# antonilo/unsupervised_detection

Measured on AMD Instinct MI355X. Metric: frame-pairs/sec per adversarial step, DAVIS 480p batch4, 1/2/4/8 GPU, higher is better.
Workload: dtype f32

## Files before the change

### include/udet.h

```cpp
#ifndef UDET_H
#define UDET_H
#include <stddef.h>
#ifdef __cplusplus
extern "C" {
#endif

#define UDET_OK 0
#define UDET_ERR_SHAPE (-1)
#define UDET_ERR_ALIGN (-2)
#define UDET_ERR_HIP (-3)
#define UDET_ERR_UNSUPPORTED (-4)
#define UDET_ERR_ARG (-5)
#define UDET_ERR_OVERFLOW (-6)

#define UDET_ACT_NONE 0
#define UDET_ACT_LEAKY 1
#define UDET_ACT_ELU 2

int udet_version(void);
const char* udet_last_error(void);


int udet_warp(const float* image, const float* flow, float flow_scale, float* out, int n, int h, int w, int c,
              void* stream);
// ... 31 lines not shown
size_t udet_conv2d_workspace_bytes(int n, int h, int w, int cin, int cout, int kh, int kw, int upsample2x);
int udet_conv2d(const float* x, const float* w_hwio, const float* bias, float* y, int n, int h, int w, int cin, int cout,
                int kh, int kw, int stride, int dilation, int upsample2x, int act, float alpha, void* workspace,
                size_t workspace_bytes, void* stream);
int udet_conv2d_backward_data(const float* dy, const float* y_saved, const float* w_hwio, float* dx, int n, int h, int w,
                              int cin, int cout, int kh, int kw, int stride, int dilation, int act, float alpha,
                              void* workspace, size_t workspace_bytes, void* stream);
int udet_conv2d_backward_filter(const float* x, const float* dy, const float* y_saved, float* dw_hwio, float* dbias, int n,
                                int h, int w, int cin, int cout, int kh, int kw, int stride, int dilation, int upsample2x,
                                int act, float alpha, void* workspace, size_t workspace_bytes, void* stream);
int udet_conv2d_transpose4x4s2(const float* x, const float* w_hwoi, const float* bias, float* y, int n, int h, int w,
                               int cin, int cout, void* workspace, size_t workspace_bytes, void* stream);


size_t udet_stage_workspace_bytes(int n);
int udet_flow_normalize(const float* flow, float* out, int n, int h, int w, void* workspace, size_t workspace_bytes, void* stream);
int udet_charbonnier_loss(const float* gt_flows, const float* pred_flows, const float* masks, int mask_channels, int n, int h, int w,
                          float cbn, float* out, void* workspace, size_t workspace_bytes, void* stream);
int udet_losses_forward(const float* flow, const float* mask, const float* pred3, int b, int h, int w, float cbn, float epsilon,
                        float* losses8, float* coef, void* workspace, size_t workspace_bytes, void* stream);
int udet_losses_backward(const float* flow, const float* mask, const float* pred3, const float* coef, int which, int b, int h, int w,
                         float cbn, float* dpred, float* dmask, void* stream);
int udet_clip_or_noise(float* g, size_t n, float clip, const float* flag2, unsigned long long seed, long step, void* stream);
int udet_adam_step(float* w, const float* g, float* m, float* v, size_t n, float lr, float beta1, float beta2, float eps, long t,
                   void* stream);

typedef struct udet_plan udet_plan;
typedef struct {
  int batch;
  int in_h, in_w;
  int img_h, img_w;
  float flow_normalizer;
  float cbn;
  float epsilon;
  float lr, beta1, beta2, adam_eps;
  float clip;
  unsigned long long noise_seed;
  int conv_fp16;
} udet_config;

int udet_plan_create(const udet_config* cfg, udet_plan** out);
void udet_plan_destroy(udet_plan* plan);
size_t udet_workspace_bytes(const udet_plan* plan);
int udet_plan_init(udet_plan* plan, void* workspace, void* stream);

int udet_param_count(int net);
size_t udet_param_total(int net);
int udet_param_info(int net, int index, const char** name, int* rank, int* shape4, size_t* offset_floats);
int udet_buffer_count(const udet_plan* plan);
int udet_buffer_info(const udet_plan* plan, int index, const char** name, size_t* offset_bytes, int* dims_nhw_ld);

int udet_pack_pwc(udet_plan* plan, const float* w_pwc, void* workspace, void* stream);
int udet_pack_trainable(udet_plan* plan, const float* w_gen, const float* w_rec, void* workspace, void* stream);

int udet_pwc_forward(udet_plan* plan, const float* img1, const float* img2, void* workspace, void* stream);
int udet_forward(udet_plan* plan, const float* img1, const float* img2, int ncalls, void* workspace, void* stream);
int udet_prefetch_flow(udet_plan* plan, const float* img1, const float* img2, void* workspace, void* stream);
int udet_forward_prefetched(udet_plan* plan, int ncalls, void* workspace, void* stream);
int udet_prefetch_consume(udet_plan* plan, void* workspace, void* stream);
int udet_forward_from_flow(udet_plan* plan, int ncalls, void* workspace, void* stream);
int udet_generator_forward(udet_plan* plan, void* workspace, void* stream);
int udet_generator_layers(udet_plan* plan, void* workspace, void* stream);
int udet_recover_forward(udet_plan* plan, int n, void* workspace, void* stream);
int udet_backward(udet_plan* plan, int which, const float* w_gen, const float* w_rec, float* g_gen, float* g_rec,
                  void* workspace, void* stream);
int udet_stream_wait_grads(udet_plan* plan, int net, void* stream);
int udet_generator_backward(udet_plan* plan, const float* w_gen, float* g_gen, void* workspace, void* stream);
int udet_recover_backward(udet_plan* plan, const float* w_rec, float* g_rec, void* workspace, void* stream);
int udet_grad_absmean(udet_plan* plan, int net, const float* g, float* out2, void* workspace, void* stream);
int udet_apply(udet_plan* plan, int net, float* w, float* g, float* m, float* v, void* workspace, void* stream);
long udet_fp16_overflow_count(udet_plan* plan);
long udet_get_adam_step(const udet_plan* plan);
void udet_set_adam_step(udet_plan* plan, long t);
int udet_train_step(udet_plan* plan, int which, const float* img1, const float* img2, float* w_gen, float* w_rec,
                    float* g_gen, float* g_rec, float* m_gen, float* v_gen, float* m_rec, float* v_rec, void* workspace,
                    void* stream);

int udet_autotune(udet_plan* plan, const float* w_gen, const float* w_rec, float* g_gen, float* g_rec, void* workspace,
                  void* stream);
int udet_tuned_shapes(void);
int udet_tune_save(const char* path);
int udet_tune_load(const char* path);
int udet_tune_rejected(void);
int udet_profile_begin(udet_plan* plan);
int udet_profile_end(udet_plan* plan, double* out, int ncat, void* stream);

int udet_plan_set_concurrent(udet_plan* plan, int on);

int udet_plan_lane_queues(udet_plan* plan, void* stream, int* queue);
int udet_plan_pin_lanes(udet_plan* plan, void* stream, void* const* side_streams, int n);

#ifdef __cplusplus
}
#endif
#endif
```

### include/udet_debug.h

```cpp
#ifndef UDET_DEBUG_H
#define UDET_DEBUG_H
#ifdef __cplusplus
extern "C" {
#endif
void udet_debug_force_conv(int bm, int bn, int ks);
void udet_debug_conv_fp16(int on);
void udet_debug_force_wgrad(int nsplit, int dma);
int udet_debug_last_wgrad(void);
void udet_debug_upb_min_pixels(long v);
void udet_debug_set_tuning(int on);
void udet_debug_force_pair(int on);
int udet_debug_last_pair(void);
#include <stddef.h>
int udet_debug_conv2d_pair(const float* xa, const float* xb, const float* wa, const float* wb, const float* ba, const float* bb, float* ya, float* yb,
                           int na, int nb, int h, int w, int cin, int cout, int k, int stride, int dilation, int act, float alpha, void* workspace,
                           size_t workspace_bytes, void* stream);
int udet_debug_last_conv(void);
#ifdef __cplusplus
}
#endif
#endif
```

### unsupervised_detection_amd/_devel.py

```python
from __future__ import annotations

import ctypes
import os

from ._ffi import lib as _lib

_PATH = os.path.join(os.path.dirname(os.path.abspath(__file__)), "libudet_debug.so")
if not os.path.exists(_PATH):
    raise RuntimeError(f"{_PATH} is missing: build it with `make -C unsupervised_detection_amd/csrc`")
dbg = ctypes.CDLL(_PATH, mode=ctypes.RTLD_GLOBAL)
dbg.udet_debug_force_conv.restype = None
dbg.udet_debug_force_conv.argtypes = [ctypes.c_int, ctypes.c_int, ctypes.c_int]
dbg.udet_debug_last_conv.restype = ctypes.c_int
dbg.udet_debug_last_conv.argtypes = []
dbg.udet_debug_conv_fp16.restype = None
dbg.udet_debug_conv_fp16.argtypes = [ctypes.c_int]
dbg.udet_debug_force_wgrad.restype = None
dbg.udet_debug_force_wgrad.argtypes = [ctypes.c_int, ctypes.c_int]
dbg.udet_debug_upb_min_pixels.restype = None
dbg.udet_debug_upb_min_pixels.argtypes = [ctypes.c_long]
dbg.udet_debug_set_tuning.restype = None
dbg.udet_debug_set_tuning.argtypes = [ctypes.c_int]
dbg.udet_debug_last_wgrad.restype = ctypes.c_int
dbg.udet_debug_last_wgrad.argtypes = []
dbg.udet_debug_force_pair.restype = None
dbg.udet_debug_force_pair.argtypes = [ctypes.c_int]
dbg.udet_debug_last_pair.restype = ctypes.c_int
dbg.udet_debug_last_pair.argtypes = []
dbg.udet_debug_conv2d_pair.restype = ctypes.c_int
dbg.udet_debug_conv2d_pair.argtypes = [ctypes.c_void_p] * 8 + [ctypes.c_int] * 10 + [ctypes.c_float, ctypes.c_void_p, ctypes.c_size_t, ctypes.c_void_p]
```

### unsupervised_detection_amd/csrc/api_plan.hip

```cpp
#include <stdlib.h>
#include <string.h>

#include "conv_host.h"
#include "elementwise.h"
#include "plan.h"

using namespace udet;

struct udet_plan {
  Plan* p;
};

extern "C" {

int udet_plan_create(const udet_config* c, udet_plan** out) {
  if (!c || !out) { set_error("plan_create: null argument"); return UDET_ERR_ARG; }
  Config k;
  k.batch = c->batch; k.in_h = c->in_h; k.in_w = c->in_w; k.img_h = c->img_h; k.img_w = c->img_w;
  k.flow_normalizer = c->flow_normalizer; k.cbn = c->cbn; k.epsilon = c->epsilon;
  k.lr = c->lr; k.beta1 = c->beta1; k.beta2 = c->beta2; k.adam_eps = c->adam_eps; k.clip = c->clip;
  k.noise_seed = c->noise_seed;
  k.conv_fp16 = c->conv_fp16 ? 1 : 0;
  Plan* P = plan_build(k);
  if (!P) return UDET_ERR_SHAPE;
// ... 8 lines not shown

int udet_param_count(int net) { return (net < 0 || net > 2) ? 0 : (int)net_params(net).p.size(); }
size_t udet_param_total(int net) { return (net < 0 || net > 2) ? 0 : net_params(net).total; }
int udet_param_info(int net, int i, const char** name, int* rank, int* shape, size_t* offset) {
  if (net < 0 || net > 2 || i < 0 || i >= (int)net_params(net).p.size()) { set_error("param_info: out of range"); return UDET_ERR_ARG; }
  const ParamDesc& d = net_params(net).p[i];
  *name = d.name.c_str(); *rank = d.rank; *offset = d.offset;
  for (int k = 0; k < 4; ++k) shape[k] = d.shape[k];
  return UDET_OK;
}
int udet_buffer_count(const udet_plan* h) { return (int)h->p->bufs.size(); }
int udet_buffer_info(const udet_plan* h, int i, const char** name, size_t* offset_bytes, int* dims) {
  if (i < 0 || i >= (int)h->p->bufs.size()) { set_error("buffer_info: out of range"); return UDET_ERR_ARG; }
  const Buf& b = h->p->bufs[i];
  *name = b.name.c_str(); *offset_bytes = b.off * sizeof(float);
  dims[0] = b.n; dims[1] = b.h; dims[2] = b.w; dims[3] = b.ld;
  return UDET_OK;
}
int udet_plan_set_concurrent(udet_plan* h, int on) {
  if (!h) { set_error("plan_set_concurrent: null plan"); return UDET_ERR_ARG; }
  if (on)
    if (h->p->cand.empty()) { set_error("plan_set_concurrent: the plan has no side streams"); return UDET_ERR_UNSUPPORTED; }
  h->p->concurrent = on != 0;
  return UDET_OK;
}
int udet_plan_lane_queues(udet_plan* h, void* stream, int* queue) {
  if (!h || !queue) { set_error("plan_lane_queues: null argument"); return UDET_ERR_ARG; }
  return plan_lane_queues(h->p, (hipStream_t)stream, queue);
}
int udet_plan_pin_lanes(udet_plan* h, void* stream, void* const* side_streams, int n) {
  if (!h || (n > 0 && !side_streams)) { set_error("plan_pin_lanes: null argument"); return UDET_ERR_ARG; }
  return plan_pin_lanes(h->p, (hipStream_t)stream, reinterpret_cast<hipStream_t const*>(side_streams), n);
}
long udet_fp16_overflow_count(udet_plan* h) {
  if (!h) return 0;
  (void)plan_check_overflow(h->p, true);
  return h->p->ovf_skipped;
}
long udet_get_adam_step(const udet_plan* h) {
  plan_settle_adam_step(h->p);
  return h->p->adam_t;
}
void udet_set_adam_step(udet_plan* h, long t) {
  plan_settle_adam_step(h->p);
  h->p->adam_t = t;
}

int udet_pack_pwc(udet_plan* h, const float* w_pwc, void* ws, void* stream) {
  return plan_pack_pwc(h->p, w_pwc, (float*)ws, (hipStream_t)stream);
}
int udet_pack_trainable(udet_plan* h, const float* w_gen, const float* w_rec, void* ws, void* stream) {
  return plan_pack_trainable(h->p, w_gen, w_rec, (float*)ws, (hipStream_t)stream);
}
int udet_pwc_forward(udet_plan* h, const float* img1, const float* img2, void* ws, void* stream) {
  return plan_pwc_forward(h->p, img1, img2, (float*)ws, (hipStream_t)stream);
}
int udet_forward_from_flow(udet_plan* h, int ncalls, void* ws, void* stream) {
  UDET_TRY(plan_check_overflow(h->p, false));
  if (ncalls < 0 || ncalls > 3) { set_error("forward: ncalls must be 0..3"); return UDET_ERR_ARG; }
  return plan_forward(h->p, nullptr, nullptr, ncalls, (float*)ws, (hipStream_t)stream);
}
int udet_generator_forward(udet_plan* h, void* ws, void* stream) {
  UDET_TRY(plan_generator_forward(h->p, (float*)ws, (hipStream_t)stream));
  return plan_recover_forward(h->p, 0, (float*)ws, (hipStream_t)stream);
}
int udet_generator_layers(udet_plan* h, void* ws, void* stream) {
  h->p->ev_next = 0;
  UDET_TRY(plan_generator_layers(h->p, (float*)ws, (hipStream_t)stream));
  return plan_recover_forward(h->p, 0, (float*)ws, (hipStream_t)stream);
}
int udet_recover_forward(udet_plan* h, int n, void* ws, void* stream) {
  if (n < 1 || n > 3) { set_error("recover_forward: n must be 1..3 (multiples of the plan batch)"); return UDET_ERR_ARG; }
  return plan_recover_forward(h->p, n, (float*)ws, (hipStream_t)stream, true);
}
int udet_forward(udet_plan* h, const float* img1, const float* img2, int ncalls, void* ws, void* stream) {
  UDET_TRY(plan_check_overflow(h->p, false));
  if (ncalls < 0 || ncalls > 3) { set_error("forward: ncalls must be 0..3"); return UDET_ERR_ARG; }
  if (!img1 || !img2) { set_error("forward: null image pointer"); return UDET_ERR_ARG; }
  return plan_forward(h->p, img1, img2, ncalls, (float*)ws, (hipStream_t)stream);
}
int udet_prefetch_flow(udet_plan* h, const float* img1, const float* img2, void* ws, void* stream) {
  if (!img1 || !img2) { set_error("prefetch_flow: null image pointer"); return UDET_ERR_ARG; }
  return plan_prefetch(h->p, img1, img2, (float*)ws, (hipStream_t)stream);
}
int udet_prefetch_consume(udet_plan* h, void* ws, void* stream) {
  return plan_prefetch_consume(h->p, (float*)ws, (hipStream_t)stream);
}
int udet_forward_prefetched(udet_plan* h, int ncalls, void* ws, void* stream) {
  UDET_TRY(plan_check_overflow(h->p, false));
  if (ncalls < 0 || ncalls > 3) { set_error("forward: ncalls must be 0..3"); return UDET_ERR_ARG; }
  return plan_forward(h->p, nullptr, nullptr, ncalls, (float*)ws, (hipStream_t)stream, true);
}
int udet_backward(udet_plan* h, int which, const float* w_gen, const float* w_rec, float* g_gen, float* g_rec, void* ws,
                  void* stream) {
  UDET_TRY(plan_check_overflow(h->p, false));
  if (which < 1 || which > 3) { set_error("backward: which must be 1 (generator), 2 (recover) or 3 (both)"); return UDET_ERR_ARG; }
  return plan_backward(h->p, which, w_gen, w_rec, g_gen, g_rec, (float*)ws, (hipStream_t)stream);
}
int udet_apply(udet_plan* h, int net, float* w, float* g, float* m, float* v, void* ws, void* stream) {
  return plan_apply(h->p, net, w, g, m, v, (float*)ws, (hipStream_t)stream);
}
int udet_train_step(udet_plan* h, int which, const float* img1, const float* img2, float* w_gen, float* w_rec, float* g_gen,
                    float* g_rec, float* m_gen, float* v_gen, float* m_rec, float* v_rec, void* ws, void* stream) {
  UDET_TRY(udet_pack_trainable(h, w_gen, w_rec, ws, stream));
  UDET_TRY(udet_forward(h, img1, img2, 3, ws, stream));
  UDET_TRY(udet_backward(h, which, w_gen, w_rec, g_gen, g_rec, ws, stream));
  if (which & 1) UDET_TRY(udet_apply(h, NET_GEN, w_gen, g_gen, m_gen, v_gen, ws, stream));
  if (which & 2) UDET_TRY(udet_apply(h, NET_REC, w_rec, g_rec, m_rec, v_rec, ws, stream));
  return UDET_OK;
}

int udet_autotune(udet_plan* h, const float* w_gen, const float* w_rec, float* g_gen, float* g_rec, void* ws_, void* stream) {
  Plan* P = h->p;
  float* ws = (float*)ws_;
  hipStream_t s = (hipStream_t)stream;
  if (!P->pwc_packed) { set_error("autotune: pack the PWC-Net and trainable weights first"); return UDET_ERR_ARG; }
  const size_t lo = P->packed_floats, hi = P->small_off;
  UDET_TRY(launch_fill_uniform(ws + lo, (long)(hi - lo), 0x5eedull, -0.5f, 0.5f, s));
  const size_t img_floats = (size_t)P->cfg.batch * P->cfg.in_h * P->cfg.in_w * 3;
  if (P->wgrad_floats < 2 * img_floats) { set_error("autotune: workspace too small for the probe images"); return UDET_ERR_ARG; }
  const float* img1 = ws + P->wgrad_off[0];
  const float* img2 = img1 + img_floats;
  const bool was_concurrent = P->concurrent;
  P->concurrent = false;
  conv_set_tuning(1);
  wgrad_set_tuning(1);
  int rc = udet_forward(h, img1, img2, 3, ws_, stream);
  if (rc == UDET_OK) rc = udet_backward(h, 3, w_gen, w_rec, g_gen, g_rec, ws_, stream);
  conv_set_tuning(0);
  wgrad_set_tuning(0);
  P->concurrent = was_concurrent;
  UDET_HIP(hipMemsetAsync(ws + lo, 0, (hi - lo) * sizeof(float), s));
  UDET_HIP(hipStreamSynchronize(s));
  return rc;
}
int udet_tuned_shapes(void) { return conv_tuned_shapes() + wgrad_tuned_shapes() + conv_pair_tuned_shapes(); }
int udet_tune_save(const char* path) {
  FILE* f = path ? fopen(path, "w") : nullptr;
  if (!f) { set_error("tune_save: cannot open %s", path ? path : "(null)"); return UDET_ERR_ARG; }
  fprintf(f, "udet-tune 2 abi %d\n", UDET_TUNE_ABI);
  conv_tune_dump(f);
  wgrad_tune_dump(f);
  conv_pair_tune_dump(f);
  fclose(f);
  return UDET_OK;
}
int udet_tune_load(const char* path) {
  FILE* f = path ? fopen(path, "r") : nullptr;
  if (!f) { set_error("tune_load: cannot open %s", path ? path : "(null)"); return UDET_ERR_ARG; }
  char line[256];
  int n = 0, ver = 0, abi = -1;
  if (!fgets(line, sizeof(line), f) || sscanf(line, "udet-tune %d abi %d", &ver, &abi) != 2 || ver != 2 || abi != UDET_TUNE_ABI) {
    fclose(f);
    set_error("tune_load: %s is not a udet-tune 2 file of this build (abi %d)", path, UDET_TUNE_ABI);
    return UDET_ERR_ARG;
  }
  while (fgets(line, sizeof(line), f)) {
    unsigned long long key;
    int a, b, c, d, e;
// ... 83 lines not shown
```

### unsupervised_detection_amd/csrc/common.h

```cpp
#pragma once
#include <hip/hip_runtime.h>
#include <hip/hip_ext.h>
#include <stdint.h>
#include <stdio.h>
#include <string>

#include "../../include/udet.h"

namespace udet {

void set_error(const char* fmt, ...);
int hip_fail(hipError_t e, const char* what);
#define UDET_HIP(x)                                   \
  do {                                                \
    hipError_t _e = (x);                              \
    if (_e != hipSuccess) return udet::hip_fail(_e, #x); \
  } while (0)
#define UDET_TRY(x)            \
  do {                         \
    int _s = (x);              \
    if (_s != 0) return _s;    \
  } while (0)

struct LaunchSink {
// ... 76 lines not shown
  int OHq, OWq;
  int osy, osx, ooy, oox;
  int isy, isx;
  int ntaps;
  ConvTap taps[UDET_MAX_TAPS];
  int ncls;
  int cls_tap[5];
  int nseg;
  ConvSeg seg[UDET_MAX_SEGS];
  int seg_tap[UDET_MAX_SEGS + 1];
  const ConvTap* tap_tab;
  int Mall;
  FastDiv fd_ohw, fd_ow;
  int kfast;
  const float* zero16;
  int act;
  float alpha;
  const float* res;
  int ldres, res_coff;
  float* y2;
  int ldy2, y2_coff;
  int accumulate;
  float* uo;
  int ldu, u_coff;
  const float* ua;
  int ldua, ua_coff, uact;
  float ualpha;
  int u_c0, u_c1;
  int ksplit;
  float* partial;
  size_t partial_cap;
  int ldp;
  int fold;
  int* tickets;
  int tail_full, tail_ks, tail_prow0;
  int f16;
  float f16_xscale;
  const float* wino_u;
  int wino_np;
  int kreal;
};
#define UDET_MAX_TICKETS 4096

int launch_conv(ConvParams& p, hipStream_t stream);
int launch_conv_pair(ConvParams& a, ConvParams& b, hipStream_t stream);
int launch_tap_gather(const ConvParams& g, const float* z, int ldz, hipStream_t stream);

struct PackJob {
  long src_off, dst_off, gamma_off, beta_off;
  long total;
  int T, R, C, Kc, ldw, k_split, k_gap, mode;
};

struct WgradParams {
  const float* x;
  int ldx, x_coff;
  int N, H, W, up_shift;
  int Cin;
  const float* dy;
  const float* ya;
  int ldy, y_coff, Cout;
  int yact;
  float yalpha;
  int OH, OW, isy, isx;
  int ycls, OHf, OWf;
  int ntaps;
  ConvTap taps[UDET_MAX_TAPS];
  float* dw;
  float* db;
  float* partial;
  size_t partial_floats;
  const float* zero16;
  int swapped, oCin, oCout, bias_m;
  int Cin4, Mpad;
  float* pbias;
  FastDiv fd_ohw, fd_ow;
  const float* w;
  const float* b;
  const float* gamma;
  float* dgamma;
  float* dbeta;
  float bn_c;
  int f16;
  float f16_yscale;
};
int launch_wgrad_T(WgradParams& p, int T, hipStream_t stream);
int launch_bn_finalize(float* dw, int T, int Cin, int Cout, const float* w, const float* b, const float* gamma, float bn_c, float* pd,
                       float* db, float* dgamma, float* dbeta, hipStream_t stream);
int launch_wgrad_up_combine(const float* deff, float* dw, int Cin, int Cout, hipStream_t stream);
size_t wgrad_partial_floats_needed(int T, int Cin, int Cout);

}
```

### unsupervised_detection_amd/csrc/conv_host.h

```cpp
#pragma once
#include "common.h"
namespace udet {
void same_pad(int in, int k, int s, int d, int* before, int* out);
void conv_setup_fwd(ConvParams& p, int N, int H, int W, int kh, int kw, int s, int d);
int conv_dgrad_classes(int s, int H, int W);
void conv_force_config(int bm, int bn, int ks);
bool conv_thin_n_ok(const ConvParams& p);
bool conv_thin_k_ok(const ConvParams& p);
int launch_conv_thin_n(const ConvParams& p, hipStream_t stream);
int launch_conv_thin_k(const ConvParams& p, hipStream_t stream);
bool conv_wino_geometry(const ConvParams& p, int* dil, int widx_at[9]);
bool conv_wino_ok(const ConvParams& p);
bool conv_wino_variant_ok(const ConvParams& p, int variant);
int conv_wino_np(int cout);
size_t conv_wino_floats(int Kc, int cout);
long conv_wino_workgroups(const ConvParams& p, int variant);
int conv_wino_max_ksplit(const ConvParams& p, int variant);
int launch_conv_wino(ConvParams& p, int variant, int ks, hipStream_t stream);
int launch_splitk_second_pass(const ConvParams& p, hipStream_t stream);
int launch_wino_pack(const float* src, float* dst, int R, int C, int Kc, int np, int k_split, int k_gap, int transposed, hipStream_t stream);
int launch_wino_from_packed(const ConvParams& p, float* dst, int np, hipStream_t stream);
void conv_debug_f16(int on);
int conv_debug_f16_on();
int conv_last_config();
void conv_set_tuning(int on);
int conv_tuned_shapes();
void conv_clear_tuning();
int conv_tune_rejected();
void conv_tune_note_reject();
float* tune_scratch(size_t floats, int which);
bool tune_compare(const float* a, const float* b, size_t n, hipStream_t stream, float* diff_out, float* scale_out);
void wgrad_set_tuning(int on);
bool wgrad_wino_ok(const WgradParams& p);
int wgrad_wino_slices(const WgradParams& p, int wanted);
int launch_wgrad_wino(const WgradParams& q, int slices, int ldn, hipStream_t stream);
int wgrad_last_config();
void wgrad_force(int nsplit, int dma);
int wgrad_tuned_shapes();
void conv_tune_dump(FILE* f);
void conv_tune_put(unsigned long long key, int bm, int bn, int ks, int ws, int fold, int tail);
void wgrad_tune_dump(FILE* f);
void conv_pair_tune_dump(FILE* f);
void conv_pair_tune_put(unsigned long long key, int bm, int bn, int ks, int ws);
int conv_pair_tuned_shapes();
void conv_pair_clear_tuning();
void conv_force_pair(int on);
int conv_last_pair();
#define UDET_TUNE_ABI 6
void wgrad_tune_put(unsigned long long key, int cfg);
bool conv_setup_dgrad(ConvParams& p, int cls, int N, int H, int W, int kh, int kw, int s, int d);
int launch_pack_weights(const float* src, float* dst, int T, int R, int C, int Kc, int ldw, int k_split, int k_gap,
                        int mode, const float* scale, hipStream_t stream);
int launch_pack_taps_into_n(const float* src, float* dst, int T, int R, int C, int Kc, int ldz, int k_split, int k_gap,
                            int transposed, hipStream_t stream);
int launch_pack_jobs(const PackJob* jobs_dev, int njobs, const float* wsrc, float* ws, float bn_c, hipStream_t stream);
int launch_fold_bn(const float* b, const float* gamma, const float* beta, float c, float* scale, float* bias_f, int n,
                   hipStream_t stream);
int launch_copy_channels(const float* src, int lds, int s_coff, float* dst, int ldd, int d_coff, long P, int C, float mul,
                         float add, hipStream_t stream);
int launch_warp(const float* img, const float* flow, int ldf, int f_coff, float flow_scale, float* out, int N, int H,
                int W, int C, int* dbg_idx, float* dbg_alpha, hipStream_t stream);
int launch_cost_volume(const float* c1, const float* wr, float* out, int ldo, int o_coff, int N, int H, int W, int C,
                       hipStream_t stream);
int launch_warp_cost_volume(const float* c1, const float* c2, const float* flow, int ldf, int f_coff, float flow_scale, float* out,
                            int ldo, int corr_coff, int c1_coff, float* warped_dbg, int N, int H, int W, int C, hipStream_t stream);
inline int round_up(int v, int m) { return (v + m - 1) / m * m; }
}
```

### unsupervised_detection_amd/csrc/conv_host.hip

```cpp
#include <string.h>

#include <stdint.h>

#include "common.h"
#include "conv_host.h"
#include "wino_pack.h"

namespace udet {

void same_pad(int in, int k, int s, int d, int* before, int* out) {
  const int o = (in + s - 1) / s;
  int total = (o - 1) * s + (k - 1) * d + 1 - in;
  if (total < 0) total = 0;
  *before = total / 2;
  *out = o;
}

static inline int floordiv2(int v) { return v >= 0 ? v / 2 : -((-v + 1) / 2); }

static void push_tap(ConvParams& p, int dy, int dx, int widx) {
  const int ymax = (p.OHq - 1) * p.isy + dy, xmax = (p.OWq - 1) * p.isx + dx;
  if (dy >= p.H || ymax < 0 || dx >= p.W || xmax < 0) return;
  p.taps[p.ntaps].dy = dy;
  p.taps[p.ntaps].dx = dx;
// ... 52 lines not shown
        if (((vx % 2) + 2) % 2) continue;
        push_tap(p, floordiv2(vy), floordiv2(vx), ky * kw + kx);
      }
    }
  }
  if (merged) {
    p.ncls = 4;
    p.cls_tap[4] = p.ntaps;
    p.ooy = p.oox = 0;
    p.OHq = H / 2; p.OWq = W / 2;
  }
  return true;
}

__global__ __launch_bounds__(256) void pack_weights_kernel(const float* __restrict__ src, float* __restrict__ dst, int T,
                                                           int R, int C, int Kc, int ldw, int k_split, int k_gap,
                                                           int mode, const float* __restrict__ scale) {
  const long total = (long)T * Kc * ldw;
  for (long e = (long)blockIdx.x * 256 + threadIdx.x; e < total; e += (long)gridDim.x * 256) {
    const int n = (int)(e % ldw);
    const int k = (int)((e / ldw) % Kc);
    const int t = (int)(e / ((long)ldw * Kc));
    float v = 0.f;
    int ks = k;
    if (k >= k_split) ks = (k < k_split + k_gap) ? -1 : k - k_gap;
    const int r = mode == 0 ? ks : n, c = mode == 0 ? n : ks;
    if (r >= 0 && r < R && c >= 0 && c < C) {
      v = src[((long)t * R + r) * C + c];
      if (scale) v *= scale[c];
    }
    dst[e] = v;
  }
}

int launch_pack_weights(const float* src, float* dst, int T, int R, int C, int Kc, int ldw, int k_split, int k_gap,
                        int mode, const float* scale, hipStream_t stream) {
  const long total = (long)T * Kc * ldw;
  int nb = (int)((total + 255) / 256);
  if (nb > 2048) nb = 2048;
  UDET_LAUNCH(pack_weights_kernel, dim3(nb), dim3(256), 0, stream, src, dst, T, R, C, Kc, ldw, k_split, k_gap,
                     mode, scale);
  UDET_HIP(hipGetLastError());
  return UDET_OK;
}

__constant__ float UPB_MERGE[2][3][3][4] = {
    {{{.5f, 0.f, 0.f, 0.f}, {.5f, 1.f, .5f, 0.f}, {0.f, 0.f, .5f, 1.f}},
     {{.5f, 0.f, 0.f, 0.f}, {.5f, 1.f, 1.f, 0.f}, {0.f, 0.f, 0.f, 0.f}},
     {{0.f, 0.f, 0.f, 0.f}, {0.f, 0.f, .5f, 0.f}, {0.f, 0.f, -.5f, -1.f}}},
    {{{1.f, .5f, 0.f, 0.f}, {0.f, .5f, 1.f, .5f}, {0.f, 0.f, 0.f, .5f}},
     {{1.f, 1.f, 0.f, 0.f}, {0.f, 0.f, 0.f, 0.f}, {0.f, 0.f, 0.f, 0.f}},
     {{0.f, .5f, 0.f, 0.f}, {0.f, -.5f, -1.f, -.5f}, {0.f, 0.f, 0.f, -.5f}}}};

__global__ __launch_bounds__(256) void pack_jobs_kernel(const PackJob* __restrict__ jobs, const float* __restrict__ wsrc,
                                                        float* __restrict__ ws, float bn_c) {
  const PackJob j = jobs[blockIdx.y];
  const float* src = wsrc + j.src_off;
  float* dst = ws + j.dst_off;
  const float* gamma = j.gamma_off >= 0 ? wsrc + j.gamma_off : nullptr;
  if (j.mode == 2) {
    for (long e = (long)blockIdx.x * 256 + threadIdx.x; e < j.total; e += (long)gridDim.x * 256)
      dst[e] = gamma ? src[e] * (gamma[e] * bn_c) + wsrc[j.beta_off + e] : src[e];
    return;
  }
  if (j.mode == 9 || j.mode == 10) {
    const int rv = (int)(j.beta_off / 3), cv = (int)(j.beta_off % 3);
    for (long e = (long)blockIdx.x * 256 + threadIdx.x; e < j.total; e += (long)gridDim.x * 256) {
      const int n = (int)(e % j.ldw), k = (int)(e / j.ldw);
      int ks = k;
      if (k >= j.k_split) ks = (k < j.k_split + j.k_gap) ? -1 : k - j.k_gap;
      const int ci = j.mode == 9 ? ks : n, co = j.mode == 9 ? n : ks;
      const bool real = ci >= 0 && ci < j.R && co >= 0 && co < j.C;
      float w[4][4];
#pragma unroll
      for (int kk = 0; kk < 4; ++kk)
#pragma unroll
        for (int ll = 0; ll < 4; ++ll) w[kk][ll] = real ? src[((long)(kk * 4 + ll) * j.R + ci) * j.C + co] : 0.f;
      const long plane = (long)j.Kc * j.ldw;
#pragma unroll
      for (int py = 0; py < 2; ++py) {
        float t1[3][4];
#pragma unroll
        for (int a = 0; a < 3; ++a)
#pragma unroll
          for (int ll = 0; ll < 4; ++ll) {
            float v = 0.f;
#pragma unroll
            for (int kk = 0; kk < 4; ++kk) v += UPB_MERGE[py][rv][a][kk] * w[kk][ll];
            t1[a][ll] = v;
          }
#pragma unroll
        for (int px = 0; px < 2; ++px)
#pragma unroll
          for (int a = 0; a < 3; ++a)
#pragma unroll
            for (int bb = 0; bb < 3; ++bb) {
              float v = 0.f;
#pragma unroll
              for (int ll = 0; ll < 4; ++ll) v += UPB_MERGE[px][cv][bb][ll] * t1[a][ll];
              dst[(long)((py * 2 + px) * 9 + a * 3 + bb) * plane + e] = v;
            }
      }
    }
    return;
  }
  if (j.mode == 7 || j.mode == 8) {
    for (long e = (long)blockIdx.x * 256 + threadIdx.x; e < j.total; e += (long)gridDim.x * 256) wino_pack_item(j, src, gamma, bn_c, dst, e);
    return;
  }
  for (long e = (long)blockIdx.x * 256 + threadIdx.x; e < j.total; e += (long)gridDim.x * 256) {
    const int n = (int)(e % j.ldw);
    const int k = (int)((e / j.ldw) % j.Kc);
    int t = (int)(e / ((long)j.ldw * j.Kc));
    float v = 0.f;
    int ks = k;
    if (k >= j.k_split) ks = (k < j.k_split + j.k_gap) ? -1 : k - j.k_gap;
    int r = j.mode == 0 ? ks : n, c = j.mode == 0 ? n : ks;
    if (j.mode == 3 || j.mode == 4) {
      t = n / j.C;
      c = n - t * j.C;
      r = ks;
      if (t >= j.T) r = -1;
    }
    if (j.mode >= 5) {
      const int cls = t >> 2, ty = (t >> 1) & 1, tx = t & 1, py = cls >> 1, px = cls & 1;
      const int y0 = py == 0 ? (ty == 0 ? 0 : 1) : (ty == 0 ? 0 : 2), y1 = py == 0 ? (ty == 0 ? 0 : 2) : (ty == 0 ? 1 : 2);
      const int x0 = px == 0 ? (tx == 0 ? 0 : 1) : (tx == 0 ? 0 : 2), x1 = px == 0 ? (tx == 0 ? 0 : 2) : (tx == 0 ? 1 : 2);
      const int ci = j.mode == 5 ? ks : n, co = j.mode == 5 ? n : ks;
      if (ci >= 0 && ci < j.R && co >= 0 && co < j.C) {
        for (int ky = y0; ky <= y1; ++ky)
          for (int kx = x0; kx <= x1; ++kx) v += src[((long)(ky * 3 + kx) * j.R + ci) * j.C + co];
        if (gamma) v *= gamma[co] * bn_c;
      }
      dst[e] = v;
      continue;
    }
    if (r >= 0 && r < j.R && c >= 0 && c < j.C) {
      v = j.mode == 4 ? src[((long)t * j.C + c) * j.R + r] : src[((long)t * j.R + r) * j.C + c];
      if (gamma) v *= gamma[c] * bn_c;
    }
    dst[e] = v;
  }
}
int launch_pack_jobs(const PackJob* jobs_dev, int njobs, const float* wsrc, float* ws, float bn_c, hipStream_t stream) {
  if (njobs < 1) return UDET_OK;
  UDET_LAUNCH(pack_jobs_kernel, dim3(48, njobs), dim3(256), 0, stream, jobs_dev, wsrc, ws, bn_c);
  UDET_HIP(hipGetLastError());
  return UDET_OK;
}

__global__ __launch_bounds__(256) void pack_job_kernel(const PackJob j, const float* __restrict__ wsrc, float* __restrict__ ws) {
  const float* src = wsrc + j.src_off;
  float* dst = ws + j.dst_off;
  for (long e = (long)blockIdx.x * 256 + threadIdx.x; e < j.total; e += (long)gridDim.x * 256) {
    const int n = (int)(e % j.ldw);
    const int k = (int)((e / j.ldw) % j.Kc);
    int ks = k;
    if (k >= j.k_split) ks = (k < j.k_split + j.k_gap) ? -1 : k - j.k_gap;
    const int t = n / j.C, c = n - t * j.C;
    float v = 0.f;
    if (ks >= 0 && ks < j.R && t < j.T) v = j.mode == 4 ? src[((long)t * j.C + c) * j.R + ks] : src[((long)t * j.R + ks) * j.C + c];
    dst[e] = v;
  }
}
int launch_pack_taps_into_n(const float* src, float* dst, int T, int R, int C, int Kc, int ldz, int k_split, int k_gap,
                            int transposed, hipStream_t stream) {
  PackJob j;
  memset(&j, 0, sizeof(j));
  j.T = T; j.R = R; j.C = C; j.Kc = Kc; j.ldw = ldz; j.k_split = k_split; j.k_gap = k_gap;
  j.mode = transposed ? 4 : 3; j.total = (long)Kc * ldz; j.gamma_off = -1;
  int nb = (int)((j.total + 255) / 256);
  if (nb > 1024) nb = 1024;
  UDET_LAUNCH(pack_job_kernel, dim3(nb), dim3(256), 0, stream, j, src, dst);
  UDET_HIP(hipGetLastError());
  return UDET_OK;
}

__global__ __launch_bounds__(256) void tap_gather_kernel(const ConvParams g, const float* __restrict__ z, int ldz) {
  const long total = (long)g.N * g.OH * g.OW * g.Cout;
  for (long e = (long)blockIdx.x * 256 + threadIdx.x; e < total; e += (long)gridDim.x * 256) {
    const int co = (int)(e % g.Cout);
    const long pix = e / g.Cout;
    const int ox = (int)(pix % g.OW), oy = (int)((pix / g.OW) % g.OH), n = (int)(pix / ((long)g.OW * g.OH));
    int cls = 0, qy = oy, qx = ox;
    if (g.ncls > 1) {
      cls = (oy & 1) * 2 + (ox & 1);
      qy = oy >> 1;
      qx = ox >> 1;
    }
    float v = g.bias ? g.bias[co] : 0.f;
    const int t1 = g.cls_tap[cls + 1];
    for (int t0 = g.cls_tap[cls]; t0 < t1; t0 += 8) {
      float a[8];
#pragma unroll
      for (int u = 0; u < 8; ++u) {
        const int t = t0 + u < t1 ? t0 + u : t1 - 1;
        const int iy = qy + g.taps[t].dy, ix = qx + g.taps[t].dx;
        const bool ok = t0 + u < t1 && (unsigned)iy < (unsigned)g.H && (unsigned)ix < (unsigned)g.W;
        a[u] = ok ? z[((size_t)(n * g.H + iy) * g.W + ix) * ldz + g.taps[t].widx * g.Cout + co] : 0.f;
// ... 97 lines not shown
```

### unsupervised_detection_amd/csrc/devel/api_debug.hip

```cpp
#include <string.h>

#include "../../../include/udet_debug.h"
#include "../conv_host.h"
#include "../plan.h"

using namespace udet;

extern "C" {
int udet_debug_last_conv(void) { return conv_last_config(); }
void udet_debug_force_conv(int bm, int bn, int ks) { conv_force_config(bm, bn, ks); }
void udet_debug_conv_fp16(int on) { conv_debug_f16(on); }
void udet_debug_force_wgrad(int nsplit, int dma) { wgrad_force(nsplit, dma); }
int udet_debug_last_wgrad(void) { return wgrad_last_config(); }
void udet_debug_upb_min_pixels(long v) { plan_debug_upb_min_pixels(v); }
void udet_debug_force_pair(int on) { conv_force_pair(on); }
int udet_debug_last_pair(void) { return conv_last_pair(); }
int udet_debug_conv2d_pair(const float* xa, const float* xb, const float* wa, const float* wb, const float* ba, const float* bb, float* ya, float* yb,
                           int na, int nb, int h, int w, int cin, int cout, int k, int stride, int dilation, int act, float alpha, void* workspace,
                           size_t workspace_bytes, void* stream_) {
  hipStream_t stream = (hipStream_t)stream_;
  if (cin % 8 != 0 || k * k > UDET_MAX_TAPS) { set_error("debug_conv2d_pair: cin must be a multiple of 8"); return UDET_ERR_SHAPE; }
  const int kc = cin, ldw = round_up(cout, 4);
  const size_t wfl = ((size_t)k * k * kc * ldw + 63) & ~(size_t)63, part_fl = (size_t)4 << 20, zero_fl = 64 + UDET_MAX_TICKETS;
  if (workspace_bytes < (2 * wfl + part_fl + zero_fl) * sizeof(float)) { set_error("debug_conv2d_pair: workspace too small"); return UDET_ERR_ARG; }
  float* wpa = reinterpret_cast<float*>(workspace);
  float* wpb = wpa + wfl;
  float* part = wpb + wfl;
  float* zero = part + part_fl;
  UDET_HIP(hipMemsetAsync(zero, 0, zero_fl * sizeof(float), stream));
  UDET_TRY(launch_pack_weights(wa, wpa, k * k, cin, cout, kc, ldw, kc, 0, 0, nullptr, stream));
  UDET_TRY(launch_pack_weights(wb, wpb, k * k, cin, cout, kc, ldw, kc, 0, 0, nullptr, stream));
  ConvParams p[2];
  for (int i = 0; i < 2; ++i) {
    memset(&p[i], 0, sizeof(ConvParams));
    conv_setup_fwd(p[i], i ? nb : na, h, w, k, k, stride, dilation);
    p[i].x = i ? xb : xa; p[i].ldx = cin; p[i].wp = i ? wpb : wpa; p[i].Kc = kc; p[i].ldw = ldw; p[i].bias = i ? bb : ba;
    p[i].y = i ? yb : ya; p[i].ldy = cout; p[i].Cout = cout; p[i].act = act; p[i].alpha = alpha;
    p[i].partial = part; p[i].partial_cap = part_fl; p[i].zero16 = zero; p[i].tickets = reinterpret_cast<int*>(zero + 64);
  }
  return launch_conv_pair(p[0], p[1], stream);
}
void udet_debug_set_tuning(int on) {
  conv_set_tuning(on);
  wgrad_set_tuning(on);
}
}
```

### unsupervised_detection_amd/csrc/elementwise.h

```cpp
#pragma once
#include "common.h"
namespace udet {
int launch_resize_bilinear_fwd(const float* x, int ldx, int x_coff, int N, int H, int W, float* y, int ldy, int y_coff,
                               int OH, int OW, int C, float mul, float div, hipStream_t s);
int launch_resize_bilinear_bwd(const float* dy, int ldy, int y_coff, int N, int OH, int OW, float* dx, int ldx, int x_coff,
                               int H, int W, int C, int accumulate, hipStream_t s);
int launch_upb_ring(const float* x, int ld, int N, int H, int W, float* xh, hipStream_t s);
int launch_upb_ring_fold(const float* dxh, int ld, int N, int H, int W, float* dx, hipStream_t s);
int launch_share_samples(float* buf, long P, int ld, int coff, int C, int copies, hipStream_t s);
int launch_fold_samples(float* buf, long P, int ld, int coff, int C, int copies, hipStream_t s);
int launch_emit_du(const float* d, const float* a, float* u, long P, int ld, int coff, int C, int act, float alpha, hipStream_t s);
int launch_pool2x2_sum(const float* du, float* dx, int N, int H, int W, int C, hipStream_t s);
int launch_pack_pwc_input(const float* i1, const float* i2, float* x8, long P, hipStream_t s);
int launch_gen_input(const float* img, const float* f, double* part, float* gin, int B, long HW, hipStream_t s);
size_t flow_stats_doubles(int B);
int launch_mask_rec_inputs(const float* logits, const float* f, float* mask, float* fin, long P, int ncalls, hipStream_t s);
int launch_pack_imgin(const float* img, float* imgin, long P, int ncalls, hipStream_t s);
int launch_losses(const float* f, const float* mask, const float* pred, long HW, int B, float cbn, float eps,
                  float num_pixels, float* part, float* losses, float* coef, float* sums, hipStream_t s);
size_t loss_part_floats(int B);
int launch_rec_loss_bwd(const float* f, const float* mask, const float* pred, float* dpred, long BHW, float cbn,
                        float inv_np, hipStream_t s);
int launch_gen_loss_bwd(const float* f, const float* mask, const float* pred, const float* coef, float* dpred,
                        float* dmask, long HW, int B, float cbn, hipStream_t s);
int launch_mask_bwd(const float* dmask, const float* dfin, const float* f, const float* mask, float* dlogits, long P,
                    hipStream_t s);
int launch_grad_absmean(const float* g, const long* seg_off, const long* seg_len, int nvars, float* vmean, float thresh,
                        float* out, hipStream_t s);
int launch_adam(float* w, float* g, float* m, float* v, long n, float lr_t, float b1, float b2, float eps, float clip,
                const float* flag, uint64_t seed, uint64_t step, hipStream_t s, int mode = 0, const int* skip = nullptr);
int launch_nonfinite_count(const float* g, long n, int* out, hipStream_t s);
int launch_flow_normalize(const float* f, double* part, float* out, int B, long HW, hipStream_t s);
int launch_charbonnier(const float* gt, const float* pred, const float* mask, int mc, int B, long HW, float cbn, float* part,
                       float* out, hipStream_t s);
int launch_crop_flip_resize(const void* src, int src_u8, int nearest, int N, int H, int W, int C, const int* prm, float* dst, int OH,
                            int OW, float div, float add, hipStream_t s);
int launch_crop_flip_resize_ragged(const void* src, int src_u8, int nearest, int N, int C, const long long* offsets, const int* hw,
                                   const int* prm, float* dst, int OH, int OW, float div, float add, hipStream_t s);
int launch_mask_stats(const float* pred, const float* gt, int N, int H, int W, float threshold, float gt_threshold, double* out,
                      hipStream_t s);
int launch_fill_uniform(float* x, long n, uint64_t seed, float lo, float hi, hipStream_t s);
int launch_axpy(const float* x, float* y, long n, float a, int accumulate, hipStream_t s);
}
```

### unsupervised_detection_amd/csrc/elementwise.hip

```cpp
#include "common.h"
#include "elementwise.h"

namespace udet {

static inline int grid_for(long total, int cap = 4096) {
  long nb = (total + 255) / 256;
  if (nb > cap) nb = cap;
  if (nb < 1) nb = 1;
  return (int)nb;
}

template <typename T>
__device__ __forceinline__ T wave_sum(T v) {
#pragma unroll
  for (int o = 32; o > 0; o >>= 1) v += __shfl_down(v, o, 64);
  return v;
}
template <typename T>
__device__ __forceinline__ T block_sum(T v, T* sm ) {
  v = wave_sum(v);
  __syncthreads();
  if ((threadIdx.x & 63) == 0) sm[threadIdx.x >> 6] = v;
  __syncthreads();
  return sm[0] + sm[1] + sm[2] + sm[3];
// ... 441 lines not shown
  return UDET_OK;
}

__global__ __launch_bounds__(256) void mask_rec_inputs_kernel(const float* __restrict__ logits ,
                                                              const float* __restrict__ f, float* __restrict__ mask,
                                                              float* __restrict__ fin, long P, int ncalls) {
  for (long q = (long)blockIdx.x * 256 + threadIdx.x; q < P; q += (long)gridDim.x * 256) {
    const float l0 = logits[q * 8] / 10.f, l1 = logits[q * 8 + 1] / 10.f;
    const float mx = fmaxf(l0, l1);
    const float e0 = expf(l0 - mx), e1 = expf(l1 - mx);
    const float m = e0 / (e0 + e1);
    mask[q] = m;
    const float cm = 1.f - m;
    const float2 v = *reinterpret_cast<const float2*>(f + q * 2);
    const float a0 = 1.f - m, a1 = 1.f - cm;
    if (ncalls > 0) {
      *reinterpret_cast<float4*>(fin + q * 4) = make_float4(v.x * a0, v.y * a0, 1.f, a0);
    }
    if (ncalls > 1) {
      *reinterpret_cast<float4*>(fin + (P + q) * 4) = make_float4(v.x * a1, v.y * a1, 1.f, a1);
    }
    if (ncalls > 2) {
      *reinterpret_cast<float4*>(fin + (2 * P + q) * 4) = make_float4(0.f, 0.f, 1.f, 0.f);
    }
  }
}
int launch_mask_rec_inputs(const float* logits, const float* f, float* mask, float* fin, long P, int ncalls, hipStream_t s) {
  hipLaunchKernelGGL(mask_rec_inputs_kernel, dim3(grid_for(P)), dim3(256), 0, s, logits, f, mask, fin, P, ncalls);
  UDET_HIP(hipGetLastError());
  return UDET_OK;
}
__global__ __launch_bounds__(256) void pack_imgin_kernel(const float* __restrict__ img, float* __restrict__ imgin, long P,
                                                         int ncalls) {
  for (long q = (long)blockIdx.x * 256 + threadIdx.x; q < P; q += (long)gridDim.x * 256) {
    const float4 im = make_float4(img[q * 3], img[q * 3 + 1], img[q * 3 + 2], 0.f);
    for (int k = 0; k < ncalls; ++k) *reinterpret_cast<float4*>(imgin + (k * P + q) * 4) = im;
  }
}
int launch_pack_imgin(const float* img, float* imgin, long P, int ncalls, hipStream_t s) {
  hipLaunchKernelGGL(pack_imgin_kernel, dim3(grid_for(P)), dim3(256), 0, s, img, imgin, P, ncalls);
  UDET_HIP(hipGetLastError());
  return UDET_OK;
}

__device__ __forceinline__ float charb(float e, float cbn) {
  const float s = e * e + 0.001f * 0.001f;
  return cbn == 0.5f ? sqrtf(s) : powf(s, cbn);
}
__device__ __forceinline__ float charb_d(float e, float cbn) {
  const float s = e * e + 0.001f * 0.001f;
  return cbn == 0.5f ? e / sqrtf(s) : cbn * powf(s, cbn - 1.f) * 2.f * e;
}
#define LS_BLOCKS 64
__global__ __launch_bounds__(256) void loss_sums_kernel(const float* __restrict__ f, const float* __restrict__ mask,
                                                        const float* __restrict__ pred , long HW, int B,
                                                        float cbn, float* __restrict__ part ) {
  __shared__ float sm[4];
  const int n = blockIdx.y;
  float R = 0, Rc = 0, Pp = 0, Dr = 0, Dc = 0;
  for (long p = (long)blockIdx.x * 256 + threadIdx.x; p < HW; p += (long)gridDim.x * 256) {
    const long q = (long)n * HW + p;
    const float2 fl = *reinterpret_cast<const float2*>(f + q * 2);
    const float2 a = *reinterpret_cast<const float2*>(pred + q * 2);
    const float2 b = *reinterpret_cast<const float2*>(pred + ((long)B * HW + q) * 2);
    const float2 c = *reinterpret_cast<const float2*>(pred + ((long)2 * B * HW + q) * 2);
    const float m = mask[q], cm = 1.f - m;
    const float pa = charb(fl.x - a.x, cbn) + charb(fl.y - a.y, cbn);
    const float pb = charb(fl.x - b.x, cbn) + charb(fl.y - b.y, cbn);
    const float pc = charb(fl.x - c.x, cbn) + charb(fl.y - c.y, cbn);
    R += pa * m; Rc += pb * cm; Pp += pc; Dr += pc * m; Dc += pc * cm;
  }
  R = block_sum(R, sm); Rc = block_sum(Rc, sm); Pp = block_sum(Pp, sm); Dr = block_sum(Dr, sm); Dc = block_sum(Dc, sm);
  if (threadIdx.x == 0) {
    float* o = part + ((long)n * LS_BLOCKS + blockIdx.x) * 5;
    o[0] = R; o[1] = Rc; o[2] = Pp; o[3] = Dr; o[4] = Dc;
  }
}
__global__ void loss_finish_kernel(const float* __restrict__ part, int B, float eps, float num_pixels,
                                   float* __restrict__ losses, float* __restrict__ coef, float* __restrict__ sums) {
  if (threadIdx.x != 0 || blockIdx.x != 0) return;
  float red = 0.f, redc = 0.f, rs = 0.f;
  for (int b = 0; b < B; ++b) {
    float v[5] = {0, 0, 0, 0, 0};
    for (int k = 0; k < LS_BLOCKS; ++k)
      for (int j = 0; j < 5; ++j) v[j] += part[((long)b * LS_BLOCKS + k) * 5 + j];
    const float D = v[3] + eps, Dc = v[4] + eps;
    red += 1.f - v[0] / D;
    redc += 1.f - v[1] / Dc;
    rs += v[0] + v[1] + v[2];
    coef[b * 4 + 0] = -1.f / (B * D);
    coef[b * 4 + 1] = v[0] / (B * D * D);
    coef[b * 4 + 2] = -1.f / (B * Dc);
    coef[b * 4 + 3] = v[1] / (B * Dc * Dc);
    for (int j = 0; j < 5; ++j) sums[b * 5 + j] = v[j];
    if (b == 0) { losses[4] = v[0]; losses[5] = v[1]; losses[6] = D; losses[7] = Dc; }
  }
  red /= B; redc /= B;
  losses[0] = red + redc;
  losses[1] = rs / num_pixels;
  losses[2] = red;
  losses[3] = redc;
}
int launch_losses(const float* f, const float* mask, const float* pred, long HW, int B, float cbn, float eps,
                  float num_pixels, float* part, float* losses, float* coef, float* sums, hipStream_t s) {
  hipLaunchKernelGGL(loss_sums_kernel, dim3(LS_BLOCKS, B), dim3(256), 0, s, f, mask, pred, HW, B, cbn, part);
  hipLaunchKernelGGL(loss_finish_kernel, dim3(1), dim3(64), 0, s, part, B, eps, num_pixels, losses, coef, sums);
  UDET_HIP(hipGetLastError());
  return UDET_OK;
}
size_t loss_part_floats(int B) { return (size_t)B * LS_BLOCKS * 5; }

__global__ __launch_bounds__(256) void charbonnier_sum_kernel(const float* __restrict__ gt, const float* __restrict__ pred,
                                                              const float* __restrict__ mask, int mc, long HW, float cbn,
                                                              float* __restrict__ part ) {
  __shared__ float sm[4];
  const int n = blockIdx.y;
  float acc = 0.f;
  for (long p = (long)blockIdx.x * 256 + threadIdx.x; p < HW; p += (long)gridDim.x * 256) {
    const long q = (long)n * HW + p;
    const float2 a = *reinterpret_cast<const float2*>(gt + q * 2);
    const float2 b = *reinterpret_cast<const float2*>(pred + q * 2);
    const float m0 = mask ? mask[q * mc] : 1.f, m1 = mask ? mask[q * mc + (mc - 1)] : 1.f;
    acc += charb(a.x - b.x, cbn) * m0 + charb(a.y - b.y, cbn) * m1;
  }
  acc = block_sum(acc, sm);
  if (threadIdx.x == 0) part[(long)n * LS_BLOCKS + blockIdx.x] = acc;
}
__global__ void charbonnier_finish_kernel(const float* __restrict__ part, int B, float* __restrict__ out) {
  const int b = blockIdx.x * blockDim.x + threadIdx.x;
  if (b >= B) return;
  float v = 0.f;
  for (int k = 0; k < LS_BLOCKS; ++k) v += part[(long)b * LS_BLOCKS + k];
  out[b] = v;
}
int launch_charbonnier(const float* gt, const float* pred, const float* mask, int mc, int B, long HW, float cbn, float* part,
                       float* out, hipStream_t s) {
  hipLaunchKernelGGL(charbonnier_sum_kernel, dim3(LS_BLOCKS, B), dim3(256), 0, s, gt, pred, mask, mc, HW, cbn, part);
  hipLaunchKernelGGL(charbonnier_finish_kernel, dim3((B + 63) / 64), dim3(64), 0, s, part, B, out);
  UDET_HIP(hipGetLastError());
  return UDET_OK;
}

__global__ __launch_bounds__(256) void rec_loss_bwd_kernel(const float* __restrict__ f, const float* __restrict__ mask,
                                                           const float* __restrict__ pred, float* __restrict__ dpred,
                                                           long BHW, float cbn, float inv_np) {
  for (long q = (long)blockIdx.x * 256 + threadIdx.x; q < BHW; q += (long)gridDim.x * 256) {
    const float2 fl = *reinterpret_cast<const float2*>(f + q * 2);
    const float m = mask[q], cm = 1.f - m;
    const float2 a = *reinterpret_cast<const float2*>(pred + q * 2);
    const float2 b = *reinterpret_cast<const float2*>(pred + (BHW + q) * 2);
    const float2 c = *reinterpret_cast<const float2*>(pred + (2 * BHW + q) * 2);
    *reinterpret_cast<float2*>(dpred + q * 2) = make_float2(-charb_d(fl.x - a.x, cbn) * m * inv_np, -charb_d(fl.y - a.y, cbn) * m * inv_np);
    *reinterpret_cast<float2*>(dpred + (BHW + q) * 2) = make_float2(-charb_d(fl.x - b.x, cbn) * cm * inv_np, -charb_d(fl.y - b.y, cbn) * cm * inv_np);
    *reinterpret_cast<float2*>(dpred + (2 * BHW + q) * 2) = make_float2(-charb_d(fl.x - c.x, cbn) * inv_np, -charb_d(fl.y - c.y, cbn) * inv_np);
  }
}
int launch_rec_loss_bwd(const float* f, const float* mask, const float* pred, float* dpred, long BHW, float cbn,
                        float inv_np, hipStream_t s) {
  hipLaunchKernelGGL(rec_loss_bwd_kernel, dim3(grid_for(BHW)), dim3(256), 0, s, f, mask, pred, dpred, BHW, cbn, inv_np);
// ... 42 lines not shown
    dm += g1.x * fl.x + g1.y * fl.y + g1.w;
    const float m = mask[q];
    const float d0 = dm * m * (1.f - m) / 10.f;
    dlogits[q * 8] = d0;
    dlogits[q * 8 + 1] = -d0;
  }
}
int launch_mask_bwd(const float* dmask, const float* dfin, const float* f, const float* mask, float* dlogits, long P,
                    hipStream_t s) {
  hipLaunchKernelGGL(mask_bwd_kernel, dim3(grid_for(P)), dim3(256), 0, s, dmask, dfin, f, mask, dlogits, P);
  UDET_HIP(hipGetLastError());
  return UDET_OK;
}

#define GA_SPLIT 8
__global__ __launch_bounds__(256) void grad_absmean_kernel(const float* __restrict__ g, const long* __restrict__ seg_off,
                                                           const long* __restrict__ seg_len, float* __restrict__ vpart) {
  __shared__ float sm[4];
  const long off = seg_off[blockIdx.x], len = seg_len[blockIdx.x];
  const long b = len * blockIdx.y / GA_SPLIT, e = len * (blockIdx.y + 1) / GA_SPLIT;
  float s0 = 0.f, s1 = 0.f, s2 = 0.f, s3 = 0.f;
  long i = b + threadIdx.x;
  for (; i + 768 < e; i += 1024) {
    s0 += fabsf(g[off + i]);
    s1 += fabsf(g[off + i + 256]);
    s2 += fabsf(g[off + i + 512]);
    s3 += fabsf(g[off + i + 768]);
  }
  for (; i < e; i += 256) s0 += fabsf(g[off + i]);
  const float s = block_sum((s0 + s1) + (s2 + s3), sm);
  if (threadIdx.x == 0) vpart[blockIdx.x * GA_SPLIT + blockIdx.y] = s;
}
__global__ void grad_flag_kernel(const float* __restrict__ vpart, const long* __restrict__ seg_len, int nvars, float thresh,
                                 float* __restrict__ out ) {
  if (threadIdx.x == 0 && blockIdx.x == 0) {
    float s = 0.f;
    for (int i = 0; i < nvars; ++i) {
      float v = 0.f;
      for (int j = 0; j < GA_SPLIT; ++j) v += vpart[i * GA_SPLIT + j];
      s += v / (float)seg_len[i];
    }
    s /= (float)nvars;
    out[0] = s;
    out[1] = s < thresh ? 1.f : 0.f;
  }
}
int launch_grad_absmean(const float* g, const long* seg_off, const long* seg_len, int nvars, float* vmean, float thresh,
                        float* out, hipStream_t s) {
  hipLaunchKernelGGL(grad_absmean_kernel, dim3(nvars, GA_SPLIT), dim3(256), 0, s, g, seg_off, seg_len, vmean);
  hipLaunchKernelGGL(grad_flag_kernel, dim3(1), dim3(64), 0, s, vmean, seg_len, nvars, thresh, out);
  UDET_HIP(hipGetLastError());
  return UDET_OK;
}

__device__ __host__ __forceinline__ float udet_uniform01(uint64_t seed, uint64_t step, uint64_t idx) {
  uint64_t z = seed * 0x9E3779B97F4A7C15ull + step * 0xBF58476D1CE4E5B9ull + idx + 0x94D049BB133111EBull;
  z = (z ^ (z >> 30)) * 0xBF58476D1CE4E5B9ull;
  z = (z ^ (z >> 27)) * 0x94D049BB133111EBull;
  z = z ^ (z >> 31);
  return (float)(z >> 40) * (1.0f / 16777216.0f);
}

__global__ __launch_bounds__(256) void adam_kernel(float* __restrict__ w, float* __restrict__ g, float* __restrict__ m,
                                                   float* __restrict__ v, long n, float lr_t, float b1, float b2, float eps,
                                                   float clip, const float* __restrict__ flag, uint64_t seed,
                                                   uint64_t step, int mode, const int* __restrict__ skip) {
  if (skip && *skip != 0) return;
  const bool noise = flag && flag[1] != 0.f;
  for (long i = (long)blockIdx.x * 256 + threadIdx.x; i < n; i += (long)gridDim.x * 256) {
    float gi = g[i];
    if (mode != 2) {
      if (noise) gi = fabsf((udet_uniform01(seed, step, (uint64_t)i) * 2.f - 1.f) * clip);
      else gi = fminf(fmaxf(gi, -clip), clip);
      g[i] = gi;
      if (mode == 1) continue;
    }
    const float mi = m[i] + (gi - m[i]) * (1.f - b1);
    const float vi = v[i] + (gi * gi - v[i]) * (1.f - b2);
    m[i] = mi;
    v[i] = vi;
    w[i] = w[i] - lr_t * mi / (sqrtf(vi) + eps);
  }
}
__global__ __launch_bounds__(256) void fill_uniform_kernel(float* __restrict__ x, long n, uint64_t seed, float lo, float hi) {
  for (long i = (long)blockIdx.x * 256 + threadIdx.x; i < n; i += (long)gridDim.x * 256)
    x[i] = lo + (hi - lo) * udet_uniform01(seed, 0, (uint64_t)i);
}
int launch_fill_uniform(float* x, long n, uint64_t seed, float lo, float hi, hipStream_t s) {
  hipLaunchKernelGGL(fill_uniform_kernel, dim3(grid_for(n, 8192)), dim3(256), 0, s, x, n, seed, lo, hi);
  UDET_HIP(hipGetLastError());
  return UDET_OK;
}
__global__ __launch_bounds__(256) void mask_stats_kernel(const float* __restrict__ pred, const float* __restrict__ gt, int H, int W,
                                                         float threshold, float gt_threshold, double* __restrict__ out) {
  __shared__ double sm[4];
  const int n = blockIdx.x;
  const long HW = (long)H * W;
  double v[8] = {0, 0, 0, 0, 0, 0, 0, 0};
  for (long q = threadIdx.x; q < HW; q += 256) {
    const int y = (int)(q / W), x = (int)(q - (long)y * W);
    const float g = gt[n * HW + q];
    const bool pr = pred[n * HW + q] > threshold, gb = g > gt_threshold;
    const int strips = (y < 2) + (y >= H - 2) + (x < 2) + (x >= W - 2);
    const double a1 = fabs((double)g - 1.0), a0 = fabs((double)g);
    if (pr) {
      v[0] += strips; v[1] += 1.0; v[4] += a1; v[7] += a0;
      if (gb) v[3] += 1.0;
    } else {
      v[5] += a0; v[6] += a1;
    }
    if (gb) v[2] += 1.0;
  }
  for (int k = 0; k < 8; ++k) {
    const double s = block_sum(v[k], sm);
    if (threadIdx.x == 0) out[(long)n * 8 + k] = s;
    __syncthreads();
  }
}
int launch_mask_stats(const float* pred, const float* gt, int N, int H, int W, float threshold, float gt_threshold, double* out,
                      hipStream_t s) {
  hipLaunchKernelGGL(mask_stats_kernel, dim3(N), dim3(256), 0, s, pred, gt, H, W, threshold, gt_threshold, out);
  UDET_HIP(hipGetLastError());
  return UDET_OK;
}
int launch_adam(float* w, float* g, float* m, float* v, long n, float lr_t, float b1, float b2, float eps, float clip,
                const float* flag, uint64_t seed, uint64_t step, hipStream_t s, int mode, const int* skip) {
  hipLaunchKernelGGL(adam_kernel, dim3(grid_for(n, 2048)), dim3(256), 0, s, w, g, m, v, n, lr_t, b1, b2, eps, clip, flag, seed,
                     step, mode, skip);
  UDET_HIP(hipGetLastError());
  return UDET_OK;
}
__global__ __launch_bounds__(256) void nonfinite_count_kernel(const float* __restrict__ g, long n, int* __restrict__ out) {
  int c = 0;
  for (long i = (long)blockIdx.x * 256 + threadIdx.x; i < n; i += (long)gridDim.x * 256) c += !(fabsf(g[i]) <= 3.402823466e38f);
#pragma unroll
  for (int o = 32; o > 0; o >>= 1) c += __shfl_xor(c, o);
  if ((threadIdx.x & 63) == 0 && c) {
    atomicAdd(out, c);
    atomicAdd(out + 1, c);
  }
}
int launch_nonfinite_count(const float* g, long n, int* out, hipStream_t s) {
  UDET_HIP(hipMemsetAsync(out, 0, sizeof(int), s));
  hipLaunchKernelGGL(nonfinite_count_kernel, dim3(grid_for(n, 1024)), dim3(256), 0, s, g, n, out);
  UDET_HIP(hipGetLastError());
  return UDET_OK;
}

__global__ __launch_bounds__(256) void upb_ring_kernel(const float* __restrict__ x, int ldx, int N, int H, int W, float* __restrict__ xh, int C4) {
  const int PH = H + 2, PW = W + 2;
  const long total = (long)N * PH * PW * C4;
  for (long e = (long)blockIdx.x * 256 + threadIdx.x; e < total; e += (long)gridDim.x * 256) {
    const int c4 = (int)(e % C4);
    const long pix = e / C4;
    const int C = (int)(pix % PW), R = (int)((pix / PW) % PH), n = (int)(pix / ((long)PW * PH));
    const int cy = R < 1 ? 0 : (R - 1 > H - 1 ? H - 1 : R - 1), cx = C < 1 ? 0 : (C - 1 > W - 1 ? W - 1 : C - 1);
    const float sg = ((R == 0) != (C == 0)) ? -1.f : 1.f;
    const float4 v = *reinterpret_cast<const float4*>(x + (((long)n * H + cy) * W + cx) * ldx + c4 * 4);
    *reinterpret_cast<float4*>(xh + pix * ldx + c4 * 4) = make_float4(v.x * sg, v.y * sg, v.z * sg, v.w * sg);
  }
}
int launch_upb_ring(const float* x, int ld, int N, int H, int W, float* xh, hipStream_t s) {
  const long total = (long)N * (H + 2) * (W + 2) * (ld / 4);
  hipLaunchKernelGGL(upb_ring_kernel, dim3(grid_for(total, 8192)), dim3(256), 0, s, x, ld, N, H, W, xh, ld / 4);
  UDET_HIP(hipGetLastError());
  return UDET_OK;
}
__global__ __launch_bounds__(256) void upb_ring_fold_kernel(const float* __restrict__ dxh, int ld, int N, int H, int W, float* __restrict__ dx, int C4) {
  const int PW = W + 2, PH = H + 2;
  const long total = (long)N * H * W * C4;
  for (long e = (long)blockIdx.x * 256 + threadIdx.x; e < total; e += (long)gridDim.x * 256) {
    const int c4 = (int)(e % C4);
    const long pix = e / C4;
    const int i = (int)(pix % W), j = (int)((pix / W) % H), n = (int)(pix / ((long)W * H));
    float4 a = make_float4(0.f, 0.f, 0.f, 0.f);
#pragma unroll
    for (int ry = 0; ry < 2; ++ry) {
      int R;
      float sy = 1.f;
      if (ry == 0) R = j + 1;
      else if (j == 0) { R = 0; sy = -1.f; }
// ... 38 lines not shown
```

### unsupervised_detection_amd/csrc/plan.h

```cpp
#pragma once
#include <map>
#include <string>
#include <vector>

#include "common.h"

namespace udet {

struct ParamDesc {
  std::string name;
  int rank;
  int shape[4];
  size_t offset, count;
};
struct NetParams {
  std::vector<ParamDesc> p;
  size_t total = 0;
  int add(const std::string& name, int a, int b = 0, int c = 0, int d = 0);
  int find(const std::string& name) const;
};
enum { NET_PWC = 0, NET_GEN = 1, NET_REC = 2 };
const NetParams& net_params(int net);

struct Buf {
// ... 31 lines not shown
    int seg_tap[UDET_MAX_SEGS + 1];
    std::vector<ConvTap> taps;
    size_t tab_off = 0;
  } upb_f, upb_b;
  int x = -1, x_coff = 0, y = -1, y_coff = 0;
  int res = -1, res_coff = 0, y2 = -1;
  int H = 0, W = 0;
  bool col2im = false;
  int ldz = 0, zbuf = -1;
  size_t wz_off = 0;
};

struct Config {
  int batch, in_h, in_w, img_h, img_w;
  float flow_normalizer, cbn, epsilon;
  float lr, beta1, beta2, adam_eps, clip;
  unsigned long long noise_seed;
  int conv_fp16 = 0;
};

struct Plan {
  Config cfg;
  std::vector<Buf> bufs;
  std::map<std::string, int> buf_by_name;
  std::vector<Layer> pwc, gen, rec;
  size_t packed_floats = 0;
  size_t arena_floats = 0;
  enum { NLANE = 6, NCAND = 8, MAXCAND = 32 };
  std::vector<hipStream_t> cand;
  struct Placement {
    hipStream_t main = nullptr;
    hipStream_t lane[NLANE] = {};
    int queue[NLANE] = {};
    int nqueues = 1;
  };
  std::vector<Placement> placements;
  int placed = -1;
  hipEvent_t prefetch_ev = nullptr;
  hipEvent_t grad_ev[3] = {nullptr, nullptr, nullptr};
  bool prefetch_pending = false;
  std::vector<hipEvent_t> ev_pool, ev_pool_prefetch;
  size_t ev_next = 0, ev_next_prefetch = 0;
  bool in_prefetch = false;
  bool concurrent = true;
  bool enc_a_shared = false;
  size_t scratch_off[NLANE] = {}, scratch_floats = 0;
  size_t wgrad_off[NLANE] = {}, wgrad_floats = 0;
  ~Plan();
  size_t small_off = 0;
  size_t ticket_off = 0;
  size_t seg_off[3] = {0, 0, 0};
  size_t jobs_off[3] = {0, 0, 0};
  int njobs[3] = {0, 0, 0};
  struct ProfRec {
    int cat; double flops, bytes; hipEvent_t a, b; std::string name;
    double mfma_scale = 1.0;
    enum { MAXK = 16 };
    hipEvent_t kev[2 * MAXK];
    LaunchSink sink;
  };
  bool profiling = false;
  std::vector<ProfRec*> prof;
  long adam_t = 0;
  int* ovf_host = nullptr;
  hipEvent_t ovf_ev[3] = {nullptr, nullptr, nullptr};
  bool ovf_pending[3] = {false, false, false};
  long ovf_skipped = 0;
  int ovf_report_values = 0, ovf_report_nets = 0;
  bool pwc_packed = false;
  int add_buf(const std::string& name, int n, int h, int w, int ld);
  const Buf& buf(int id) const { return bufs[id]; }
  int bid(const std::string& name) const;
};

#define UDET_PACKJOB_CAP(layers) (8 * (layers) + 32)
#define UDET_SMALL_NOISE 256
#define UDET_SMALL_OVF 300
#define UDET_SMALL_SUMS 1024
Plan* plan_build(const Config& cfg);
void plan_debug_upb_min_pixels(long v);
enum { UDET_KNOB_ENC_A_LANE = 0, UDET_KNOB_REC_DEC_WGRAD_LANE = 1, UDET_KNOB_REC_ENC_WGRAD_LANE = 2, UDET_KNOB_GEN_WGRAD_LATE = 3, UDET_KNOB_NO_WGRAD_WINO = 6, UDET_KNOB_SKIP = 7, UDET_KNOB_NO_PAIRS = 8, UDET_KNOB_COUNT = 12 };
#ifdef UDET_EXPERIMENT
void plan_debug_knob(int id, long v);
long plan_knob(int id);
#else
constexpr long plan_knob(int) { return 0; }
#endif

int plan_init_workspace(Plan* P, float* ws, hipStream_t s);
int plan_pack_pwc(Plan* P, const float* w_pwc, float* ws, hipStream_t s);
int plan_pack_trainable(Plan* P, const float* w_gen, const float* w_rec, float* ws, hipStream_t s);
int plan_pwc_forward(Plan* P, const float* img1, const float* img2, float* ws, hipStream_t s);
int plan_forward(Plan* P, const float* img1, const float* img2, int ncalls, float* ws, hipStream_t s, bool prefetched = false);
int plan_prefetch(Plan* P, const float* img1, const float* img2, float* ws, hipStream_t s);
int plan_prefetch_consume(Plan* P, float* ws, hipStream_t s);
int plan_generator_forward(Plan* P, float* ws, hipStream_t s);
int plan_generator_layers(Plan* P, float* ws, hipStream_t s);
int plan_recover_forward(Plan* P, int ncalls, float* ws, hipStream_t s, bool inputs_prepacked = false, bool skip_enc_a = false, bool enc_a_input_packed = false);
int plan_losses(Plan* P, float* ws, hipStream_t s);
int plan_backward(Plan* P, int which, const float* w_gen, const float* w_rec, float* g_gen, float* g_rec, float* ws, hipStream_t s);
int plan_apply(Plan* P, int net, float* w, float* g, float* m, float* v, float* ws, hipStream_t s);
int plan_check_overflow(Plan* P, bool wait);
void plan_settle_adam_step(Plan* P);
int plan_lane_queues(Plan* P, hipStream_t s, int* queue);
int plan_pin_lanes(Plan* P, hipStream_t main, hipStream_t const* streams, int n);
enum { PROF_CONV_FWD = 0, PROF_CONV_DGRAD = 1, PROF_CONV_WGRAD = 2, PROF_WARP = 3, PROF_CORR = 4, PROF_NCAT = 5 };
void prof_begin(Plan* P, int cat, double flops, double bytes, hipStream_t s, const char* name = "");
void prof_end(Plan* P, hipStream_t s);

}
```

### unsupervised_detection_amd/csrc/plan_build.hip

```cpp
#include <stdarg.h>
#include <stdlib.h>
#include <string.h>

#include "conv_host.h"
#include "elementwise.h"
#include "plan.h"

namespace udet {

int NetParams::add(const std::string& name, int a, int b, int c, int d) {
  ParamDesc q;
  q.name = name;
  q.shape[0] = a; q.shape[1] = b; q.shape[2] = c; q.shape[3] = d;
  q.rank = d ? 4 : (c ? 3 : (b ? 2 : 1));
  q.count = (size_t)a * (b ? b : 1) * (c ? c : 1) * (d ? d : 1);
  q.offset = total;
  total += q.count;
  p.push_back(q);
  return (int)p.size() - 1;
}
int NetParams::find(const std::string& name) const {
  for (size_t i = 0; i < p.size(); ++i)
    if (p[i].name == name) return (int)i;
  return -1;
// ... 91 lines not shown
    for (int i = 0; i < 9; ++i) {
      const int ci = ENC[i].cin ? ENC[i].cin : (e == 0 ? 3 : 4);
      n.add(S("FlownetS/%c%s/weights", e == 0 ? 'a' : 'b', ENC[i].suf), ENC[i].k, ENC[i].k, ci, ENC[i].cout);
      n.add(S("FlownetS/%c%s/biases", e == 0 ? 'a' : 'b', ENC[i].suf), ENC[i].cout);
    }
  for (int i = 0; i < 14; ++i) {
    n.add(S("FlownetS/%s/weights", DEC[i].name), DEC[i].k, DEC[i].k, DEC[i].cin, DEC[i].cout);
    n.add(S("FlownetS/%s/biases", DEC[i].name), DEC[i].cout);
  }
  return n;
}

const NetParams& net_params(int net) {
  static const NetParams pwc = build_pwc_params(), gen = build_gen_params(), rec = build_rec_params();
  return net == NET_PWC ? pwc : (net == NET_GEN ? gen : rec);
}

int Plan::add_buf(const std::string& name, int n, int h, int w, int ld) {
  Buf b;
  b.name = name; b.n = n; b.h = h; b.w = w; b.ld = ld; b.off = 0;
  bufs.push_back(b);
  buf_by_name[name] = (int)bufs.size() - 1;
  return (int)bufs.size() - 1;
}
int Plan::bid(const std::string& name) const {
  auto it = buf_by_name.find(name);
  return it == buf_by_name.end() ? -1 : it->second;
}

static Layer mk_layer(int net, const std::string& name, const std::string& wname, const std::string& bname, int k, int cin,
                      int cout, int stride, int dil, int act, float alpha) {
  Layer L;
  L.name = name; L.net = net;
  L.kh = L.kw = k; L.cin = cin; L.cout = cout; L.stride = stride; L.dil = dil;
  L.act = act; L.alpha = alpha;
  const NetParams& np = net_params(net);
  L.w_idx = np.find(wname);
  L.b_idx = np.find(bname);
  L.Kc = round_up(cin, cin <= 4 ? 4 : 8);
  L.ldw = round_up(cout, 4);
  L.k_split = L.Kc;
  L.k_gap = 0;
  return L;
}

static size_t align64(size_t v) { return (v + 63) & ~(size_t)63; }

Plan::~Plan() {
  for (auto& st : cand)
    if (st) (void)hipStreamDestroy(st);
  for (auto& e : ev_pool) (void)hipEventDestroy(e);
  for (auto& e : ev_pool_prefetch) (void)hipEventDestroy(e);
  if (prefetch_ev) (void)hipEventDestroy(prefetch_ev);
  for (auto* r : prof) delete r;
  for (auto& ev : grad_ev)
    if (ev) (void)hipEventDestroy(ev);
  for (auto& ev : ovf_ev)
    if (ev) (void)hipEventDestroy(ev);
  if (ovf_host) (void)hipHostFree(ovf_host);
}

static long g_upb_bwd_min = 8192;
void plan_debug_upb_min_pixels(long v) { g_upb_bwd_min = v < 0 ? 8192 : v; }
#ifdef UDET_EXPERIMENT
static long g_knob[UDET_KNOB_COUNT] = {};
void plan_debug_knob(int id, long v) { if (id >= 0 && id < UDET_KNOB_COUNT) g_knob[id] = v; }
long plan_knob(int id) { return id >= 0 && id < UDET_KNOB_COUNT ? g_knob[id] : 0; }
extern "C" void udet_exp_knob(int id, long v) { plan_debug_knob(id, v); }
#endif

static inline bool upb_used(int parity, int last, int a) { return !last || (parity == 0 ? a < 2 : a < 1); }
static void build_upb_launches(Layer& L, int h, int w) {
  Layer::SegLaunch& F = L.upb_f;
  F.nseg = 0; F.taps.clear();
  for (int r = 0; r < 4; ++r) {
    const int rv = r & 1, cv = r >> 1;
    const int r0 = rv ? h - 1 : 0, c0 = cv ? w - 1 : 0, nr = rv ? 1 : h - 1, nc = cv ? 1 : w - 1;
    for (int c = 0; c < 4; ++c) {
      const int py = c >> 1, px = c & 1;
      ConvSeg& g = F.seg[F.nseg];
      memset(&g, 0, sizeof(g));
      g.oy = 2 * r0 + py; g.ox = 2 * c0 + px; g.h = nr; g.w = nc;
      F.seg_tap[F.nseg++] = (int)F.taps.size();
      for (int a = 0; a < 3; ++a)
        for (int b = 0; b < 3; ++b) {
          if (!upb_used(py, rv, a) || !upb_used(px, cv, b)) continue;
          F.taps.push_back(ConvTap{r0 + a + py, c0 + b + px, r * 36 + 9 * c + 3 * a + b});
        }
    }
  }
  F.seg_tap[F.nseg] = (int)F.taps.size();
  Layer::SegLaunch& B = L.upb_b;
  B.nseg = 0; B.taps.clear();
  struct Combo { int p, a, last; };
  auto combos = [](int grp, std::vector<Combo>& out) {
    out.clear();
    for (int p = 0; p < 2; ++p)
      for (int a = 0; a < 3; ++a) {
        int last = 0;
        if (grp > 0) {
          const int rp = grp - 1;
          if (p + a < rp) continue;
          last = (p + a == rp);
        }
        if (upb_used(p, last, a)) out.push_back(Combo{p, a, last});
      }
// ... 295 lines not shown
      L.ldwT = round_up(L.cin, 4);
      L.wpT_off = off; off = align64(off + (size_t)T * L.KcT * L.ldwT);
    }
    if (L.up) {
      L.wu_off = off; off = align64(off + (size_t)16 * L.Kc * L.ldw);
      L.wuT_off = off; off = align64(off + (size_t)16 * L.KcT * L.ldwT);
    }
    if (L.upb) {
      L.wupb_off = off; off = align64(off + (size_t)4 * 36 * L.Kc * L.ldw);
      L.upb_f.tab_off = off; off = align64(off + L.upb_f.taps.size() * (sizeof(ConvTap) / sizeof(float)));
      if (L.upb_bwd) {
        L.wupbT_off = off; off = align64(off + (size_t)4 * 36 * L.KcT * L.ldwT);
        L.upb_b.tab_off = off; off = align64(off + L.upb_b.taps.size() * (sizeof(ConvTap) / sizeof(float)));
      }
    }
    if (!cfg.conv_fp16 && L.kh == 3 && L.kw == 3 && L.stride == 1 && !L.up && !L.transposed && !L.col2im && L.cout >= 16 && L.H * L.W >= 512) {
      if (L.Kc % 8 == 0) {
        L.wino_np = conv_wino_np(L.cout);
        L.wino_off = off; off = align64(off + conv_wino_floats(L.Kc, L.cout));
      }
      if (trainable && L.KcT % 8 == 0 && L.cin >= 16) {
        L.winoT_np = conv_wino_np(L.cin);
        L.winoT_off = off; off = align64(off + conv_wino_floats(L.KcT, L.cin));
      }
    }
  };
  for (auto& L : P->pwc) place(L, false);
  for (auto& L : P->gen) place(L, true);
  for (auto& L : P->rec) place(L, true);
  P->packed_floats = off;

  for (auto& b : P->bufs) { b.off = off; off = align64(off + b.floats()); }
  P->scratch_floats = (size_t)24 << 20;
  P->wgrad_floats = (size_t)48 << 20;
  for (int l = 0; l < Plan::NLANE; ++l) {
    P->scratch_off[l] = off;
    off = align64(off + P->scratch_floats);
    P->wgrad_off[l] = off;
    if (l < 4) off = align64(off + P->wgrad_floats);
  }
  P->small_off = off;
  off = align64(off + 65536);
  P->ticket_off = off;
  off = align64(off + (size_t)Plan::NLANE * UDET_MAX_TICKETS);
  for (int net = 1; net <= 2; ++net) {
    P->seg_off[net] = off;
    off = align64(off + 4 * net_params(net).p.size() + 64);
  }
  for (int net = 1; net <= 2; ++net) {
    const size_t nl = net == NET_GEN ? P->gen.size() : P->rec.size();
    P->jobs_off[net] = off;
    off = align64(off + UDET_PACKJOB_CAP(nl) * (sizeof(PackJob) / sizeof(float)) + 64);
  }
  P->arena_floats = off;
  if (const char* e = getenv("UDET_SERIAL")) P->concurrent = atoi(e) == 0;
  for (int i = 0; i < Plan::NCAND; ++i) {
    hipStream_t c = nullptr;
    if (hipStreamCreateWithFlags(&c, hipStreamNonBlocking) == hipSuccess) P->cand.push_back(c);
  }
  if (P->cand.empty()) P->concurrent = false;
  struct { const char* n; int a, d; size_t o; } views[5] = {{"losses", 1, 8, 0}, {"loss_coef", B, 4, 16}, {"noise_flag", 1, 2, UDET_SMALL_NOISE},
                                                            {"fp16_overflow", 2, 2, UDET_SMALL_OVF}, {"loss_sums", B, 5, UDET_SMALL_SUMS}};
  for (auto& v : views) {
    const int id = P->add_buf(v.n, v.a, 1, 1, v.d);
    P->bufs[id].off = P->small_off + v.o;
  }
  return P;
}

}
```

### unsupervised_detection_amd/csrc/plan_exec.hip

```cpp
#include <math.h>
#include <stdlib.h>
#include <string.h>

#include "conv_host.h"
#include "elementwise.h"
#include "lanes.h"
#include "plan.h"

namespace udet {

static const float BN_C = 0.99950037468777316f;

static const Layer* find_layer(const std::vector<Layer>& v, const std::string& name) {
  for (const auto& L : v)
    if (L.name == name) return &L;
  return nullptr;
}
static std::string S(const char* fmt, int a, int b = 0) {
  char buf[128];
  snprintf(buf, sizeof(buf), fmt, a, b);
  return buf;
}

void prof_begin(Plan* P, int cat, double flops, double bytes, hipStream_t s, const char* name) {
// ... 430 lines not shown
    UDET_TRY(run_fwd(P, La, Na, ws, ln));
    return run_fwd(P, Lb, Nb, ws, ln);
  }
  if (skip_launch(0, La.net)) return UDET_OK;
  ConvParams a, b;
  fwd_params(P, La, Na, ws, ln.slot, a);
  fwd_params(P, Lb, Nb, ws, ln.slot, b);
  prof_begin(P, PROF_CONV_FWD, layer_flops(La, Na) + layer_flops(Lb, Nb), layer_bytes(La, Na) + layer_bytes(Lb, Nb), ln.s, (La.name + "+" + Lb.name).c_str());
  const int rc = launch_conv_pair(a, b, ln.s);
  prof_end(P, ln.s);
  return rc;
}
static bool dgrad_params(Plan* P, const Layer& L, int N, int dy, int dx, int dx_coff, int accumulate, const Emit& em, float* ws, int slot, ConvParams& p) {
  if (L.up || L.upb || L.transposed || conv_dgrad_classes(L.stride, L.H, L.W) != 1) return false;
  const Buf &bdy = P->buf(dy), &bdx = P->buf(dx);
  memset(&p, 0, sizeof(p));
  if (!conv_setup_dgrad(p, 0, N, L.H, L.W, L.kh, L.kw, L.stride, L.dil)) return false;
  p.x = ws + bdy.off; p.ldx = bdy.ld; p.x_coff = L.y_coff;
  p.wp = ws + L.wpT_off; p.Kc = L.KcT; p.ldw = L.ldwT; p.kreal = L.cout;
  p.y = ws + bdx.off; p.ldy = bdx.ld; p.y_coff = dx_coff; p.Cout = L.cin;
  p.accumulate = accumulate;
  if (em.ubuf >= 0) {
    const Buf &bu = P->buf(em.ubuf), &bua = P->buf(em.abuf);
    p.uo = ws + bu.off; p.ldu = bu.ld; p.u_coff = dx_coff;
    p.ua = ws + bua.off; p.ldua = bua.ld; p.ua_coff = dx_coff;
    p.uact = em.act; p.ualpha = em.alpha; p.u_c0 = em.c0; p.u_c1 = em.c1;
  }
  if (L.winoT_off) { p.wino_u = ws + L.winoT_off; p.wino_np = L.winoT_np; }
  fill_common(P, p, ws, slot);
  p.f16_xscale = UDET_F16_GRAD_SCALE;
  return true;
}
struct DgradJob {
  const Layer* L;
  int N, dy, dx, dx_coff, accumulate;
  Emit em;
};
static int run_dgrad_pair(Plan* P, const DgradJob& ja, const DgradJob& jb, float* ws, const Lane& ln) {
  ConvParams a, b;
  if (!pairs_on(P, 1) || !dgrad_params(P, *ja.L, ja.N, ja.dy, ja.dx, ja.dx_coff, ja.accumulate, ja.em, ws, ln.slot, a) ||
      !dgrad_params(P, *jb.L, jb.N, jb.dy, jb.dx, jb.dx_coff, jb.accumulate, jb.em, ws, ln.slot, b)) {
    UDET_TRY(run_dgrad(P, *ja.L, ja.N, ja.dy, true, ja.dx, ja.dx_coff, ja.accumulate, -1, ja.em, ws, ln));
    return run_dgrad(P, *jb.L, jb.N, jb.dy, true, jb.dx, jb.dx_coff, jb.accumulate, -1, jb.em, ws, ln);
  }
  if (skip_launch(1, ja.L->net)) return UDET_OK;
  a.wino_u = b.wino_u = nullptr;
  prof_begin(P, PROF_CONV_DGRAD, layer_flops(*ja.L, ja.N) + layer_flops(*jb.L, jb.N), layer_bytes(*ja.L, ja.N) + layer_bytes(*jb.L, jb.N), ln.s,
             (ja.L->name + "+" + jb.L->name).c_str());
  const int rc = launch_conv_pair(a, b, ln.s);
  prof_end(P, ln.s);
  return rc;
}

int plan_init_workspace(Plan* P, float* ws, hipStream_t s) {
  UDET_HIP(hipMemsetAsync(ws, 0, P->arena_floats * sizeof(float), s));
  for (int net = 1; net <= 2; ++net) {
    const NetParams& np = net_params(net);
    std::vector<long> tab(2 * np.p.size());
    for (size_t i = 0; i < np.p.size(); ++i) {
      tab[i] = (long)np.p[i].offset;
      tab[np.p.size() + i] = (long)np.p[i].count;
    }
    UDET_HIP(hipMemcpyAsync(ws + P->seg_off[net], tab.data(), tab.size() * sizeof(long), hipMemcpyHostToDevice, s));
    UDET_HIP(hipStreamSynchronize(s));
  }
  for (int net = 1; net <= 2; ++net) {
    const NetParams& np = net_params(net);
    const std::vector<Layer>& layers = net == NET_GEN ? P->gen : P->rec;
    std::vector<PackJob> jobs;
    for (const auto& L : layers) {
      const int T = L.kh * L.kw;
      const long goff = L.g_idx >= 0 ? (long)np.p[L.g_idx].offset : -1, beoff = L.be_idx >= 0 ? (long)np.p[L.be_idx].offset : -1;
      PackJob j;
      memset(&j, 0, sizeof(j));
      j.src_off = (long)np.p[L.w_idx].offset; j.gamma_off = goff; j.beta_off = beoff;
      j.T = T;
      j.dst_off = (long)L.wp_off; j.R = L.cin; j.C = L.cout; j.Kc = L.Kc; j.ldw = L.ldw; j.k_split = L.k_split; j.k_gap = L.k_gap;
      j.mode = 0; j.total = (long)T * L.Kc * L.ldw;
      jobs.push_back(j);
      j.dst_off = (long)L.wpT_off; j.Kc = L.KcT; j.ldw = L.ldwT; j.k_split = L.KcT; j.k_gap = 0;
      j.mode = 1; j.total = (long)T * L.KcT * L.ldwT;
      jobs.push_back(j);
      if (L.col2im) {
        j.dst_off = (long)L.wz_off; j.R = L.cin; j.C = L.cout; j.Kc = L.Kc; j.ldw = L.ldz; j.k_split = L.k_split; j.k_gap = L.k_gap;
        j.mode = 3; j.total = (long)L.Kc * L.ldz;
        jobs.push_back(j);
      }
      if (L.up) {
        j.T = 16;
        j.dst_off = (long)L.wu_off; j.R = L.cin; j.C = L.cout; j.Kc = L.Kc; j.ldw = L.ldw; j.k_split = L.Kc; j.k_gap = 0;
        j.mode = 5; j.total = (long)16 * L.Kc * L.ldw;
        jobs.push_back(j);
        j.dst_off = (long)L.wuT_off; j.Kc = L.KcT; j.ldw = L.ldwT; j.k_split = L.KcT; j.k_gap = 0;
        j.mode = 6; j.total = (long)16 * L.KcT * L.ldwT;
        jobs.push_back(j);
        j.T = T;
      }
      if (L.upb)
        for (int r = 0; r < 4; ++r) {
          j.T = 36; j.gamma_off = -1;
          j.dst_off = (long)(L.wupb_off + (size_t)r * 36 * L.Kc * L.ldw); j.R = L.cin; j.C = L.cout; j.Kc = L.Kc; j.ldw = L.ldw; j.k_split = L.k_split; j.k_gap = L.k_gap;
          j.mode = 9; j.beta_off = (long)((r & 1) * 3 + (r >> 1)); j.total = (long)L.Kc * L.ldw;
          jobs.push_back(j);
          if (L.upb_bwd) {
            j.dst_off = (long)(L.wupbT_off + (size_t)r * 36 * L.KcT * L.ldwT); j.Kc = L.KcT; j.ldw = L.ldwT; j.k_split = L.KcT; j.k_gap = 0;
            j.mode = 10; j.total = (long)L.KcT * L.ldwT;
            jobs.push_back(j);
          }
          j.T = T; j.beta_off = beoff;
        }
      if (L.wino_off) {
        j.dst_off = (long)L.wino_off; j.R = L.cin; j.C = L.cout; j.Kc = L.Kc; j.ldw = L.wino_np; j.k_split = L.k_split; j.k_gap = L.k_gap;
        j.mode = 7; j.total = (long)(L.Kc / 8) * 2 * L.wino_np;
        jobs.push_back(j);
      }
      if (L.winoT_off) {
        j.dst_off = (long)L.winoT_off; j.R = L.cin; j.C = L.cout; j.Kc = L.KcT; j.ldw = L.winoT_np; j.k_split = L.KcT; j.k_gap = 0;
        j.mode = 8; j.total = (long)(L.KcT / 8) * 2 * L.winoT_np;
        jobs.push_back(j);
      }
      j.src_off = (long)np.p[L.b_idx].offset; j.dst_off = (long)L.bias_f_off; j.mode = 2; j.total = L.cout;
      jobs.push_back(j);
    }
    if (jobs.size() > UDET_PACKJOB_CAP(layers.size())) {
      set_error("plan_init: %zu weight re-layout jobs for %zu layers exceed the table's %zu entries", jobs.size(), layers.size(),
                (size_t)UDET_PACKJOB_CAP(layers.size()));
      return UDET_ERR_ARG;
    }
    P->njobs[net] = (int)jobs.size();
    UDET_HIP(hipMemcpyAsync(ws + P->jobs_off[net], jobs.data(), jobs.size() * sizeof(PackJob), hipMemcpyHostToDevice, s));
    UDET_HIP(hipStreamSynchronize(s));
  }
  for (const auto& L : P->rec)
    if (L.upb)
      for (const Layer::SegLaunch* g : {&L.upb_f, &L.upb_b})
        if (g == &L.upb_f || L.upb_bwd)
          UDET_HIP(hipMemcpyAsync(ws + g->tab_off, g->taps.data(), g->taps.size() * sizeof(ConvTap), hipMemcpyHostToDevice, s));
  UDET_HIP(hipStreamSynchronize(s));
  P->pwc_packed = false;
  return UDET_OK;
}

static int pack_layer(const Layer& L, const float* w_flat, float* ws, const float* scale, bool trainable, hipStream_t s) {
  const NetParams& np = net_params(L.net);
  const float* w = w_flat + np.p[L.w_idx].offset;
  const int T = L.kh * L.kw;
  if (L.transposed)
    UDET_TRY(launch_pack_weights(w, ws + L.wp_off, T, L.cout, L.cin, L.Kc, L.ldw, L.k_split, L.k_gap, 1, nullptr, s));
  else
    UDET_TRY(launch_pack_weights(w, ws + L.wp_off, T, L.cin, L.cout, L.Kc, L.ldw, L.k_split, L.k_gap, 0, scale, s));
  if (trainable)
    UDET_TRY(launch_pack_weights(w, ws + L.wpT_off, T, L.cin, L.cout, L.KcT, L.ldwT, L.KcT, 0, 1, scale, s));
  if (L.col2im)
    UDET_TRY(launch_pack_taps_into_n(w, ws + L.wz_off, T, L.cin, L.cout, L.Kc, L.ldz, L.k_split, L.k_gap, L.transposed ? 1 : 0, s));
  if (L.wino_off && !trainable)
    UDET_TRY(launch_wino_pack(w, ws + L.wino_off, L.cin, L.cout, L.Kc, L.wino_np, L.k_split, L.k_gap, 0, s));
  return UDET_OK;
}

int plan_pack_pwc(Plan* P, const float* w, float* ws, hipStream_t s) {
  const NetParams& np = net_params(NET_PWC);
  for (const auto& L : P->pwc) {
    UDET_TRY(pack_layer(L, w, ws, nullptr, false, s));
    UDET_TRY(launch_copy_channels(w + np.p[L.b_idx].offset, L.cout, 0, ws + L.bias_f_off, L.cout, 0, 1, L.cout, 1.f, 0.f, s));
  }
  P->pwc_packed = true;
  return UDET_OK;
}

int plan_pack_trainable(Plan* P, const float* w_gen, const float* w_rec, float* ws, hipStream_t s) {
  if (w_gen)
    UDET_TRY(launch_pack_jobs(reinterpret_cast<const PackJob*>(ws + P->jobs_off[NET_GEN]), P->njobs[NET_GEN], w_gen, ws, BN_C, s));
  if (w_rec)
    UDET_TRY(launch_pack_jobs(reinterpret_cast<const PackJob*>(ws + P->jobs_off[NET_REC]), P->njobs[NET_REC], w_rec, ws, BN_C, s));
  return UDET_OK;
}

static const int PWC_CH[7] = {0, 16, 32, 64, 96, 128, 196};

static int pwc_forward_on(Plan* P, const float* img1, const float* img2, float* ws, const Lane& L0, const Lane& LH) {
  if (!P->pwc_packed) {
    set_error("pwc_forward: call udet_pack_pwc first");
    return UDET_ERR_ARG;
  }
  const Config& c = P->cfg;
  const int B = c.batch;
  hipStream_t s = L0.s;
  UDET_TRY(launch_pack_pwc_input(img1, img2, ws + P->buf(P->bid("pwc.x8")).off, (long)B * c.in_h * c.in_w, s));
  for (int l = 1; l <= 6; ++l)
    for (const char* suf : {"a", "aa", "b"}) {
      char nm[64];
      snprintf(nm, sizeof(nm), "pwcnet/featpyr/conv%d%s", l, suf);
      UDET_TRY(run_fwd(P, *find_layer(P->pwc, nm), 2 * B, ws, L0));
    }
  for (int l = 6; l >= 2; --l) {
    const int h = c.in_h >> l, w = c.in_w >> l, C = PWC_CH[l];
    const Buf& cb = P->buf(P->bid(S("pwc.c%d", l)));
    const Buf& slab = P->buf(P->bid(S("pwc.slab%d", l)));
    const float* c1 = ws + cb.off;
    const float* c2 = ws + cb.off + (size_t)B * h * w * C;
    const bool warped = l != 6;
    const double px = (double)B * h * w;
    prof_begin(P, PROF_CORR, 2.0 * px * 81.0 * C, px * ((warped ? 3.0 * C + 2.0 : 2.0 * C) + 81.0) * 4.0, s, S("warp_costvol%d", l).c_str());
    UDET_TRY(launch_warp_cost_volume(c1, c2, warped ? ws + slab.off : nullptr, slab.ld, 532 + C, 20.0f / (float)(1 << l), ws + slab.off,
                                     slab.ld, 448, warped ? 532 : -1, nullptr, B, h, w, C, s));
    prof_end(P, s);
    for (int i = 0; i < 5; ++i) UDET_TRY(run_fwd(P, *find_layer(P->pwc, S("pwcnet/predict_flow/conv%d_%d", l, i)), B, ws, L0));
    order_after(P, L0, LH);
    UDET_TRY(run_fwd(P, *find_layer(P->pwc, S("pwcnet/predict_flow/flow%d", l)), B, ws, LH));
    if (l != 2) UDET_TRY(run_fwd(P, *find_layer(P->pwc, S("pwcnet/upsample/up_feat%d", l)), B, ws, LH));
    for (int i = 1; i <= 6; ++i) UDET_TRY(run_fwd(P, *find_layer(P->pwc, S("pwcnet/ctxt/dc_conv%d%d", l, i)), B, ws, L0));
    order_after(P, LH, L0);
    UDET_TRY(run_fwd(P, *find_layer(P->pwc, S("pwcnet/ctxt/dc_conv%d%d", l, 7)), B, ws, L0));
    if (l != 2) UDET_TRY(run_fwd(P, *find_layer(P->pwc, S("pwcnet/upsample/up_flow%d", l)), B, ws, L0));
  }
  const Buf& fr = P->buf(P->bid("pwc.rflow2"));
  const Buf& ff = P->buf(P->bid("flow_full"));
  return launch_resize_bilinear_fwd(ws + fr.off, fr.ld, 0, B, fr.h, fr.w, ws + ff.off, 2, 0, c.in_h, c.in_w, 2, 4.0f, 1.f, s);
}

int plan_pwc_forward(Plan* P, const float* img1, const float* img2, float* ws, hipStream_t s) {
  P->ev_next = 0;
  if (P->prefetch_pending) (void)hipStreamWaitEvent(s, P->prefetch_ev, 0);
  return pwc_forward_on(P, img1, img2, ws, lane_of(P, s, 0), lane_of(P, s, 2));
}

static int plan_prepare_image(Plan* P, const float* img1, const char* dst, float* ws, hipStream_t s) {
// ... 65 lines not shown
    UDET_TRY(share_enc_a_output(P, L, ncalls, ws, ln.s));
  }
  P->enc_a_shared = true;
  return UDET_OK;
}

int plan_recover_forward(Plan* P, int ncalls, float* ws, hipStream_t s, bool inputs_prepacked, bool skip_enc_a, bool enc_a_input_packed) {
  const Config& c = P->cfg;
  const int B = c.batch, N = ncalls * B;
  const long Ppix = (long)B * c.img_h * c.img_w;
  const Lane L0 = lane_of(P, s, 0);
  if (!inputs_prepacked)
    UDET_TRY(launch_mask_rec_inputs(ws + P->buf(P->bid("gen.a17")).off, ws + P->buf(P->bid("flow")).off,
                                    ws + P->buf(P->bid("mask")).off, ws + P->buf(P->bid("rec.fin")).off, Ppix, ncalls, s));
  if (ncalls < 1) return UDET_OK;
  if (!skip_enc_a && pairs_on(P)) {
    if (!inputs_prepacked && !enc_a_input_packed) UDET_TRY(plan_rec_image_branch(P, ncalls, ws, L0, false));
    for (int i = 0; i < 9; ++i) {
      const Layer& La = *find_layer(P->rec, std::string("a") + ENC_NAMES[i]);
      UDET_TRY(run_fwd_pair(P, La, inputs_prepacked ? N : B, *find_layer(P->rec, std::string("b") + ENC_NAMES[i]), N, ws, L0));
      if (!inputs_prepacked) UDET_TRY(share_enc_a_output(P, La, ncalls, ws, s));
    }
    P->enc_a_shared = !inputs_prepacked;
  } else {
    if (!skip_enc_a) {
      if (inputs_prepacked) {
        for (int i = 0; i < 9; ++i) UDET_TRY(run_fwd(P, *find_layer(P->rec, std::string("a") + ENC_NAMES[i]), N, ws, L0));
        P->enc_a_shared = false;
      } else {
        UDET_TRY(plan_rec_image_branch(P, ncalls, ws, L0));
      }
    }
    for (int i = 0; i < 9; ++i) UDET_TRY(run_fwd(P, *find_layer(P->rec, std::string("b") + ENC_NAMES[i]), N, ws, L0));
  }
  for (int k = 5; k >= 1; --k) {
    const Layer& dcl = *find_layer(P->rec, S("deconv%d", k));
    if (!dcl.upb) UDET_TRY(rec_resize(P, k == 5 ? "rec.conv6" : S("rec.concat%d", k + 1).c_str(), S("rec.r%d", k + 1).c_str(), N, ws, s));
    UDET_TRY(run_fwd(P, dcl, N, ws, L0));
    if (k < 5) {
      UDET_TRY(rec_resize(P, S("rec.flow%d", k + 1).c_str(), S("rec.rf%d", k + 1).c_str(), N, ws, s));
      UDET_TRY(run_fwd(P, *find_layer(P->rec, S("upflow%d", k)), N, ws, L0));
    }
    UDET_TRY(run_fwd(P, *find_layer(P->rec, S("flow%d", k)), N, ws, L0));
  }
  const Buf& f1 = P->buf(P->bid("rec.flow1"));
  return launch_resize_bilinear_fwd(ws + f1.off, f1.ld, 0, N, f1.h, f1.w, ws + P->buf(P->bid("pred")).off, 2, 0, c.img_h,
                                    c.img_w, 2, 1.f, 1.f, s);
}

int plan_losses(Plan* P, float* ws, hipStream_t s) {
  const Config& c = P->cfg;
  float* sm = ws + P->small_off;
  const long HW = (long)c.img_h * c.img_w;
  return launch_losses(ws + P->buf(P->bid("flow")).off, ws + P->buf(P->bid("mask")).off, ws + P->buf(P->bid("pred")).off, HW,
                       c.batch, c.cbn, c.epsilon, (float)(c.img_w * c.img_h * c.batch), sm + 8192, sm, sm + 16, sm + UDET_SMALL_SUMS, s);
}

int plan_prefetch_consume(Plan* P, float* ws, hipStream_t s) {
  if (!P->prefetch_pending) {
    set_error("forward_prefetched: no udet_prefetch_flow is pending");
    return UDET_ERR_ARG;
  }
  (void)hipStreamWaitEvent(s, P->prefetch_ev, 0);
  P->prefetch_pending = false;
  const Buf &fn = P->buf(P->bid("flow.next")), &in = P->buf(P->bid("image.next"));
  UDET_HIP(hipMemcpyAsync(ws + P->buf(P->bid("flow")).off, ws + fn.off, fn.floats() * sizeof(float), hipMemcpyDeviceToDevice, s));
  UDET_HIP(hipMemcpyAsync(ws + P->buf(P->bid("image")).off, ws + in.off, in.floats() * sizeof(float), hipMemcpyDeviceToDevice, s));
  return UDET_OK;
}

int plan_forward(Plan* P, const float* img1, const float* img2, int ncalls, float* ws, hipStream_t s, bool prefetched) {
  P->ev_next = 0;
  const Lane L0 = lane_of(P, s, 0), LI = lane_of(P, s, 1);
  if (prefetched) {
    UDET_TRY(plan_prefetch_consume(P, ws, s));
    img1 = img2 = nullptr;
  } else if (img1 && P->prefetch_pending) {
    (void)hipStreamWaitEvent(s, P->prefetch_ev, 0);
  }
  order_after(P, L0, LI);
  if (img1) UDET_TRY(plan_prepare_image(P, img1, "image", ws, LI.s));
  hipEvent_t e_img = nullptr;
  if (LI.s != L0.s) {
    e_img = next_event(P);
    (void)hipEventRecord(e_img, LI.s);
  }
  const bool paired = pairs_on(P);
  UDET_TRY(plan_rec_image_branch(P, ncalls, ws, LI, !paired));
  if (img1) {
    UDET_TRY(pwc_forward_on(P, img1, img2, ws, L0, lane_of(P, s, 2)));
    UDET_TRY(plan_prepare_flow(P, "flow", ws, s));
  }
  if (e_img) (void)hipStreamWaitEvent(s, e_img, 0);
  UDET_TRY(plan_generator_forward(P, ws, s));
  order_after(P, LI, L0);
  UDET_TRY(plan_recover_forward(P, ncalls, ws, s, false, !paired, paired));
  if (ncalls == 3) UDET_TRY(plan_losses(P, ws, s));
  return UDET_OK;
}

static int rec_backward(Plan* P, int N, const char* dp, bool with_wgrad, bool need_dfin, const float* w_rec, float* g_rec, float* ws,
                        const Lane& LD, const Lane& LW, const Lane* LAp = nullptr, const Lane* LWdecp = nullptr) {
  const Config& c = P->cfg;
  hipStream_t s = LD.s;
  const std::string pre = std::string("rec.") + dp + ".", upre = std::string("rec.u") + dp + ".";
  auto B_ = [&](const std::string& n) { return P->bid(n); };
  auto D_ = [&](const std::string& n) { return P->bid(pre + n); };
  auto U_ = [&](const std::string& n) { return P->bid(upre + n); };
  auto Lr = [&](const std::string& n) { return find_layer(P->rec, n); };
  const Lane LWdec = LWdecp ? *LWdecp : LW;
  auto wgrad_on = [&](const Lane& lw, const Layer& L, int dy, bool is_du, int n) -> int {
    order_after(P, LD, lw);
    return run_wgrad(P, L, n < 0 ? N : n, dy, is_du, w_rec, g_rec, ws, lw);
  };
  auto wgrad = [&](const Layer& L, int dy, bool is_du, int n = -1) -> int { return wgrad_on(LW, L, dy, is_du, n); };
  auto wgrad_dec = [&](const Layer& L, int dy, bool is_du) -> int { return wgrad_on(LWdec, L, dy, is_du, -1); };
  const Lane LA = LAp ? *LAp : LD;
  const bool a_own_lane = LA.s != LD.s;
  const int ncopies = N / c.batch;
  const bool a_shared = P->enc_a_shared && ncopies > 1;
  const Emit none;
  const float LEAK = 0.2f;
  {
    const Buf& df1 = P->buf(D_("flow1"));
    UDET_TRY(launch_resize_bilinear_bwd(ws + P->buf(B_(std::string(dp) + ".pred")).off, 2, 0, N, c.img_h, c.img_w, ws + df1.off,
                                        df1.ld, 0, df1.h, df1.w, 2, 0, s));
  }
  for (int k = 1; k <= 5; ++k) {
    const std::string cname = S("concat%d", k);
    const int dconcat = D_(cname), uconcat = U_(cname);
    const Layer* fl = Lr(S("flow%d", k));
    const Layer* dc = Lr(S("deconv%d", k));
    Emit em;
    em.ubuf = uconcat; em.abuf = fl->x; em.c0 = 0; em.c1 = dc->cout; em.act = ACT_LEAKY; em.alpha = LEAK;
    UDET_TRY(run_dgrad(P, *fl, N, D_(S("flow%d", k)), false, dconcat, 0, k == 1 ? 0 : 1, -1, em, ws, LD));
    if (with_wgrad) UDET_TRY(wgrad_dec(*fl, D_(S("flow%d", k)), false));
    if (k < 5) {
      const Layer* uf = Lr(S("upflow%d", k));
      if (with_wgrad) UDET_TRY(wgrad_dec(*uf, dconcat, false));
      UDET_TRY(run_dgrad(P, *uf, N, dconcat, false, D_(S("rf%d", k + 1)), 0, 0, -1, none, ws, LD));
      const Buf &drf = P->buf(D_(S("rf%d", k + 1))), &dfn = P->buf(D_(S("flow%d", k + 1)));
      UDET_TRY(launch_resize_bilinear_bwd(ws + drf.off, drf.ld, 0, N, drf.h, drf.w, ws + dfn.off, dfn.ld, 0, dfn.h, dfn.w, drf.ld, 0, s));
    }
    if (with_wgrad) {
      if (dc->upb) {
        order_after(P, LD, LWdec);
        UDET_TRY(rec_resize(P, k == 5 ? "rec.conv6" : S("rec.concat%d", k + 1).c_str(), S("rec.r%d", k + 1).c_str(), N, ws, LWdec.s));
      }
// ... 63 lines not shown
  if (a_own_lane) order_after(P, LA, LD);
  if (with_wgrad && LWdec.s != LW.s) order_after(P, LWdec, LD);
  return UDET_OK;
}

static int backward_recover(Plan* P, const float* w_rec, float* g_rec, float* ws, const Lane& LD, const Lane& LW, const Lane* LA = nullptr,
                            const Lane* LWdec = nullptr) {
  const Config& c = P->cfg;
  const long BHW = (long)c.batch * c.img_h * c.img_w;
  UDET_TRY(launch_rec_loss_bwd(ws + P->buf(P->bid("flow")).off, ws + P->buf(P->bid("mask")).off, ws + P->buf(P->bid("pred")).off,
                               ws + P->buf(P->bid("d.pred")).off, BHW, c.cbn, 1.0f / (float)(c.img_w * c.img_h * c.batch), LD.s));
  return rec_backward(P, 3 * c.batch, "d", true, false, w_rec, g_rec, ws, LD, LW, LA, LWdec);
}

static int backward_generator(Plan* P, const float* w_gen, float* g_gen, float* ws, const Lane& LD, const Lane& LW, const Lane* LWlate = nullptr,
                              int nlate = 0) {
  const Config& c = P->cfg;
  const int B = c.batch;
  const long HW = (long)c.img_h * c.img_w;
  hipStream_t s = LD.s;
  float* sm = ws + P->small_off;
  auto B_ = [&](const std::string& n) { return P->bid(n); };
  UDET_TRY(launch_gen_loss_bwd(ws + P->buf(B_("flow")).off, ws + P->buf(B_("mask")).off, ws + P->buf(B_("pred")).off, sm + 16,
                               ws + P->buf(B_("e.pred")).off, ws + P->buf(B_("d.mask")).off, HW, B, c.cbn, s));
  UDET_TRY(rec_backward(P, 2 * B, "e", false, true, nullptr, nullptr, ws, LD, LD));
  UDET_TRY(launch_mask_bwd(ws + P->buf(B_("d.mask")).off, ws + P->buf(B_("rec.e.fin")).off, ws + P->buf(B_("flow")).off,
                           ws + P->buf(B_("mask")).off, ws + P->buf(B_("gen.d17")).off, B * HW, s));
  for (int i = 16; i >= 0; --i) {
    const Layer& L = P->gen[i];
    const bool has_act = L.act != ACT_NONE;
    const int dy = has_act ? B_(S("gen.u%d", i + 1)) : B_(S("gen.d%d", i + 1));
    const Lane& LWi = (LWlate && i < nlate) ? *LWlate : LW;
    order_after(P, LD, LWi);
    UDET_TRY(run_wgrad(P, L, B, dy, has_act, w_gen, g_gen, ws, LWi));
    if (i == 0) break;
    int res = -1;
    if (i == 6) res = B_("gen.d11");
    if (i == 3) res = B_("gen.d14");
    if (i == 1) res = B_("gen.d15");
    const int dx = B_(S("gen.d%d", i));
    const Layer& Lp = P->gen[i - 1];
    const int ap = Lp.y2 >= 0 ? Lp.y2 : Lp.y;
    {
      Emit em;
      if (Lp.act != ACT_NONE) { em.ubuf = B_(S("gen.u%d", i)); em.abuf = ap; em.c0 = 0; em.c1 = L.cin; em.act = Lp.act; em.alpha = Lp.alpha; }
      UDET_TRY(run_dgrad(P, L, B, dy, has_act, dx, 0, 0, res, em, ws, LD));
    }
  }
  return UDET_OK;
}

int plan_backward(Plan* P, int which, const float* w_gen, const float* w_rec, float* g_gen, float* g_rec, float* ws, hipStream_t s) {
  P->ev_next = 0;
  const Lane L0 = lane_of(P, s, 0), L1 = lane_of(P, s, 1), L2 = lane_of(P, s, 2), L3 = lane_of(P, s, 3);
  auto mark = [&](int net) {
    if (!P->grad_ev[net]) (void)hipEventCreateWithFlags(&P->grad_ev[net], hipEventDisableTiming);
    (void)hipEventRecord(P->grad_ev[net], s);
  };
  if (which == 3) {
    order_after(P, L0, L1);
    const int la = (int)plan_knob(UDET_KNOB_ENC_A_LANE);
    const Lane LA = lane_of(P, s, la > 0 && la < Plan::NLANE ? la : 0);
    const int lw = (int)plan_knob(UDET_KNOB_REC_DEC_WGRAD_LANE), le = (int)plan_knob(UDET_KNOB_REC_ENC_WGRAD_LANE);
    const Lane LWD = lane_of(P, s, lw > 0 && lw < Plan::NLANE ? lw : 3);
    const Lane LWE = lane_of(P, s, le > 0 && le < Plan::NLANE ? le : 2);
    UDET_TRY(backward_recover(P, w_rec, g_rec, ws, L0, LWE, la > 0 ? &LA : nullptr, &LWD));
    if (LWE.s != L2.s) order_after(P, LWE, L0);
    const long kl = plan_knob(UDET_KNOB_GEN_WGRAD_LATE);
    const int nlate = kl > 0 ? (int)kl : (kl < 0 ? 0 : 4);
    order_after(P, L2, L0);
    mark(NET_REC);
    UDET_TRY(backward_generator(P, w_gen, g_gen, ws, L1, L3, nlate > 0 ? &L2 : nullptr, nlate));
    order_after(P, L2, L0);
    order_after(P, L1, L0);
    order_after(P, L3, L0);
    mark(NET_GEN);
  } else if (which == 2) {
    UDET_TRY(backward_recover(P, w_rec, g_rec, ws, L0, L2, nullptr, &L3));
    order_after(P, L2, L0);
    mark(NET_REC);
  } else {
    UDET_TRY(backward_generator(P, w_gen, g_gen, ws, L0, L3));
    order_after(P, L3, L0);
    mark(NET_GEN);
  }
  return UDET_OK;
}

static int overflow_consume(Plan* P, int net, bool wait);
int plan_apply(Plan* P, int net, float* w, float* g, float* m, float* v, float* ws, hipStream_t s) {
  if (net != NET_GEN && net != NET_REC) {
    set_error("apply: net must be 1 (generator) or 2 (recover)");
    return UDET_ERR_ARG;
  }
  const Config& c = P->cfg;
  const NetParams& np = net_params(net);
  float* sm = ws + P->small_off;
  const float* flag = nullptr;
  if (net == NET_GEN) {
    const long* tab = reinterpret_cast<const long*>(ws + P->seg_off[net]);
    UDET_TRY(launch_grad_absmean(g, tab, tab + np.p.size(), (int)np.p.size(), sm + 2048, 1e-5f, sm + UDET_SMALL_NOISE, s));
    flag = sm + UDET_SMALL_NOISE;
  }
  if (c.conv_fp16) UDET_TRY(overflow_consume(P, net, true));
  const long t = ++P->adam_t;
  const double lr_t = (double)c.lr * sqrt(1.0 - pow((double)c.beta2, (double)t)) / (1.0 - pow((double)c.beta1, (double)t));
  const int* skip = nullptr;
  if (c.conv_fp16) {
    int* cnt = reinterpret_cast<int*>(sm + UDET_SMALL_OVF) + 2 * (net - 1);
    UDET_TRY(launch_nonfinite_count(g, (long)np.total, cnt, s));
    skip = cnt;
  }
  UDET_TRY(launch_adam(w, g, m, v, (long)np.total, (float)lr_t, c.beta1, c.beta2, c.adam_eps, c.clip, flag, c.noise_seed,
                       (uint64_t)t, s, 0, skip));
  if (c.conv_fp16) {
    if (!P->ovf_host) UDET_HIP(hipHostMalloc(reinterpret_cast<void**>(&P->ovf_host), 4 * sizeof(int), hipHostMallocDefault));
    if (!P->ovf_ev[net]) UDET_HIP(hipEventCreateWithFlags(&P->ovf_ev[net], hipEventDisableTiming));
    UDET_HIP(hipMemcpyAsync(P->ovf_host + 2 * (net - 1), skip, 2 * sizeof(int), hipMemcpyDeviceToHost, s));
    UDET_HIP(hipEventRecord(P->ovf_ev[net], s));
    P->ovf_pending[net] = true;
  }
  return UDET_OK;
}

static int overflow_consume(Plan* P, int net, bool wait) {
  if (!P->ovf_pending[net]) return UDET_OK;
  if (wait) UDET_HIP(hipEventSynchronize(P->ovf_ev[net]));
  else if (hipEventQuery(P->ovf_ev[net]) != hipSuccess) return UDET_OK;
  P->ovf_pending[net] = false;
  const int n = P->ovf_host[2 * (net - 1)];
  if (n > 0) {
    P->ovf_report_values += n; P->ovf_report_nets |= net; ++P->ovf_skipped;
    if (P->adam_t > 0) --P->adam_t;
  }
  return UDET_OK;
}

void plan_settle_adam_step(Plan* P) {
  if (!P->cfg.conv_fp16) return;
  for (int net = 1; net <= 2; ++net) (void)overflow_consume(P, net, true);
}

int plan_check_overflow(Plan* P, bool wait) {
  if (!P->cfg.conv_fp16) return UDET_OK;
  for (int net = 1; net <= 2; ++net) UDET_TRY(overflow_consume(P, net, wait));
  if (!P->ovf_report_values) return UDET_OK;
  const int bad = P->ovf_report_values, which = P->ovf_report_nets;
  P->ovf_report_values = 0;
  P->ovf_report_nets = 0;
  set_error("fp16 mode: %d non-finite gradient value(s) in the %s gradients -- a gradient operand times 4096 overflowed fp16 (|dU| > 16); "
            "the optimizer update(s) concerned were NOT applied (weights and Adam slots unchanged)", bad,
            which == 3 ? "generator and recover" : (which == 1 ? "generator" : "recover"));
  return UDET_ERR_OVERFLOW;
}

}
```

### unsupervised_detection_amd/engine.py

```python
from __future__ import annotations

import ctypes
from dataclasses import dataclass

import torch

from ._ffi import c_f, c_i, c_p, c_sz, check, lib
from .weights import NET_GEN, NET_REC


class _Cfg(ctypes.Structure):
    _fields_ = [("batch", c_i), ("in_h", c_i), ("in_w", c_i), ("img_h", c_i), ("img_w", c_i), ("flow_normalizer", c_f),
                ("cbn", c_f), ("epsilon", c_f), ("lr", c_f), ("beta1", c_f), ("beta2", c_f), ("adam_eps", c_f), ("clip", c_f),
                ("noise_seed", ctypes.c_ulonglong), ("conv_fp16", c_i)]


lib.udet_plan_create.restype = c_i
lib.udet_plan_create.argtypes = [ctypes.POINTER(_Cfg), ctypes.POINTER(c_p)]
lib.udet_plan_destroy.restype = None
lib.udet_plan_destroy.argtypes = [c_p]
lib.udet_workspace_bytes.restype = c_sz
lib.udet_workspace_bytes.argtypes = [c_p]
lib.udet_plan_init.restype = c_i
lib.udet_plan_init.argtypes = [c_p, c_p, c_p]
lib.udet_buffer_count.restype = c_i
lib.udet_buffer_count.argtypes = [c_p]
lib.udet_buffer_info.restype = c_i
lib.udet_buffer_info.argtypes = [c_p, c_i, ctypes.POINTER(ctypes.c_char_p), ctypes.POINTER(c_sz), ctypes.POINTER(c_i)]
lib.udet_plan_set_concurrent.restype = c_i
lib.udet_plan_set_concurrent.argtypes = [c_p, c_i]
lib.udet_plan_lane_queues.restype = c_i
lib.udet_plan_lane_queues.argtypes = [c_p, c_p, ctypes.POINTER(c_i)]
lib.udet_plan_pin_lanes.restype = c_i
lib.udet_plan_pin_lanes.argtypes = [c_p, c_p, ctypes.POINTER(c_p), c_i]
lib.udet_fp16_overflow_count.restype = ctypes.c_long
lib.udet_fp16_overflow_count.argtypes = [c_p]
lib.udet_get_adam_step.restype = ctypes.c_long
lib.udet_get_adam_step.argtypes = [c_p]
lib.udet_set_adam_step.restype = None
lib.udet_set_adam_step.argtypes = [c_p, ctypes.c_long]
for _n, _a in (("udet_pack_pwc", [c_p, c_p, c_p, c_p]), ("udet_pack_trainable", [c_p, c_p, c_p, c_p, c_p]),
               ("udet_pwc_forward", [c_p, c_p, c_p, c_p, c_p]), ("udet_forward", [c_p, c_p, c_p, c_i, c_p, c_p]),
               ("udet_forward_from_flow", [c_p, c_i, c_p, c_p]), ("udet_generator_forward", [c_p, c_p, c_p]),
               ("udet_recover_forward", [c_p, c_i, c_p, c_p]),
               ("udet_prefetch_flow", [c_p, c_p, c_p, c_p, c_p]), ("udet_forward_prefetched", [c_p, c_i, c_p, c_p]),
               ("udet_prefetch_consume", [c_p, c_p, c_p]),
               ("udet_backward", [c_p, c_i, c_p, c_p, c_p, c_p, c_p, c_p]),
               ("udet_apply", [c_p, c_i, c_p, c_p, c_p, c_p, c_p, c_p]),
               ("udet_train_step", [c_p, c_i] + [c_p] * 12)):
    getattr(lib, _n).restype = c_i
    getattr(lib, _n).argtypes = _a

lib.udet_autotune.restype = c_i
lib.udet_autotune.argtypes = [c_p] * 7
lib.udet_tuned_shapes.restype = c_i
lib.udet_tuned_shapes.argtypes = []
lib.udet_profile_begin.restype = c_i
lib.udet_profile_begin.argtypes = [c_p]
lib.udet_profile_end.restype = c_i
lib.udet_profile_end.argtypes = [c_p, ctypes.POINTER(ctypes.c_double), c_i, c_p]

GEN, REC, BOTH = 1, 2, 3
LOSS_KEYS = ("generator", "recover", "red_rate", "red_rate_compl", "reconstruction_loss", "reconstruction_compl_loss",
             "denominator_red_rate", "denominator_red_rate_compl")


@dataclass
class EngineConfig:
    batch_size: int = 4
    in_height: int = 384
    in_width: int = 640
    img_height: int = 192
    img_width: int = 384
    flow_normalizer: float = 80.0
    cbn: float = 0.5
    epsilon: float = 75.0
    beta1: float = 0.9
    lr: float = 1e-4
    beta2: float = 0.999
    adam_eps: float = 1e-8
    clip: float = 0.2
    noise_seed: int = 8964
    conv_fp16: bool = False


def _ptr(t):
    if t is None:
        return None
    if not (t.is_cuda and t.dtype == torch.float32 and t.is_contiguous()):
        raise ValueError("expected a contiguous float32 CUDA(HIP) tensor")
    return t.data_ptr()


class Engine:
    def __init__(self, cfg: EngineConfig, device="cuda"):
        if not torch.cuda.is_available():
            raise RuntimeError("unsupervised_detection_amd needs an MI355X (no CPU fallback exists)")
        self.cfg = cfg
        self.device = torch.device(device)
        c = _Cfg(cfg.batch_size, cfg.in_height, cfg.in_width, cfg.img_height, cfg.img_width, cfg.flow_normalizer, cfg.cbn,
                 cfg.epsilon, cfg.lr, cfg.beta1, cfg.beta2, cfg.adam_eps, cfg.clip, cfg.noise_seed, 1 if cfg.conv_fp16 else 0)
        h = c_p()
        check(lib.udet_plan_create(ctypes.byref(c), ctypes.byref(h)))
        self._h = h
        self.workspace_bytes = int(lib.udet_workspace_bytes(h))
        self.ws = torch.empty(self.workspace_bytes, dtype=torch.uint8, device=self.device)
        self._bufs = {}
        for i in range(lib.udet_buffer_count(h)):
            name = ctypes.c_char_p()
            off = c_sz()
            dims = (c_i * 4)()
            check(lib.udet_buffer_info(h, i, ctypes.byref(name), ctypes.byref(off), dims))
            self._bufs[name.value.decode()] = (off.value, tuple(dims))
        check(lib.udet_plan_init(h, self.ws.data_ptr(), self._stream()))

    def __del__(self):
        h = getattr(self, "_h", None)
        if h:
            lib.udet_plan_destroy(h)
            self._h = None

    @staticmethod
    def _stream():
        return torch.cuda.current_stream().cuda_stream

    def buffer_names(self):
        return list(self._bufs)

    def buffer(self, name: str) -> torch.Tensor:
        off, (n, h, w, ld) = self._bufs[name]
        cnt = n * h * w * ld
        return self.ws[off:off + 4 * cnt].view(torch.float32).view(n, h, w, ld)

    def pack_pwc(self, w_pwc):
        check(lib.udet_pack_pwc(self._h, _ptr(w_pwc), self.ws.data_ptr(), self._stream()))

    def pack_trainable(self, w_gen=None, w_rec=None):
        check(lib.udet_pack_trainable(self._h, _ptr(w_gen), _ptr(w_rec), self.ws.data_ptr(), self._stream()))

    def _check_pair(self, img1, img2):
        c = self.cfg
        want = (c.batch_size, c.in_height, c.in_width, 3)
        for name, t in (("img1", img1), ("img2", img2)):
            if tuple(t.shape) != want:
                raise ValueError("%s has shape %s, this plan takes %s (pad the last batch of a one-pass reader: "
                                 "learner.pad_batch)" % (name, tuple(t.shape), want))

    def pwc_forward(self, img1, img2):
        self._check_pair(img1, img2)
        check(lib.udet_pwc_forward(self._h, _ptr(img1), _ptr(img2), self.ws.data_ptr(), self._stream()))
        return self.buffer("flow_full")

    def forward(self, img1, img2, ncalls=3):
        self._check_pair(img1, img2)
        check(lib.udet_forward(self._h, _ptr(img1), _ptr(img2), ncalls, self.ws.data_ptr(), self._stream()))

    def prefetch_flow(self, img1, img2):
        self._check_pair(img1, img2)
        self._prefetch_keep = (img1, img2)
        check(lib.udet_prefetch_flow(self._h, _ptr(img1), _ptr(img2), self.ws.data_ptr(), self._stream()))

    def prefetch_consume(self):
        check(lib.udet_prefetch_consume(self._h, self.ws.data_ptr(), self._stream()))
        self._prefetch_keep = None

    def forward_in_place(self, ncalls=3):
        check(lib.udet_forward_from_flow(self._h, ncalls, self.ws.data_ptr(), self._stream()))

    def forward_prefetched(self, ncalls=3):
        check(lib.udet_forward_prefetched(self._h, ncalls, self.ws.data_ptr(), self._stream()))
        self._prefetch_keep = None

    def forward_from_flow(self, image, flow, ncalls=3):
        if tuple(image.shape) != tuple(self.buffer("image").shape) or tuple(flow.shape) != tuple(self.buffer("flow").shape):
            raise ValueError("image / flow must be %s / %s" % (tuple(self.buffer("image").shape), tuple(self.buffer("flow").shape)))
        self.buffer("image").copy_(image)
        self.buffer("flow").copy_(flow)
        check(lib.udet_forward_from_flow(self._h, ncalls, self.ws.data_ptr(), self._stream()))

    def losses(self):
        v = self.buffer("losses").view(-1).cpu().tolist()
        return dict(zip(LOSS_KEYS, v))

    def backward(self, which, w_gen, w_rec, g_gen, g_rec):
        check(lib.udet_backward(self._h, which, _ptr(w_gen), _ptr(w_rec), _ptr(g_gen), _ptr(g_rec), self.ws.data_ptr(),
                                self._stream()))

    def apply(self, net, w, g, m, v):
        check(lib.udet_apply(self._h, net, _ptr(w), _ptr(g), _ptr(m), _ptr(v), self.ws.data_ptr(), self._stream()))

    def train_step(self, which, img1, img2, w_gen, w_rec, g_gen, g_rec, m_gen, v_gen, m_rec, v_rec):
        self._check_pair(img1, img2)
        check(lib.udet_train_step(self._h, which, _ptr(img1), _ptr(img2), _ptr(w_gen), _ptr(w_rec), _ptr(g_gen), _ptr(g_rec),
                                  _ptr(m_gen), _ptr(v_gen), _ptr(m_rec), _ptr(v_rec), self.ws.data_ptr(), self._stream()))

    def autotune(self, w_gen, w_rec, g_gen, g_rec):
        check(lib.udet_autotune(self._h, _ptr(w_gen), _ptr(w_rec), _ptr(g_gen), _ptr(g_rec), self.ws.data_ptr(), self._stream()))
        return int(lib.udet_tuned_shapes())

    def profile(self, fn):
        cats = ("conv_fwd", "conv_dgrad", "conv_wgrad", "warp", "cost_volume")
        check(lib.udet_profile_begin(self._h))
        try:
            fn()
        finally:
            out = (ctypes.c_double * (5 * len(cats)))()
            check(lib.udet_profile_end(self._h, out, len(cats), self._stream()))
        return {c: dict(groups=out[5 * i], ms=out[5 * i + 1], flops=out[5 * i + 2], bytes=out[5 * i + 3], bracket_ms=out[5 * i + 4])
                for i, c in enumerate(cats)}

    def set_concurrent(self, on: bool):
        check(lib.udet_plan_set_concurrent(self._h, 1 if on else 0))

    def lane_queues(self):
        q = (c_i * 6)()
        n = int(lib.udet_plan_lane_queues(self._h, self._stream(), q))
        if n < 0:
            check(n)
        return n, [int(v) for v in q]

    def pin_lanes(self, side_streams):
        side_streams = list(side_streams)
        arr = (c_p * max(1, len(side_streams)))(*[s.cuda_stream for s in side_streams])
        check(lib.udet_plan_pin_lanes(self._h, self._stream(), arr, len(side_streams)))
        self._pinned_streams = getattr(self, "_pinned_streams", []) + side_streams

    def fp16_overflow_count(self) -> int:
        return int(lib.udet_fp16_overflow_count(self._h))

    @property
    def adam_step(self):
        return int(lib.udet_get_adam_step(self._h))

    @adam_step.setter
    def adam_step(self, t):
        lib.udet_set_adam_step(self._h, int(t))
```

### unsupervised_detection_amd/trainer.py

```python
from __future__ import annotations

import torch

from . import weights as W
from .engine import BOTH, GEN, REC, Engine


class TrainState:

    def __init__(self, engine: Engine, seed: int = 8964, w_pwc=None, w_gen=None, w_rec=None, autotune: bool = False):
        dev = engine.device
        self.engine = engine
        self.w_pwc = (w_pwc if w_pwc is not None else W.init_flat(W.NET_PWC, seed)).to(dev)
        self.w_gen = (w_gen if w_gen is not None else W.init_flat(W.NET_GEN, seed)).to(dev)
        self.w_rec = (w_rec if w_rec is not None else W.init_flat(W.NET_REC, seed)).to(dev)
        n_gen, n_rec = self.w_gen.numel(), self.w_rec.numel()
        off_rec = (n_gen + 63) // 64 * 64
        self.g_all = torch.zeros(off_rec + n_rec, dtype=torch.float32, device=dev)
        self.g_gen, self.g_rec = self.g_all[:n_gen], self.g_all[off_rec:off_rec + n_rec]
        self.m_gen, self.v_gen = torch.zeros_like(self.w_gen), torch.zeros_like(self.w_gen)
        self.m_rec, self.v_rec = torch.zeros_like(self.w_rec), torch.zeros_like(self.w_rec)
        engine.pack_pwc(self.w_pwc)
        engine.pack_trainable(self.w_gen, self.w_rec)
        self._dirty = 0
        if autotune:
            self.tuned_shapes = self._autotune_shared()

    def _autotune_shared(self) -> int:
        import os
        import tempfile

        import torch.distributed as dist

        from ._ffi import lib
        e = self.engine
        if not (dist.is_available() and dist.is_initialized()) or dist.get_world_size() == 1:
            return e.autotune(self.w_gen, self.w_rec, self.g_gen, self.g_rec)
        text, n = [None], 0
        fd, path = tempfile.mkstemp(prefix="udet_tune_", suffix=".txt")
        os.close(fd)
        try:
            if dist.get_rank() == 0:
                n = e.autotune(self.w_gen, self.w_rec, self.g_gen, self.g_rec)
                lib.udet_tune_save(path.encode())
                with open(path) as f:
                    text[0] = f.read()
            dist.broadcast_object_list(text, src=0)
            if dist.get_rank() != 0:
                with open(path, "w") as f:
                    f.write(text[0])
                n = int(lib.udet_tune_load(path.encode()))
                if n < 0:
                    n = e.autotune(self.w_gen, self.w_rec, self.g_gen, self.g_rec)
        finally:
            os.remove(path)
        return n


def flush_weights(st: TrainState):
    dirty = getattr(st, "_dirty", 0)
    if dirty:
        st.engine.pack_trainable(st.w_gen if dirty & GEN else None, st.w_rec if dirty & REC else None)
    st._dirty = 0


def _dp_active(group) -> bool:
    import os

    import torch.distributed as dist
    if group is False or not (dist.is_available() and dist.is_initialized()):
        return False
    return dist.get_world_size(group) > 1 or os.environ.get("UDET_DP_WORLD1") == "1"


def allreduce_mean_(t: torch.Tensor, group=None, async_op=False):
    import torch.distributed as dist
    if not _dp_active(group):
        return None
    work = dist.all_reduce(t, op=dist.ReduceOp.SUM, group=group, async_op=False)
    t.div_(dist.get_world_size(group))
    return work if async_op else None


def _exchange_gradients(st: TrainState, which: int, group):
    if not _dp_active(group):
        return
    e = st.engine
    if which != BOTH:
        allreduce_mean_(st.g_rec if which & REC else st.g_gen, group)
        return
    from ._ffi import check, lib
    comm = getattr(st, "_comm_stream", None)
    if comm is None:
        comm = st._comm_stream = torch.cuda.Stream(device=e.device)
    main = torch.cuda.current_stream(e.device)
    check(lib.udet_stream_wait_grads(e._h, W.NET_REC, comm.cuda_stream))
    with torch.cuda.stream(comm):
        allreduce_mean_(st.g_rec, group)
        done = comm.record_event()
    allreduce_mean_(st.g_gen, group)
    main.wait_event(done)


def exchange_alone(st: TrainState, group=None):
    if not _dp_active(group):
        return
    e = st.engine
    comm = getattr(st, "_comm_stream", None)
    if comm is None:
        comm = st._comm_stream = torch.cuda.Stream(device=e.device)
    main = torch.cuda.current_stream(e.device)
    comm.wait_stream(main)
    with torch.cuda.stream(comm):
        allreduce_mean_(st.g_rec, group)
        done = comm.record_event()
    allreduce_mean_(st.g_gen, group)
    main.wait_event(done)


def train_step(st: TrainState, img1, img2, which: int = BOTH, group=None, next_pair=None):
    e = st.engine
    flush_weights(st)

    def call(fn, *a):
        if not getattr(e.cfg, "conv_fp16", False):
            return fn(*a)
        from ._ffi import UdetOverflow
        for _ in range(4):
            try:
                return fn(*a)
            except UdetOverflow as ex:
                st.overflow_skipped = getattr(st, "overflow_skipped", 0) + 1
                import sys
                print("[udet] fp16 overflow: an optimizer update was dropped (%d so far): %s" % (st.overflow_skipped, ex), file=sys.stderr)
        return fn(*a)

    if getattr(st, "_prefetched", None) is not None:
        p1, p2 = st._prefetched
        if p1.data_ptr() != img1.data_ptr() or p2.data_ptr() != img2.data_ptr():
            raise ValueError("train_step: this step's pair is not the one prefetched by the previous call")
        e.prefetch_consume()
        st._prefetched = None
        if next_pair is not None:
            e.prefetch_flow(next_pair[0], next_pair[1])
            st._prefetched = (next_pair[0], next_pair[1])
        call(e.forward_in_place, 3)
    else:
        call(e.forward, img1, img2, 3)
        if next_pair is not None:
            e.prefetch_flow(next_pair[0], next_pair[1])
            st._prefetched = (next_pair[0], next_pair[1])
    call(e.backward, which, st.w_gen, st.w_rec, st.g_gen, st.g_rec)
    _exchange_gradients(st, which, group)
    if which & GEN:
        e.apply(W.NET_GEN, st.w_gen, st.g_gen, st.m_gen, st.v_gen)
    if which & REC:
        e.apply(W.NET_REC, st.w_rec, st.g_rec, st.m_rec, st.v_rec)
    st._dirty = which & (GEN | REC)
```

Baseline: 502.1.

## Defer weight packing, fuse both Adam updates, balance pack workgroups, parallelize loss finish

Weight packing can now be issued in deferred mode and joined lazily right before the generator, recover, backward or apply stages first need it, so packing can overlap with flow and forward work. The two per-network Adam updates are merged into one multi-segment launch, and the gradient abs-mean reduction is folded into that step. The pack kernel now uses a flat list of balanced workgroups instead of a fixed 48-by-jobs grid. The loss finish kernel sums block partials in parallel across threads instead of on a single thread. The changes add join bookkeeping and more complex launch setup, and the reordered loss summation can change float results slightly.

```diff
diff --git a/include/udet.h b/include/udet.h
--- a/include/udet.h
+++ b/include/udet.h
@@ -107,6 +107,9 @@
 
 int udet_pack_pwc(udet_plan* plan, const float* w_pwc, void* workspace, void* stream);
 int udet_pack_trainable(udet_plan* plan, const float* w_gen, const float* w_rec, void* workspace, void* stream);
+int udet_pack_trainable_deferred(udet_plan* plan, const float* w_gen, const float* w_rec, void* workspace, void* stream);
+int udet_plan_join(udet_plan* plan, void* stream);
+size_t udet_packed_bytes(const udet_plan* plan);
 
 int udet_pwc_forward(udet_plan* plan, const float* img1, const float* img2, void* workspace, void* stream);
 int udet_forward(udet_plan* plan, const float* img1, const float* img2, int ncalls, void* workspace, void* stream);
@@ -124,6 +127,8 @@
 int udet_recover_backward(udet_plan* plan, const float* w_rec, float* g_rec, void* workspace, void* stream);
 int udet_grad_absmean(udet_plan* plan, int net, const float* g, float* out2, void* workspace, void* stream);
 int udet_apply(udet_plan* plan, int net, float* w, float* g, float* m, float* v, void* workspace, void* stream);
+int udet_apply_both(udet_plan* plan, int first, float* w_gen, float* g_gen, float* m_gen, float* v_gen, float* w_rec, float* g_rec,
+                    float* m_rec, float* v_rec, void* workspace, void* stream);
 long udet_fp16_overflow_count(udet_plan* plan);
 long udet_get_adam_step(const udet_plan* plan);
 void udet_set_adam_step(udet_plan* plan, long t);
diff --git a/include/udet_debug.h b/include/udet_debug.h
--- a/include/udet_debug.h
+++ b/include/udet_debug.h
@@ -15,6 +15,7 @@
 int udet_debug_conv2d_pair(const float* xa, const float* xb, const float* wa, const float* wb, const float* ba, const float* bb, float* ya, float* yb,
                            int na, int nb, int h, int w, int cin, int cout, int k, int stride, int dilation, int act, float alpha, void* workspace,
                            size_t workspace_bytes, void* stream);
+int udet_debug_loss_finish_serial(const float* part, int b, float eps, float num_pixels, float* losses8, float* coef, float* sums, void* stream);
 int udet_debug_last_conv(void);
 #ifdef __cplusplus
 }
diff --git a/unsupervised_detection_amd/_devel.py b/unsupervised_detection_amd/_devel.py
--- a/unsupervised_detection_amd/_devel.py
+++ b/unsupervised_detection_amd/_devel.py
@@ -29,3 +29,6 @@
 dbg.udet_debug_last_pair.argtypes = []
 dbg.udet_debug_conv2d_pair.restype = ctypes.c_int
 dbg.udet_debug_conv2d_pair.argtypes = [ctypes.c_void_p] * 8 + [ctypes.c_int] * 10 + [ctypes.c_float, ctypes.c_void_p, ctypes.c_size_t, ctypes.c_void_p]
+dbg.udet_debug_loss_finish_serial.restype = ctypes.c_int
+dbg.udet_debug_loss_finish_serial.argtypes = [ctypes.c_void_p, ctypes.c_int, ctypes.c_float, ctypes.c_float, ctypes.c_void_p, ctypes.c_void_p, ctypes.c_void_p,
+                                              ctypes.c_void_p]
diff --git a/unsupervised_detection_amd/csrc/api_plan.hip b/unsupervised_detection_amd/csrc/api_plan.hip
--- a/unsupervised_detection_amd/csrc/api_plan.hip
+++ b/unsupervised_detection_amd/csrc/api_plan.hip
@@ -84,6 +84,15 @@
 int udet_pack_trainable(udet_plan* h, const float* w_gen, const float* w_rec, void* ws, void* stream) {
   return plan_pack_trainable(h->p, w_gen, w_rec, (float*)ws, (hipStream_t)stream);
 }
+int udet_pack_trainable_deferred(udet_plan* h, const float* w_gen, const float* w_rec, void* ws, void* stream) {
+  return plan_pack_trainable(h->p, w_gen, w_rec, (float*)ws, (hipStream_t)stream, true);
+}
+int udet_plan_join(udet_plan* h, void* stream) {
+  if (!h) { set_error("plan_join: null plan"); return UDET_ERR_ARG; }
+  plan_join_deferred(h->p, (hipStream_t)stream);
+  return UDET_OK;
+}
+size_t udet_packed_bytes(const udet_plan* h) { return h->p->packed_floats * sizeof(float); }
 int udet_pwc_forward(udet_plan* h, const float* img1, const float* img2, void* ws, void* stream) {
   return plan_pwc_forward(h->p, img1, img2, (float*)ws, (hipStream_t)stream);
 }
@@ -93,16 +102,19 @@
   return plan_forward(h->p, nullptr, nullptr, ncalls, (float*)ws, (hipStream_t)stream);
 }
 int udet_generator_forward(udet_plan* h, void* ws, void* stream) {
+  plan_join_deferred(h->p, (hipStream_t)stream);
   UDET_TRY(plan_generator_forward(h->p, (float*)ws, (hipStream_t)stream));
   return plan_recover_forward(h->p, 0, (float*)ws, (hipStream_t)stream);
 }
 int udet_generator_layers(udet_plan* h, void* ws, void* stream) {
+  plan_join_deferred(h->p, (hipStream_t)stream);
   h->p->ev_next = 0;
   UDET_TRY(plan_generator_layers(h->p, (float*)ws, (hipStream_t)stream));
   return plan_recover_forward(h->p, 0, (float*)ws, (hipStream_t)stream);
 }
 int udet_recover_forward(udet_plan* h, int n, void* ws, void* stream) {
   if (n < 1 || n > 3) { set_error("recover_forward: n must be 1..3 (multiples of the plan batch)"); return UDET_ERR_ARG; }
+  plan_join_deferred(h->p, (hipStream_t)stream);
   return plan_recover_forward(h->p, n, (float*)ws, (hipStream_t)stream, true);
 }
 int udet_forward(udet_plan* h, const float* img1, const float* img2, int ncalls, void* ws, void* stream) {
@@ -132,11 +144,17 @@
 int udet_apply(udet_plan* h, int net, float* w, float* g, float* m, float* v, void* ws, void* stream) {
   return plan_apply(h->p, net, w, g, m, v, (float*)ws, (hipStream_t)stream);
 }
+int udet_apply_both(udet_plan* h, int first, float* w_gen, float* g_gen, float* m_gen, float* v_gen, float* w_rec, float* g_rec, float* m_rec,
+                    float* v_rec, void* ws, void* stream) {
+  if (!w_gen || !g_gen || !m_gen || !v_gen || !w_rec || !g_rec || !m_rec || !v_rec) { set_error("apply_both: null argument"); return UDET_ERR_ARG; }
+  return plan_apply_both(h->p, first, w_gen, g_gen, m_gen, v_gen, w_rec, g_rec, m_rec, v_rec, (float*)ws, (hipStream_t)stream);
+}
 int udet_train_step(udet_plan* h, int which, const float* img1, const float* img2, float* w_gen, float* w_rec, float* g_gen,
                     float* g_rec, float* m_gen, float* v_gen, float* m_rec, float* v_rec, void* ws, void* stream) {
-  UDET_TRY(udet_pack_trainable(h, w_gen, w_rec, ws, stream));
+  UDET_TRY(udet_pack_trainable_deferred(h, w_gen, w_rec, ws, stream));
   UDET_TRY(udet_forward(h, img1, img2, 3, ws, stream));
   UDET_TRY(udet_backward(h, which, w_gen, w_rec, g_gen, g_rec, ws, stream));
+  if (which == 3) return udet_apply_both(h, NET_GEN, w_gen, g_gen, m_gen, v_gen, w_rec, g_rec, m_rec, v_rec, ws, stream);
   if (which & 1) UDET_TRY(udet_apply(h, NET_GEN, w_gen, g_gen, m_gen, v_gen, ws, stream));
   if (which & 2) UDET_TRY(udet_apply(h, NET_REC, w_rec, g_rec, m_rec, v_rec, ws, stream));
   return UDET_OK;
diff --git a/unsupervised_detection_amd/csrc/common.h b/unsupervised_detection_amd/csrc/common.h
--- a/unsupervised_detection_amd/csrc/common.h
+++ b/unsupervised_detection_amd/csrc/common.h
@@ -152,6 +152,11 @@
   int T, R, C, Kc, ldw, k_split, k_gap, mode;
 };
 
+struct PackWg {
+  int job, count;
+  long first;
+};
+
 struct WgradParams {
   const float* x;
   int ldx, x_coff;
diff --git a/unsupervised_detection_amd/csrc/conv_host.h b/unsupervised_detection_amd/csrc/conv_host.h
--- a/unsupervised_detection_amd/csrc/conv_host.h
+++ b/unsupervised_detection_amd/csrc/conv_host.h
@@ -53,7 +53,7 @@
                         int mode, const float* scale, hipStream_t stream);
 int launch_pack_taps_into_n(const float* src, float* dst, int T, int R, int C, int Kc, int ldz, int k_split, int k_gap,
                             int transposed, hipStream_t stream);
-int launch_pack_jobs(const PackJob* jobs_dev, int njobs, const float* wsrc, float* ws, float bn_c, hipStream_t stream);
+int launch_pack_jobs(const PackJob* jobs_dev, const PackWg* wgs_dev, int nwg, const float* wsrc, float* ws, float bn_c, hipStream_t stream);
 int launch_fold_bn(const float* b, const float* gamma, const float* beta, float c, float* scale, float* bias_f, int n,
                    hipStream_t stream);
 int launch_copy_channels(const float* src, int lds, int s_coff, float* dst, int ldd, int d_coff, long P, int C, float mul,
diff --git a/unsupervised_detection_amd/csrc/conv_host.hip b/unsupervised_detection_amd/csrc/conv_host.hip
--- a/unsupervised_detection_amd/csrc/conv_host.hip
+++ b/unsupervised_detection_amd/csrc/conv_host.hip
@@ -128,20 +128,22 @@
      {{1.f, 1.f, 0.f, 0.f}, {0.f, 0.f, 0.f, 0.f}, {0.f, 0.f, 0.f, 0.f}},
      {{0.f, .5f, 0.f, 0.f}, {0.f, -.5f, -1.f, -.5f}, {0.f, 0.f, 0.f, -.5f}}}};
 
-__global__ __launch_bounds__(256) void pack_jobs_kernel(const PackJob* __restrict__ jobs, const float* __restrict__ wsrc,
-                                                        float* __restrict__ ws, float bn_c) {
-  const PackJob j = jobs[blockIdx.y];
+__global__ __launch_bounds__(256) void pack_jobs_kernel(const PackJob* __restrict__ jobs, const PackWg* __restrict__ wgs,
+                                                        const float* __restrict__ wsrc, float* __restrict__ ws, float bn_c) {
+  const PackWg g = wgs[blockIdx.x];
+  const PackJob j = jobs[g.job];
+  const long e0 = g.first + threadIdx.x, e1 = g.first + g.count;
   const float* src = wsrc + j.src_off;
   float* dst = ws + j.dst_off;
   const float* gamma = j.gamma_off >= 0 ? wsrc + j.gamma_off : nullptr;
   if (j.mode == 2) {
-    for (long e = (long)blockIdx.x * 256 + threadIdx.x; e < j.total; e += (long)gridDim.x * 256)
+    for (long e = e0; e < e1; e += 256)
       dst[e] = gamma ? src[e] * (gamma[e] * bn_c) + wsrc[j.beta_off + e] : src[e];
     return;
   }
   if (j.mode == 9 || j.mode == 10) {
     const int rv = (int)(j.beta_off / 3), cv = (int)(j.beta_off % 3);
-    for (long e = (long)blockIdx.x * 256 + threadIdx.x; e < j.total; e += (long)gridDim.x * 256) {
+    for (long e = e0; e < e1; e += 256) {
       const int n = (int)(e % j.ldw), k = (int)(e / j.ldw);
       int ks = k;
       if (k >= j.k_split) ks = (k < j.k_split + j.k_gap) ? -1 : k - j.k_gap;
@@ -181,10 +183,10 @@
     return;
   }
   if (j.mode == 7 || j.mode == 8) {
-    for (long e = (long)blockIdx.x * 256 + threadIdx.x; e < j.total; e += (long)gridDim.x * 256) wino_pack_item(j, src, gamma, bn_c, dst, e);
+    for (long e = e0; e < e1; e += 256) wino_pack_item(j, src, gamma, bn_c, dst, e);
     return;
   }
-  for (long e = (long)blockIdx.x * 256 + threadIdx.x; e < j.total; e += (long)gridDim.x * 256) {
+  for (long e = e0; e < e1; e += 256) {
     const int n = (int)(e % j.ldw);
     const int k = (int)((e / j.ldw) % j.Kc);
     int t = (int)(e / ((long)j.ldw * j.Kc));
@@ -218,9 +220,9 @@
     dst[e] = v;
   }
 }
-int launch_pack_jobs(const PackJob* jobs_dev, int njobs, const float* wsrc, float* ws, float bn_c, hipStream_t stream) {
-  if (njobs < 1) return UDET_OK;
-  UDET_LAUNCH(pack_jobs_kernel, dim3(48, njobs), dim3(256), 0, stream, jobs_dev, wsrc, ws, bn_c);
+int launch_pack_jobs(const PackJob* jobs_dev, const PackWg* wgs_dev, int nwg, const float* wsrc, float* ws, float bn_c, hipStream_t stream) {
+  if (nwg < 1) return UDET_OK;
+  UDET_LAUNCH(pack_jobs_kernel, dim3(nwg), dim3(256), 0, stream, jobs_dev, wgs_dev, wsrc, ws, bn_c);
   UDET_HIP(hipGetLastError());
   return UDET_OK;
 }
diff --git a/unsupervised_detection_amd/csrc/devel/api_debug.hip b/unsupervised_detection_amd/csrc/devel/api_debug.hip
--- a/unsupervised_detection_amd/csrc/devel/api_debug.hip
+++ b/unsupervised_detection_amd/csrc/devel/api_debug.hip
@@ -5,6 +5,34 @@
 #include "../plan.h"
 
 using namespace udet;
+
+#define DBG_LS_BLOCKS 64
+#pragma clang fp contract(off)
+__global__ void loss_finish_serial_kernel(const float* __restrict__ part, int B, float eps, float num_pixels, float* __restrict__ losses,
+                                          float* __restrict__ coef, float* __restrict__ sums) {
+  if (threadIdx.x != 0 || blockIdx.x != 0) return;
+  float red = 0.f, redc = 0.f, rs = 0.f;
+  for (int b = 0; b < B; ++b) {
+    float v[5] = {0, 0, 0, 0, 0};
+    for (int k = 0; k < DBG_LS_BLOCKS; ++k)
+      for (int j = 0; j < 5; ++j) v[j] += part[((long)b * DBG_LS_BLOCKS + k) * 5 + j];
+    const float D = v[3] + eps, Dc = v[4] + eps;
+    red += 1.f - v[0] / D;
+    redc += 1.f - v[1] / Dc;
+    rs += v[0] + v[1] + v[2];
+    coef[b * 4 + 0] = -1.f / (B * D);
+    coef[b * 4 + 1] = v[0] / (B * D * D);
+    coef[b * 4 + 2] = -1.f / (B * Dc);
+    coef[b * 4 + 3] = v[1] / (B * Dc * Dc);
+    for (int j = 0; j < 5; ++j) sums[b * 5 + j] = v[j];
+    if (b == 0) { losses[4] = v[0]; losses[5] = v[1]; losses[6] = D; losses[7] = Dc; }
+  }
+  red /= B; redc /= B;
+  losses[0] = red + redc;
+  losses[1] = rs / num_pixels;
+  losses[2] = red;
+  losses[3] = redc;
+}
 
 extern "C" {
 int udet_debug_last_conv(void) { return conv_last_config(); }
@@ -40,6 +68,12 @@
   }
   return launch_conv_pair(p[0], p[1], stream);
 }
+int udet_debug_loss_finish_serial(const float* part, int b, float eps, float num_pixels, float* losses8, float* coef, float* sums, void* stream) {
+  if (!part || !losses8 || !coef || !sums || b < 1) { set_error("debug_loss_finish_serial: bad argument"); return UDET_ERR_ARG; }
+  hipLaunchKernelGGL(loss_finish_serial_kernel, dim3(1), dim3(64), 0, (hipStream_t)stream, part, b, eps, num_pixels, losses8, coef, sums);
+  UDET_HIP(hipGetLastError());
+  return UDET_OK;
+}
 void udet_debug_set_tuning(int on) {
   conv_set_tuning(on);
   wgrad_set_tuning(on);
diff --git a/unsupervised_detection_amd/csrc/elementwise.h b/unsupervised_detection_amd/csrc/elementwise.h
--- a/unsupervised_detection_amd/csrc/elementwise.h
+++ b/unsupervised_detection_amd/csrc/elementwise.h
@@ -27,6 +27,20 @@
                     hipStream_t s);
 int launch_grad_absmean(const float* g, const long* seg_off, const long* seg_len, int nvars, float* vmean, float thresh,
                         float* out, hipStream_t s);
+int launch_grad_abssum(const float* g, const long* seg_off, const long* seg_len, int nvars, float* vpart, hipStream_t s);
+struct AdamSeg {
+  float *w, *g, *m, *v;
+  long n;
+  float lr_t;
+  uint64_t step;
+  const int* skip;
+  const float* vpart;
+  const long* seg_len;
+  int nvars;
+  float thresh;
+  float* flag_out;
+};
+int launch_adam_step(const AdamSeg* seg, int nseg, float b1, float b2, float eps, float clip, uint64_t seed, hipStream_t s);
 int launch_adam(float* w, float* g, float* m, float* v, long n, float lr_t, float b1, float b2, float eps, float clip,
                 const float* flag, uint64_t seed, uint64_t step, hipStream_t s, int mode = 0, const int* skip = nullptr);
 int launch_nonfinite_count(const float* g, long n, int* out, hipStream_t s);
diff --git a/unsupervised_detection_amd/csrc/elementwise.hip b/unsupervised_detection_amd/csrc/elementwise.hip
--- a/unsupervised_detection_amd/csrc/elementwise.hip
+++ b/unsupervised_detection_amd/csrc/elementwise.hip
@@ -517,6 +517,7 @@
   return cbn == 0.5f ? e / sqrtf(s) : cbn * powf(s, cbn - 1.f) * 2.f * e;
 }
 #define LS_BLOCKS 64
+static_assert(LS_BLOCKS % 8 == 0, "loss_finish_kernel adds the block partials eight at a time");
 __global__ __launch_bounds__(256) void loss_sums_kernel(const float* __restrict__ f, const float* __restrict__ mask,
                                                         const float* __restrict__ pred , long HW, int B,
                                                         float cbn, float* __restrict__ part ) {
@@ -541,14 +542,29 @@
     o[0] = R; o[1] = Rc; o[2] = Pp; o[3] = Dr; o[4] = Dc;
   }
 }
-__global__ void loss_finish_kernel(const float* __restrict__ part, int B, float eps, float num_pixels,
-                                   float* __restrict__ losses, float* __restrict__ coef, float* __restrict__ sums) {
-  if (threadIdx.x != 0 || blockIdx.x != 0) return;
+__global__ __launch_bounds__(64) void loss_finish_kernel(const float* __restrict__ part, int B, float eps, float num_pixels,
+                                                         float* __restrict__ losses, float* __restrict__ coef, float* __restrict__ sums) {
+  extern __shared__ float lsum[];
+  if (blockIdx.x != 0) return;
+  for (int idx = threadIdx.x; idx < B * 5; idx += blockDim.x) {
+    const int b = idx / 5, j = idx - b * 5;
+    const float* p = part + (long)b * LS_BLOCKS * 5 + j;
+    float acc = 0.f;
+    for (int k = 0; k < LS_BLOCKS; k += 8) {
+      float t[8];
+#pragma unroll
+      for (int u = 0; u < 8; ++u) t[u] = p[(long)(k + u) * 5];
+#pragma unroll
+      for (int u = 0; u < 8; ++u) acc += t[u];
+    }
+    lsum[idx] = acc;
+  }
+  __syncthreads();
+  if (threadIdx.x != 0) return;
   float red = 0.f, redc = 0.f, rs = 0.f;
   for (int b = 0; b < B; ++b) {
-    float v[5] = {0, 0, 0, 0, 0};
-    for (int k = 0; k < LS_BLOCKS; ++k)
-      for (int j = 0; j < 5; ++j) v[j] += part[((long)b * LS_BLOCKS + k) * 5 + j];
+    float v[5];
+    for (int j = 0; j < 5; ++j) v[j] = lsum[b * 5 + j];
     const float D = v[3] + eps, Dc = v[4] + eps;
     red += 1.f - v[0] / D;
     redc += 1.f - v[1] / Dc;
@@ -569,7 +585,7 @@
 int launch_losses(const float* f, const float* mask, const float* pred, long HW, int B, float cbn, float eps,
                   float num_pixels, float* part, float* losses, float* coef, float* sums, hipStream_t s) {
   hipLaunchKernelGGL(loss_sums_kernel, dim3(LS_BLOCKS, B), dim3(256), 0, s, f, mask, pred, HW, B, cbn, part);
-  hipLaunchKernelGGL(loss_finish_kernel, dim3(1), dim3(64), 0, s, part, B, eps, num_pixels, losses, coef, sums);
+  hipLaunchKernelGGL(loss_finish_kernel, dim3(1), dim3(64), (size_t)B * 5 * sizeof(float), s, part, B, eps, num_pixels, losses, coef, sums);
   UDET_HIP(hipGetLastError());
   return UDET_OK;
 }
@@ -718,6 +734,32 @@
   UDET_HIP(hipGetLastError());
   return UDET_OK;
 }
+int launch_grad_abssum(const float* g, const long* seg_off, const long* seg_len, int nvars, float* vpart, hipStream_t s) {
+  hipLaunchKernelGGL(grad_absmean_kernel, dim3(nvars, GA_SPLIT), dim3(256), 0, s, g, seg_off, seg_len, vpart);
+  UDET_HIP(hipGetLastError());
+  return UDET_OK;
+}
+#define GF_MAXVARS 1024
+__device__ __forceinline__ float grad_flag_block(const float* __restrict__ vpart, const long* __restrict__ seg_len, int nvars, float thresh,
+                                                 float* __restrict__ out, float* sh ) {
+  for (int i = threadIdx.x; i < nvars; i += blockDim.x) {
+    float v = 0.f;
+    for (int j = 0; j < GA_SPLIT; ++j) v += vpart[i * GA_SPLIT + j];
+    sh[i] = v / (float)seg_len[i];
+  }
+  __syncthreads();
+  if (threadIdx.x == 0) {
+    float s = 0.f;
+#pragma unroll 8
+    for (int i = 0; i < nvars; ++i) s += sh[i];
+    s /= (float)nvars;
+    const float f = s < thresh ? 1.f : 0.f;
+    if (out) { out[0] = s; out[1] = f; }
+    sh[GF_MAXVARS] = f;
+  }
+  __syncthreads();
+  return sh[GF_MAXVARS];
+}
 
 __device__ __host__ __forceinline__ float udet_uniform01(uint64_t seed, uint64_t step, uint64_t idx) {
   uint64_t z = seed * 0x9E3779B97F4A7C15ull + step * 0xBF58476D1CE4E5B9ull + idx + 0x94D049BB133111EBull;
@@ -727,26 +769,42 @@
   return (float)(z >> 40) * (1.0f / 16777216.0f);
 }
 
+__device__ __forceinline__ void adam_range(float* __restrict__ w, float* __restrict__ g, float* __restrict__ m, float* __restrict__ v, long n,
+                                           long first, long stride, float lr_t, float b1, float b2, float eps, float clip, bool noise,
+                                           uint64_t seed, uint64_t step, int mode) {
+  for (long i = first; i < n; i += stride) {
+    float gi = g[i];
+    if (mode != 2) {
+      if (noise) gi = fabsf((udet_uniform01(seed, step, (uint64_t)i) * 2.f - 1.f) * clip);
+      else gi = fminf(fmaxf(gi, -clip), clip);
+      g[i] = gi;
+      if (mode == 1) continue;
+    }
+    const float mi = m[i] + (gi - m[i]) * (1.f - b1);
+    const float vi = v[i] + (gi * gi - v[i]) * (1.f - b2);
+    m[i] = mi;
+    v[i] = vi;
+    w[i] = w[i] - lr_t * mi / (sqrtf(vi) + eps);
+  }
+}
 __global__ __launch_bounds__(256) void adam_kernel(float* __restrict__ w, float* __restrict__ g, float* __restrict__ m,
                                                    float* __restrict__ v, long n, float lr_t, float b1, float b2, float eps,
                                                    float clip, const float* __restrict__ flag, uint64_t seed,
                                                    uint64_t step, int mode, const int* __restrict__ skip) {
   if (skip && *skip != 0) return;
   const bool noise = flag && flag[1] != 0.f;
-  for (long i = (long)blockIdx.x * 256 + threadIdx.x; i < n; i += (long)gridDim.x * 256) {
-    float gi = g[i];
-    if (mode != 2) {
-      if (noise) gi = fabsf((udet_uniform01(seed, step, (uint64_t)i) * 2.f - 1.f) * clip);
-      else gi = fminf(fmaxf(gi, -clip), clip);
-      g[i] = gi;
-      if (mode == 1) continue;
-    }
-    const float mi = m[i] + (gi - m[i]) * (1.f - b1);
-    const float vi = v[i] + (gi * gi - v[i]) * (1.f - b2);
-    m[i] = mi;
-    v[i] = vi;
-    w[i] = w[i] - lr_t * mi / (sqrtf(vi) + eps);
-  }
+  adam_range(w, g, m, v, n, (long)blockIdx.x * 256 + threadIdx.x, (long)gridDim.x * 256, lr_t, b1, b2, eps, clip, noise, seed, step, mode);
+}
+__global__ __launch_bounds__(256) void adam_step_kernel(const AdamSeg a, const AdamSeg b, int nblk_a, float b1, float b2, float eps, float clip,
+                                                        uint64_t seed) {
+  __shared__ float sh[GF_MAXVARS + 1];
+  const bool in_a = (int)blockIdx.x < nblk_a;
+  const AdamSeg& sg = in_a ? a : b;
+  const int blk = in_a ? (int)blockIdx.x : (int)blockIdx.x - nblk_a, nblk = in_a ? nblk_a : (int)gridDim.x - nblk_a;
+  bool noise = false;
+  if (sg.vpart) noise = grad_flag_block(sg.vpart, sg.seg_len, sg.nvars, sg.thresh, blk == 0 ? sg.flag_out : nullptr, sh) != 0.f;
+  if (sg.skip && *sg.skip != 0) return;
+  adam_range(sg.w, sg.g, sg.m, sg.v, sg.n, (long)blk * 256 + threadIdx.x, (long)nblk * 256, sg.lr_t, b1, b2, eps, clip, noise, seed, sg.step, 0);
 }
 __global__ __launch_bounds__(256) void fill_uniform_kernel(float* __restrict__ x, long n, uint64_t seed, float lo, float hi) {
   for (long i = (long)blockIdx.x * 256 + threadIdx.x; i < n; i += (long)gridDim.x * 256)
@@ -793,6 +851,15 @@
                 const float* flag, uint64_t seed, uint64_t step, hipStream_t s, int mode, const int* skip) {
   hipLaunchKernelGGL(adam_kernel, dim3(grid_for(n, 2048)), dim3(256), 0, s, w, g, m, v, n, lr_t, b1, b2, eps, clip, flag, seed,
                      step, mode, skip);
+  UDET_HIP(hipGetLastError());
+  return UDET_OK;
+}
+int launch_adam_step(const AdamSeg* seg, int nseg, float b1, float b2, float eps, float clip, uint64_t seed, hipStream_t s) {
+  if (nseg < 1 || nseg > 2) { set_error("adam_step: one or two segments"); return UDET_ERR_ARG; }
+  for (int k = 0; k < nseg; ++k)
+    if (seg[k].vpart && seg[k].nvars > GF_MAXVARS) { set_error("adam_step: %d variables exceed the flag table (%d)", seg[k].nvars, GF_MAXVARS); return UDET_ERR_ARG; }
+  const int na = grid_for(seg[0].n, 2048), nb = nseg == 2 ? grid_for(seg[1].n, 2048) : 0;
+  hipLaunchKernelGGL(adam_step_kernel, dim3(na + nb), dim3(256), 0, s, seg[0], seg[nseg - 1], na, b1, b2, eps, clip, seed);
   UDET_HIP(hipGetLastError());
   return UDET_OK;
 }
diff --git a/unsupervised_detection_amd/csrc/plan.h b/unsupervised_detection_amd/csrc/plan.h
--- a/unsupervised_detection_amd/csrc/plan.h
+++ b/unsupervised_detection_amd/csrc/plan.h
@@ -107,6 +107,11 @@
   size_t seg_off[3] = {0, 0, 0};
   size_t jobs_off[3] = {0, 0, 0};
   int njobs[3] = {0, 0, 0};
+  size_t wgs_off[3] = {0, 0, 0};
+  int nwg[3] = {0, 0, 0}, nwg_fwd[3] = {0, 0, 0};
+  enum { PEND_REC_FWD = 0, PEND_BWD = 1, NPEND = 2 };
+  hipEvent_t pend_ev[NPEND] = {nullptr, nullptr};
+  bool pend[NPEND] = {false, false};
   struct ProfRec {
     int cat; double flops, bytes; hipEvent_t a, b; std::string name;
     double mfma_scale = 1.0;
@@ -123,6 +128,7 @@
   long ovf_skipped = 0;
   int ovf_report_values = 0, ovf_report_nets = 0;
   bool pwc_packed = false;
+  bool trainable_packed = false;
   int add_buf(const std::string& name, int n, int h, int w, int ld);
   const Buf& buf(int id) const { return bufs[id]; }
   int bid(const std::string& name) const;
@@ -134,7 +140,7 @@
 #define UDET_SMALL_SUMS 1024
 Plan* plan_build(const Config& cfg);
 void plan_debug_upb_min_pixels(long v);
-enum { UDET_KNOB_ENC_A_LANE = 0, UDET_KNOB_REC_DEC_WGRAD_LANE = 1, UDET_KNOB_REC_ENC_WGRAD_LANE = 2, UDET_KNOB_GEN_WGRAD_LATE = 3, UDET_KNOB_NO_WGRAD_WINO = 6, UDET_KNOB_SKIP = 7, UDET_KNOB_NO_PAIRS = 8, UDET_KNOB_COUNT = 12 };
+enum { UDET_KNOB_ENC_A_LANE = 0, UDET_KNOB_REC_DEC_WGRAD_LANE = 1, UDET_KNOB_REC_ENC_WGRAD_LANE = 2, UDET_KNOB_GEN_WGRAD_LATE = 3, UDET_KNOB_NO_WGRAD_WINO = 6, UDET_KNOB_SKIP = 7, UDET_KNOB_NO_PAIRS = 8, UDET_KNOB_PACK_WG_WORK = 9, UDET_KNOB_EAGER_HEAD = 10, UDET_KNOB_COUNT = 12 };
 #ifdef UDET_EXPERIMENT
 void plan_debug_knob(int id, long v);
 long plan_knob(int id);
@@ -144,7 +150,9 @@
 
 int plan_init_workspace(Plan* P, float* ws, hipStream_t s);
 int plan_pack_pwc(Plan* P, const float* w_pwc, float* ws, hipStream_t s);
-int plan_pack_trainable(Plan* P, const float* w_gen, const float* w_rec, float* ws, hipStream_t s);
+int plan_pack_trainable(Plan* P, const float* w_gen, const float* w_rec, float* ws, hipStream_t s, bool deferred = false);
+void plan_join_deferred(Plan* P, hipStream_t s);
+void plan_pack_tables(const Plan* P, int net, std::vector<PackJob>& jobs, std::vector<PackWg>& wgs, int* nwg_fwd);
 int plan_pwc_forward(Plan* P, const float* img1, const float* img2, float* ws, hipStream_t s);
 int plan_forward(Plan* P, const float* img1, const float* img2, int ncalls, float* ws, hipStream_t s, bool prefetched = false);
 int plan_prefetch(Plan* P, const float* img1, const float* img2, float* ws, hipStream_t s);
@@ -155,6 +163,8 @@
 int plan_losses(Plan* P, float* ws, hipStream_t s);
 int plan_backward(Plan* P, int which, const float* w_gen, const float* w_rec, float* g_gen, float* g_rec, float* ws, hipStream_t s);
 int plan_apply(Plan* P, int net, float* w, float* g, float* m, float* v, float* ws, hipStream_t s);
+int plan_apply_both(Plan* P, int first, float* w_gen, float* g_gen, float* m_gen, float* v_gen, float* w_rec, float* g_rec, float* m_rec,
+                    float* v_rec, float* ws, hipStream_t s);
 int plan_check_overflow(Plan* P, bool wait);
 void plan_settle_adam_step(Plan* P);
 int plan_lane_queues(Plan* P, hipStream_t s, int* queue);
diff --git a/unsupervised_detection_amd/csrc/plan_build.hip b/unsupervised_detection_amd/csrc/plan_build.hip
--- a/unsupervised_detection_amd/csrc/plan_build.hip
+++ b/unsupervised_detection_amd/csrc/plan_build.hip
@@ -167,6 +167,8 @@
   for (auto& e : ev_pool) (void)hipEventDestroy(e);
   for (auto& e : ev_pool_prefetch) (void)hipEventDestroy(e);
   if (prefetch_ev) (void)hipEventDestroy(prefetch_ev);
+  for (auto& ev : pend_ev)
+    if (ev) (void)hipEventDestroy(ev);
   for (auto* r : prof) delete r;
   for (auto& ev : grad_ev)
     if (ev) (void)hipEventDestroy(ev);
@@ -568,6 +570,14 @@
     P->jobs_off[net] = off;
     off = align64(off + UDET_PACKJOB_CAP(nl) * (sizeof(PackJob) / sizeof(float)) + 64);
   }
+  for (int net = 1; net <= 2; ++net) {
+    std::vector<PackJob> jobs;
+    std::vector<PackWg> wgs;
+    plan_pack_tables(P, net, jobs, wgs, &P->nwg_fwd[net]);
+    P->nwg[net] = (int)wgs.size();
+    P->wgs_off[net] = off;
+    off = align64(off + wgs.size() * (sizeof(PackWg) / sizeof(float)) + 64);
+  }
   P->arena_floats = off;
   if (const char* e = getenv("UDET_SERIAL")) P->concurrent = atoi(e) == 0;
   for (int i = 0; i < Plan::NCAND; ++i) {
diff --git a/unsupervised_detection_amd/csrc/plan_exec.hip b/unsupervised_detection_amd/csrc/plan_exec.hip
--- a/unsupervised_detection_amd/csrc/plan_exec.hip
+++ b/unsupervised_detection_amd/csrc/plan_exec.hip
@@ -506,6 +506,87 @@
   return rc;
 }
 
+static inline bool pack_job_is_bwd(int mode) { return mode == 1 || mode == 6 || mode == 8 || mode == 10; }
+void plan_pack_tables(const Plan* P, int net, std::vector<PackJob>& out_jobs, std::vector<PackWg>& wgs, int* nwg_fwd) {
+  const NetParams& np = net_params(net);
+  const std::vector<Layer>& layers = net == NET_GEN ? P->gen : P->rec;
+  std::vector<PackJob> jobs;
+  for (const auto& L : layers) {
+    const int T = L.kh * L.kw;
+    const long goff = L.g_idx >= 0 ? (long)np.p[L.g_idx].offset : -1, beoff = L.be_idx >= 0 ? (long)np.p[L.be_idx].offset : -1;
+    PackJob j;
+    memset(&j, 0, sizeof(j));
+    j.src_off = (long)np.p[L.w_idx].offset; j.gamma_off = goff; j.beta_off = beoff;
+    j.T = T;
+    j.dst_off = (long)L.wp_off; j.R = L.cin; j.C = L.cout; j.Kc = L.Kc; j.ldw = L.ldw; j.k_split = L.k_split; j.k_gap = L.k_gap;
+    j.mode = 0; j.total = (long)T * L.Kc * L.ldw;
+    jobs.push_back(j);
+    j.dst_off = (long)L.wpT_off; j.Kc = L.KcT; j.ldw = L.ldwT; j.k_split = L.KcT; j.k_gap = 0;
+    j.mode = 1; j.total = (long)T * L.KcT * L.ldwT;
+    jobs.push_back(j);
+    if (L.col2im) {
+      j.dst_off = (long)L.wz_off; j.R = L.cin; j.C = L.cout; j.Kc = L.Kc; j.ldw = L.ldz; j.k_split = L.k_split; j.k_gap = L.k_gap;
+      j.mode = 3; j.total = (long)L.Kc * L.ldz;
+      jobs.push_back(j);
+    }
+    if (L.up) {
+      j.T = 16;
+      j.dst_off = (long)L.wu_off; j.R = L.cin; j.C = L.cout; j.Kc = L.Kc; j.ldw = L.ldw; j.k_split = L.Kc; j.k_gap = 0;
+      j.mode = 5; j.total = (long)16 * L.Kc * L.ldw;
+      jobs.push_back(j);
+      j.dst_off = (long)L.wuT_off; j.Kc = L.KcT; j.ldw = L.ldwT; j.k_split = L.KcT; j.k_gap = 0;
+      j.mode = 6; j.total = (long)16 * L.KcT * L.ldwT;
+      jobs.push_back(j);
+      j.T = T;
+    }
+    if (L.upb)
+      for (int r = 0; r < 4; ++r) {
+        j.T = 36; j.gamma_off = -1;
+        j.dst_off = (long)(L.wupb_off + (size_t)r * 36 * L.Kc * L.ldw); j.R = L.cin; j.C = L.cout; j.Kc = L.Kc; j.ldw = L.ldw; j.k_split = L.k_split; j.k_gap = L.k_gap;
+        j.mode = 9; j.beta_off = (long)((r & 1) * 3 + (r >> 1)); j.total = (long)L.Kc * L.ldw;
+        jobs.push_back(j);
+        if (L.upb_bwd) {
+          j.dst_off = (long)(L.wupbT_off + (size_t)r * 36 * L.KcT * L.ldwT); j.Kc = L.KcT; j.ldw = L.ldwT; j.k_split = L.KcT; j.k_gap = 0;
+          j.mode = 10; j.total = (long)L.KcT * L.ldwT;
+          jobs.push_back(j);
+        }
+        j.T = T; j.beta_off = beoff;
+      }
+    if (L.wino_off) {
+      j.dst_off = (long)L.wino_off; j.R = L.cin; j.C = L.cout; j.Kc = L.Kc; j.ldw = L.wino_np; j.k_split = L.k_split; j.k_gap = L.k_gap;
+      j.mode = 7; j.total = (long)(L.Kc / 8) * 2 * L.wino_np;
+      jobs.push_back(j);
+    }
+    if (L.winoT_off) {
+      j.dst_off = (long)L.winoT_off; j.R = L.cin; j.C = L.cout; j.Kc = L.KcT; j.ldw = L.winoT_np; j.k_split = L.KcT; j.k_gap = 0;
+      j.mode = 8; j.total = (long)(L.KcT / 8) * 2 * L.winoT_np;
+      jobs.push_back(j);
+    }
+    j.src_off = (long)np.p[L.b_idx].offset; j.dst_off = (long)L.bias_f_off; j.mode = 2; j.total = L.cout;
+    jobs.push_back(j);
+  }
+  out_jobs.clear();
+  wgs.clear();
+  const long PACK_WG_WORK = plan_knob(UDET_KNOB_PACK_WG_WORK) > 0 ? plan_knob(UDET_KNOB_PACK_WG_WORK) : 2048;
+  for (int grp = 0; grp < 2; ++grp) {
+    for (const PackJob& j : jobs) {
+      if ((int)pack_job_is_bwd(j.mode) != grp) continue;
+      const long per_item = (j.mode == 9 || j.mode == 10) ? 36 : ((j.mode == 7 || j.mode == 8) ? 64 : 1);
+      long chunk = (PACK_WG_WORK / per_item + 255) / 256 * 256;
+      if (chunk < 256) chunk = 256;
+      for (long first = 0; first < j.total; first += chunk) {
+        PackWg g;
+        g.job = (int)out_jobs.size();
+        g.first = first;
+        g.count = (int)(j.total - first < chunk ? j.total - first : chunk);
+        wgs.push_back(g);
+      }
+      out_jobs.push_back(j);
+    }
+    if (grp == 0) *nwg_fwd = (int)wgs.size();
+  }
+}
+
 int plan_init_workspace(Plan* P, float* ws, hipStream_t s) {
   UDET_HIP(hipMemsetAsync(ws, 0, P->arena_floats * sizeof(float), s));
   for (int net = 1; net <= 2; ++net) {
@@ -519,70 +600,23 @@
     UDET_HIP(hipStreamSynchronize(s));
   }
   for (int net = 1; net <= 2; ++net) {
-    const NetParams& np = net_params(net);
     const std::vector<Layer>& layers = net == NET_GEN ? P->gen : P->rec;
     std::vector<PackJob> jobs;
-    for (const auto& L : layers) {
-      const int T = L.kh * L.kw;
-      const long goff = L.g_idx >= 0 ? (long)np.p[L.g_idx].offset : -1, beoff = L.be_idx >= 0 ? (long)np.p[L.be_idx].offset : -1;
-      PackJob j;
-      memset(&j, 0, sizeof(j));
-      j.src_off = (long)np.p[L.w_idx].offset; j.gamma_off = goff; j.beta_off = beoff;
-      j.T = T;
-      j.dst_off = (long)L.wp_off; j.R = L.cin; j.C = L.cout; j.Kc = L.Kc; j.ldw = L.ldw; j.k_split = L.k_split; j.k_gap = L.k_gap;
-      j.mode = 0; j.total = (long)T * L.Kc * L.ldw;
-      jobs.push_back(j);
-      j.dst_off = (long)L.wpT_off; j.Kc = L.KcT; j.ldw = L.ldwT; j.k_split = L.KcT; j.k_gap = 0;
-      j.mode = 1; j.total = (long)T * L.KcT * L.ldwT;
-      jobs.push_back(j);
-      if (L.col2im) {
-        j.dst_off = (long)L.wz_off; j.R = L.cin; j.C = L.cout; j.Kc = L.Kc; j.ldw = L.ldz; j.k_split = L.k_split; j.k_gap = L.k_gap;
-        j.mode = 3; j.total = (long)L.Kc * L.ldz;
-        jobs.push_back(j);
-      }
-      if (L.up) {
-        j.T = 16;
-        j.dst_off = (long)L.wu_off; j.R = L.cin; j.C = L.cout; j.Kc = L.Kc; j.ldw = L.ldw; j.k_split = L.Kc; j.k_gap = 0;
-        j.mode = 5; j.total = (long)16 * L.Kc * L.ldw;
-        jobs.push_back(j);
-        j.dst_off = (long)L.wuT_off; j.Kc = L.KcT; j.ldw = L.ldwT; j.k_split = L.KcT; j.k_gap = 0;
-        j.mode = 6; j.total = (long)16 * L.KcT * L.ldwT;
-        jobs.push_back(j);
-        j.T = T;
-      }
-      if (L.upb)
-        for (int r = 0; r < 4; ++r) {
-          j.T = 36; j.gamma_off = -1;
-          j.dst_off = (long)(L.wupb_off + (size_t)r * 36 * L.Kc * L.ldw); j.R = L.cin; j.C = L.cout; j.Kc = L.Kc; j.ldw = L.ldw; j.k_split = L.k_split; j.k_gap = L.k_gap;
-          j.mode = 9; j.beta_off = (long)((r & 1) * 3 + (r >> 1)); j.total = (long)L.Kc * L.ldw;
-          jobs.push_back(j);
-          if (L.upb_bwd) {
-            j.dst_off = (long)(L.wupbT_off + (size_t)r * 36 * L.KcT * L.ldwT); j.Kc = L.KcT; j.ldw = L.ldwT; j.k_split = L.KcT; j.k_gap = 0;
-            j.mode = 10; j.total = (long)L.KcT * L.ldwT;
-            jobs.push_back(j);
-          }
-          j.T = T; j.beta_off = beoff;
-        }
-      if (L.wino_off) {
-        j.dst_off = (long)L.wino_off; j.R = L.cin; j.C = L.cout; j.Kc = L.Kc; j.ldw = L.wino_np; j.k_split = L.k_split; j.k_gap = L.k_gap;
-        j.mode = 7; j.total = (long)(L.Kc / 8) * 2 * L.wino_np;
-        jobs.push_back(j);
-      }
-      if (L.winoT_off) {
-        j.dst_off = (long)L.winoT_off; j.R = L.cin; j.C = L.cout; j.Kc = L.KcT; j.ldw = L.winoT_np; j.k_split = L.KcT; j.k_gap = 0;
-        j.mode = 8; j.total = (long)(L.KcT / 8) * 2 * L.winoT_np;
-        jobs.push_back(j);
-      }
-      j.src_off = (long)np.p[L.b_idx].offset; j.dst_off = (long)L.bias_f_off; j.mode = 2; j.total = L.cout;
-      jobs.push_back(j);
-    }
+    std::vector<PackWg> wgs;
+    int nfwd = 0;
+    plan_pack_tables(P, net, jobs, wgs, &nfwd);
     if (jobs.size() > UDET_PACKJOB_CAP(layers.size())) {
       set_error("plan_init: %zu weight re-layout jobs for %zu layers exceed the table's %zu entries", jobs.size(), layers.size(),
                 (size_t)UDET_PACKJOB_CAP(layers.size()));
       return UDET_ERR_ARG;
     }
+    if ((int)wgs.size() != P->nwg[net] || nfwd != P->nwg_fwd[net]) {
+      set_error("plan_init: re-layout workgroup table of net %d changed since plan_build (%zu vs %d)", net, wgs.size(), P->nwg[net]);
+      return UDET_ERR_ARG;
+    }
     P->njobs[net] = (int)jobs.size();
     UDET_HIP(hipMemcpyAsync(ws + P->jobs_off[net], jobs.data(), jobs.size() * sizeof(PackJob), hipMemcpyHostToDevice, s));
+    UDET_HIP(hipMemcpyAsync(ws + P->wgs_off[net], wgs.data(), wgs.size() * sizeof(PackWg), hipMemcpyHostToDevice, s));
     UDET_HIP(hipStreamSynchronize(s));
   }
   for (const auto& L : P->rec)
@@ -622,11 +656,45 @@
   return UDET_OK;
 }
 
-int plan_pack_trainable(Plan* P, const float* w_gen, const float* w_rec, float* ws, hipStream_t s) {
-  if (w_gen)
-    UDET_TRY(launch_pack_jobs(reinterpret_cast<const PackJob*>(ws + P->jobs_off[NET_GEN]), P->njobs[NET_GEN], w_gen, ws, BN_C, s));
-  if (w_rec)
-    UDET_TRY(launch_pack_jobs(reinterpret_cast<const PackJob*>(ws + P->jobs_off[NET_REC]), P->njobs[NET_REC], w_rec, ws, BN_C, s));
+static void join_deferred(Plan* P, hipStream_t s, int k) {
+  if (!P->pend[k]) return;
+  (void)hipStreamWaitEvent(s, P->pend_ev[k], 0);
+  P->pend[k] = false;
+}
+void plan_join_deferred(Plan* P, hipStream_t s) {
+  for (int k = 0; k < Plan::NPEND; ++k) join_deferred(P, s, k);
+}
+static int pack_range(Plan* P, int net, const float* w, int w0, int w1, float* ws, hipStream_t s) {
+  return launch_pack_jobs(reinterpret_cast<const PackJob*>(ws + P->jobs_off[net]), reinterpret_cast<const PackWg*>(ws + P->wgs_off[net]) + w0,
+                          w1 - w0, w, ws, BN_C, s);
+}
+
+int plan_pack_trainable(Plan* P, const float* w_gen, const float* w_rec, float* ws, hipStream_t s, bool deferred) {
+  if (((plan_knob(UDET_KNOB_SKIP) >> 7) & 1) && P->trainable_packed) return UDET_OK;
+  P->trainable_packed = true;
+  plan_join_deferred(P, s);
+  const Lane L3 = (deferred && !plan_knob(UDET_KNOB_EAGER_HEAD)) ? lane_of(P, s, 3) : Lane{s, 0};
+  if (L3.s == s) {
+    if (w_gen) UDET_TRY(pack_range(P, NET_GEN, w_gen, 0, P->nwg[NET_GEN], ws, s));
+    if (w_rec) UDET_TRY(pack_range(P, NET_REC, w_rec, 0, P->nwg[NET_REC], ws, s));
+    return UDET_OK;
+  }
+  for (int k = 0; k < Plan::NPEND; ++k)
+    if (!P->pend_ev[k]) UDET_HIP(hipEventCreateWithFlags(&P->pend_ev[k], hipEventDisableTiming));
+  (void)hipEventRecord(P->pend_ev[Plan::PEND_BWD], s);
+  (void)hipStreamWaitEvent(L3.s, P->pend_ev[Plan::PEND_BWD], 0);
+  if (w_gen) UDET_TRY(pack_range(P, NET_GEN, w_gen, 0, P->nwg_fwd[NET_GEN], ws, s));
+  if (w_rec) {
+    UDET_TRY(pack_range(P, NET_REC, w_rec, 0, P->nwg_fwd[NET_REC], ws, L3.s));
+    (void)hipEventRecord(P->pend_ev[Plan::PEND_REC_FWD], L3.s);
+    P->pend[Plan::PEND_REC_FWD] = true;
+  }
+  if (w_gen) UDET_TRY(pack_range(P, NET_GEN, w_gen, P->nwg_fwd[NET_GEN], P->nwg[NET_GEN], ws, L3.s));
+  if (w_rec) UDET_TRY(pack_range(P, NET_REC, w_rec, P->nwg_fwd[NET_REC], P->nwg[NET_REC], ws, L3.s));
+  if (w_gen || w_rec) {
+    (void)hipEventRecord(P->pend_ev[Plan::PEND_BWD], L3.s);
+    P->pend[Plan::PEND_BWD] = true;
+  }
   return UDET_OK;
 }
 
@@ -798,6 +866,7 @@
   const Config& c = P->cfg;
   float* sm = ws + P->small_off;
   const long HW = (long)c.img_h * c.img_w;
+  if ((plan_knob(UDET_KNOB_SKIP) >> 9) & 1) return UDET_OK;
   return launch_losses(ws + P->buf(P->bid("flow")).off, ws + P->buf(P->bid("mask")).off, ws + P->buf(P->bid("pred")).off, HW,
                        c.batch, c.cbn, c.epsilon, (float)(c.img_w * c.img_h * c.batch), sm + 8192, sm, sm + 16, sm + UDET_SMALL_SUMS, s);
 }
@@ -818,6 +887,7 @@
 int plan_forward(Plan* P, const float* img1, const float* img2, int ncalls, float* ws, hipStream_t s, bool prefetched) {
   P->ev_next = 0;
   const Lane L0 = lane_of(P, s, 0), LI = lane_of(P, s, 1);
+  if (!pairs_on(P)) join_deferred(P, s, Plan::PEND_REC_FWD);
   if (prefetched) {
     UDET_TRY(plan_prefetch_consume(P, ws, s));
     img1 = img2 = nullptr;
@@ -840,6 +910,7 @@
   if (e_img) (void)hipStreamWaitEvent(s, e_img, 0);
   UDET_TRY(plan_generator_forward(P, ws, s));
   order_after(P, LI, L0);
+  join_deferred(P, s, Plan::PEND_REC_FWD);
   UDET_TRY(plan_recover_forward(P, ncalls, ws, s, false, !paired, paired));
   if (ncalls == 3) UDET_TRY(plan_losses(P, ws, s));
   return UDET_OK;
@@ -1009,6 +1080,7 @@
 
 int plan_backward(Plan* P, int which, const float* w_gen, const float* w_rec, float* g_gen, float* g_rec, float* ws, hipStream_t s) {
   P->ev_next = 0;
+  plan_join_deferred(P, s);
   const Lane L0 = lane_of(P, s, 0), L1 = lane_of(P, s, 1), L2 = lane_of(P, s, 2), L3 = lane_of(P, s, 3);
   auto mark = [&](int net) {
     if (!P->grad_ev[net]) (void)hipEventCreateWithFlags(&P->grad_ev[net], hipEventDisableTiming);
@@ -1045,39 +1117,65 @@
 }
 
 static int overflow_consume(Plan* P, int net, bool wait);
-int plan_apply(Plan* P, int net, float* w, float* g, float* m, float* v, float* ws, hipStream_t s) {
-  if (net != NET_GEN && net != NET_REC) {
-    set_error("apply: net must be 1 (generator) or 2 (recover)");
-    return UDET_ERR_ARG;
-  }
+static int apply_prepare(Plan* P, int net, float* w, float* g, float* m, float* v, float* ws, hipStream_t s, AdamSeg& sg) {
   const Config& c = P->cfg;
   const NetParams& np = net_params(net);
   float* sm = ws + P->small_off;
-  const float* flag = nullptr;
+  memset(&sg, 0, sizeof(sg));
+  sg.w = w; sg.g = g; sg.m = m; sg.v = v; sg.n = (long)np.total;
   if (net == NET_GEN) {
     const long* tab = reinterpret_cast<const long*>(ws + P->seg_off[net]);
-    UDET_TRY(launch_grad_absmean(g, tab, tab + np.p.size(), (int)np.p.size(), sm + 2048, 1e-5f, sm + UDET_SMALL_NOISE, s));
-    flag = sm + UDET_SMALL_NOISE;
+    UDET_TRY(launch_grad_abssum(g, tab, tab + np.p.size(), (int)np.p.size(), sm + 2048, s));
+    sg.vpart = sm + 2048; sg.seg_len = tab + np.p.size(); sg.nvars = (int)np.p.size(); sg.thresh = 1e-5f; sg.flag_out = sm + UDET_SMALL_NOISE;
   }
   if (c.conv_fp16) UDET_TRY(overflow_consume(P, net, true));
   const long t = ++P->adam_t;
   const double lr_t = (double)c.lr * sqrt(1.0 - pow((double)c.beta2, (double)t)) / (1.0 - pow((double)c.beta1, (double)t));
-  const int* skip = nullptr;
+  sg.lr_t = (float)lr_t; sg.step = (uint64_t)t;
   if (c.conv_fp16) {
     int* cnt = reinterpret_cast<int*>(sm + UDET_SMALL_OVF) + 2 * (net - 1);
     UDET_TRY(launch_nonfinite_count(g, (long)np.total, cnt, s));
-    skip = cnt;
-  }
-  UDET_TRY(launch_adam(w, g, m, v, (long)np.total, (float)lr_t, c.beta1, c.beta2, c.adam_eps, c.clip, flag, c.noise_seed,
-                       (uint64_t)t, s, 0, skip));
+    sg.skip = cnt;
+  }
+  return UDET_OK;
+}
+static bool apply_args_ok(int net) {
+  if (net == NET_GEN || net == NET_REC) return true;
+  set_error("apply: net must be 1 (generator) or 2 (recover)");
+  return false;
+}
+int plan_apply(Plan* P, int net, float* w, float* g, float* m, float* v, float* ws, hipStream_t s) {
+  if (!apply_args_ok(net)) return UDET_ERR_ARG;
+  if ((plan_knob(UDET_KNOB_SKIP) >> 8) & 1) return UDET_OK;
+  plan_join_deferred(P, s);
+  const Config& c = P->cfg;
+  AdamSeg sg;
+  UDET_TRY(apply_prepare(P, net, w, g, m, v, ws, s, sg));
+  UDET_TRY(launch_adam_step(&sg, 1, c.beta1, c.beta2, c.adam_eps, c.clip, c.noise_seed, s));
   if (c.conv_fp16) {
     if (!P->ovf_host) UDET_HIP(hipHostMalloc(reinterpret_cast<void**>(&P->ovf_host), 4 * sizeof(int), hipHostMallocDefault));
     if (!P->ovf_ev[net]) UDET_HIP(hipEventCreateWithFlags(&P->ovf_ev[net], hipEventDisableTiming));
-    UDET_HIP(hipMemcpyAsync(P->ovf_host + 2 * (net - 1), skip, 2 * sizeof(int), hipMemcpyDeviceToHost, s));
+    UDET_HIP(hipMemcpyAsync(P->ovf_host + 2 * (net - 1), sg.skip, 2 * sizeof(int), hipMemcpyDeviceToHost, s));
     UDET_HIP(hipEventRecord(P->ovf_ev[net], s));
     P->ovf_pending[net] = true;
   }
   return UDET_OK;
+}
+int plan_apply_both(Plan* P, int first, float* w_gen, float* g_gen, float* m_gen, float* v_gen, float* w_rec, float* g_rec, float* m_rec,
+                    float* v_rec, float* ws, hipStream_t s) {
+  if (!apply_args_ok(first)) return UDET_ERR_ARG;
+  const Config& c = P->cfg;
+  float* const a[3][4] = {{nullptr, nullptr, nullptr, nullptr}, {w_gen, g_gen, m_gen, v_gen}, {w_rec, g_rec, m_rec, v_rec}};
+  const int order[2] = {first, first == NET_GEN ? NET_REC : NET_GEN};
+  if (c.conv_fp16) {
+    for (int net : order) UDET_TRY(plan_apply(P, net, a[net][0], a[net][1], a[net][2], a[net][3], ws, s));
+    return UDET_OK;
+  }
+  if ((plan_knob(UDET_KNOB_SKIP) >> 8) & 1) return UDET_OK;
+  plan_join_deferred(P, s);
+  AdamSeg sg[2];
+  for (int k = 0; k < 2; ++k) UDET_TRY(apply_prepare(P, order[k], a[order[k]][0], a[order[k]][1], a[order[k]][2], a[order[k]][3], ws, s, sg[k]));
+  return launch_adam_step(sg, 2, c.beta1, c.beta2, c.adam_eps, c.clip, c.noise_seed, s);
 }
 
 static int overflow_consume(Plan* P, int net, bool wait) {
diff --git a/unsupervised_detection_amd/engine.py b/unsupervised_detection_amd/engine.py
--- a/unsupervised_detection_amd/engine.py
+++ b/unsupervised_detection_amd/engine.py
@@ -23,6 +23,8 @@
 lib.udet_workspace_bytes.argtypes = [c_p]
 lib.udet_plan_init.restype = c_i
 lib.udet_plan_init.argtypes = [c_p, c_p, c_p]
+lib.udet_packed_bytes.restype = c_sz
+lib.udet_packed_bytes.argtypes = [c_p]
 lib.udet_buffer_count.restype = c_i
 lib.udet_buffer_count.argtypes = [c_p]
 lib.udet_buffer_info.restype = c_i
@@ -47,6 +49,8 @@
                ("udet_prefetch_consume", [c_p, c_p, c_p]),
                ("udet_backward", [c_p, c_i, c_p, c_p, c_p, c_p, c_p, c_p]),
                ("udet_apply", [c_p, c_i, c_p, c_p, c_p, c_p, c_p, c_p]),
+               ("udet_pack_trainable_deferred", [c_p, c_p, c_p, c_p, c_p]), ("udet_plan_join", [c_p, c_p]),
+               ("udet_apply_both", [c_p, c_i] + [c_p] * 10),
                ("udet_train_step", [c_p, c_i] + [c_p] * 12)):
     getattr(lib, _n).restype = c_i
     getattr(lib, _n).argtypes = _a
@@ -138,6 +142,16 @@
     def pack_trainable(self, w_gen=None, w_rec=None):
         check(lib.udet_pack_trainable(self._h, _ptr(w_gen), _ptr(w_rec), self.ws.data_ptr(), self._stream()))
 
+    def pack_trainable_deferred(self, w_gen=None, w_rec=None):
+        check(lib.udet_pack_trainable_deferred(self._h, _ptr(w_gen), _ptr(w_rec), self.ws.data_ptr(), self._stream()))
+
+    def join(self):
+        check(lib.udet_plan_join(self._h, self._stream()))
+
+    @property
+    def packed_bytes(self) -> int:
+        return int(lib.udet_packed_bytes(self._h))
+
     def _check_pair(self, img1, img2):
         c = self.cfg
         want = (c.batch_size, c.in_height, c.in_width, 3)
@@ -188,6 +202,10 @@
 
     def apply(self, net, w, g, m, v):
         check(lib.udet_apply(self._h, net, _ptr(w), _ptr(g), _ptr(m), _ptr(v), self.ws.data_ptr(), self._stream()))
+
+    def apply_both(self, first, w_gen, g_gen, m_gen, v_gen, w_rec, g_rec, m_rec, v_rec):
+        check(lib.udet_apply_both(self._h, first, _ptr(w_gen), _ptr(g_gen), _ptr(m_gen), _ptr(v_gen), _ptr(w_rec), _ptr(g_rec),
+                                  _ptr(m_rec), _ptr(v_rec), self.ws.data_ptr(), self._stream()))
 
     def train_step(self, which, img1, img2, w_gen, w_rec, g_gen, g_rec, m_gen, v_gen, m_rec, v_rec):
         self._check_pair(img1, img2)
diff --git a/unsupervised_detection_amd/trainer.py b/unsupervised_detection_amd/trainer.py
--- a/unsupervised_detection_amd/trainer.py
+++ b/unsupervised_detection_amd/trainer.py
@@ -57,10 +57,11 @@
         return n
 
 
-def flush_weights(st: TrainState):
+def flush_weights(st: TrainState, deferred: bool = False):
     dirty = getattr(st, "_dirty", 0)
     if dirty:
-        st.engine.pack_trainable(st.w_gen if dirty & GEN else None, st.w_rec if dirty & REC else None)
+        pack = st.engine.pack_trainable_deferred if deferred else st.engine.pack_trainable
+        pack(st.w_gen if dirty & GEN else None, st.w_rec if dirty & REC else None)
     st._dirty = 0
 
 
@@ -120,7 +121,7 @@
 
 def train_step(st: TrainState, img1, img2, which: int = BOTH, group=None, next_pair=None):
     e = st.engine
-    flush_weights(st)
+    flush_weights(st, deferred=True)
 
     def call(fn, *a):
         if not getattr(e.cfg, "conv_fp16", False):
@@ -152,8 +153,11 @@
             st._prefetched = (next_pair[0], next_pair[1])
     call(e.backward, which, st.w_gen, st.w_rec, st.g_gen, st.g_rec)
     _exchange_gradients(st, which, group)
-    if which & GEN:
-        e.apply(W.NET_GEN, st.w_gen, st.g_gen, st.m_gen, st.v_gen)
-    if which & REC:
-        e.apply(W.NET_REC, st.w_rec, st.g_rec, st.m_rec, st.v_rec)
+    if which == BOTH:
+        e.apply_both(W.NET_GEN, st.w_gen, st.g_gen, st.m_gen, st.v_gen, st.w_rec, st.g_rec, st.m_rec, st.v_rec)
+    else:
+        if which & GEN:
+            e.apply(W.NET_GEN, st.w_gen, st.g_gen, st.m_gen, st.v_gen)
+        if which & REC:
+            e.apply(W.NET_REC, st.w_rec, st.g_rec, st.m_rec, st.v_rec)
     st._dirty = which & (GEN | REC)
```

Result: no change. 502.9 (median of 6 runs) (+0.2%).
